# shiyao-li/NextBestPath

Hardware: AMD Instinct MI355X
Metric: exploration steps/s (+ NBP maps/s) at 256x256 (higher is better)
Workload: dtype f32

## Files before the change

include/nbp_hip.h:

```cpp
#ifndef NBP_HIP_H
#define NBP_HIP_H

#include <stddef.h>
#include <stdint.h>

#ifdef __cplusplus
extern "C" {
#endif

#define NBP_E_ARG      (-1)
#define NBP_E_WS       (-2)
#define NBP_E_SHAPE    (-3)

int nbp_abi_version(void);
int nbp_device_info(char* arch_host, int arch_len, int* cu_count_host);
int nbp_tuning_active(void);
int nbp_tuning_report(char* buf_host, int len);
int nbp_tile_kernel_symbol(int tile, char* buf_host, int len);

#define NBP_N_CONV 48

typedef struct nbp_weights nbp_weights;

size_t nbp_packed_weights_bytes(void);

int nbp_pack_weights(const void* const* w_host_array, const void* const* scale_host_array,
                     const void* const* shift_host_array, void* packed, size_t packed_bytes,
                     void* stream, nbp_weights** handle_out);
void nbp_free_weights(nbp_weights* handle);

size_t nbp_forward_workspace_bytes(int B, int S);

int nbp_forward_f32(const nbp_weights* handle, const float* x, int B, int S, float* out1,
                    float* out2, void* ws, size_t ws_bytes, void* stream);

typedef struct nbp_layer_timing {
    char name[48];
    double flops;
    float ms;
    int tile, split_k;
    long long M;
    int N, K;
} nbp_layer_timing;
int nbp_forward_timed_f32(const nbp_weights* handle, const float* x, int B, int S, float* out1,
                          float* out2, void* ws, size_t ws_bytes, void* stream,
                          nbp_layer_timing* timings_host, int max_entries, int* n_entries_host);

double nbp_forward_flops(int B, int S);

int nbp_pack_weights_bf16(const void* const* w_host_array, const void* const* scale_host_array,
                          const void* const* shift_host_array, void* packed, size_t packed_bytes,
                          void* stream, nbp_weights** handle_out);
size_t nbp_packed_weights_bytes_bf16(void);
size_t nbp_forward_workspace_bytes_bf16(int B, int S);
int nbp_pack_upconv_weight_bf16(const float* w_oihw, int N, int C, unsigned short* dst, void* stream);
int nbp_forward_bf16(const nbp_weights* handle, const float* x, int B, int S, float* out1,
                     float* out2, void* ws, size_t ws_bytes, void* stream);
int nbp_forward_timed_bf16(const nbp_weights* handle, const float* x, int B, int S, float* out1,
                           float* out2, void* ws, size_t ws_bytes, void* stream,
                           nbp_layer_timing* timings_host, int max_entries, int* n_entries_host);

size_t nbp_packed_weights_bytes_split(void);
int nbp_pack_weights_split(const void* const* w_host_array, const void* const* scale_host_array,
                           const void* const* shift_host_array, void* packed, size_t packed_bytes, void* stream,
                           nbp_weights** handle_out);
size_t nbp_forward_workspace_bytes_split(int B, int S);
int nbp_forward_split_f32(const nbp_weights* handle, const float* x, int B, int S, float* out1, float* out2, void* ws,
                          size_t ws_bytes, void* stream);
int nbp_forward_timed_split_f32(const nbp_weights* handle, const float* x, int B, int S, float* out1, float* out2,
                                void* ws, size_t ws_bytes, void* stream, nbp_layer_timing* timings_host,
                                int max_entries, int* n_entries_host);
int nbp_pack_conv_weight_split(const float* w_oihw, int N, int C, int ksize, const float* scale_or_null, int c_off,
                               int c_total, void* dst_planes, void* wamax_out, void* stream);
int nbp_amax_f32(const float* x, long long n, void* amax_inout, void* stream);
int nbp_pack_upconv_weight_split(const float* w_oihw, int N, int C, void* dst_planes, void* wamax_out, void* stream);
int nbp_upconv3x3_split_f32(const float* src, int C, int B, int H, int W, const void* planes_up, const void* wamax_up, int N,
                            const float* scale, const float* shift, int relu, float* out, const void* amax_in_or_null,
                            void* amax_out_or_null, int split_k, void* ws, size_t ws_bytes, void* stream);
size_t nbp_conv_split_workspace_bytes(int B, int H, int W, int N, int split_k);
size_t nbp_conv_split_planned_workspace_bytes(int B, int H, int W, int C, int N, int ups, int* split_k_out);
size_t nbp_conv_split_planned_workspace_bytes_k(int B, int H, int W, int C, int N, int ups, int split_k, int* split_k_out);
int nbp_conv3x3_split_f32(const float* src0, int C0, const float* src1, int C1, int ups, int B, int H, int W,
                          const void* w_planes, const void* wamax, int N, const float* scale, const float* shift, int relu,
                          float* out, const void* amax_in_or_null, void* amax_out_or_null, int split_k, void* ws,
                          size_t ws_bytes, void* stream);
size_t nbp_conv_first_wgrad_workspace_bytes(void);
int nbp_conv_first_wgrad_f32(const float* x_nchw, int B, int H, int W, const float* dy, float* dw, void* ws, size_t ws_bytes, void* stream);
int nbp_prepack_weights_split(const void* descs_dev, int n, void* wamax_words, void* stream);
int nbp_prepack_desc_bytes(void);
int nbp_pack_conv_weight_split_prezeroed(const float* w_oihw, int N, int C, int ksize, int c_total, void* dst_planes,
                                         void* wamax_zeroed, void* stream);
int nbp_pack_conv_weight_split_dgrad_known(const float* w_oihw, int N, int C, int c_total, void* dst_planes, const void* wamax_known,
                                           void* stream);
int nbp_pack_upconv_weight_split_dgrad(const float* w_oihw, int N, int C, void* dst_planes, void* wamax_out, void* stream);
size_t nbp_upconv_split_dgrad_workspace_bytes(int B, int H, int W, int N, int C);
int nbp_upconv3x3_split_dgrad_f32(const float* dy, int N, int B, int H, int W, const void* planes, const void* wamax, int C,
                                  const float* scale, const float* shift, float* dx, const void* amax_in, void* amax_out_or_null,
                                  void* ws, size_t ws_bytes, void* stream);
size_t nbp_upconv_wgrad_split_workspace_bytes(int B, int Hs, int Ws, int C, int N);
int nbp_upconv_wgrad_split_f32(const float* x, int C, int B, int Hs, int Ws, const float* dy, int N, float* dw,
                               const void* amax_x, const void* amax_y, void* ws, size_t ws_bytes, void* stream);
int nbp_conv1x1_split_f32(const float* src, int C, long long M, const void* w_planes, const void* wamax, int N,
                          const float* scale, const float* shift, int relu, float* out, const void* amax_in, void* stream);
int nbp_pack_conv1x1_weight_split_dgrad(const float* w_nc, int N, int C, void* dst_planes, void* wamax_out, void* stream);
int nbp_pack_conv_weight_split_dgrad(const float* w_oihw, int N, int C, int c_total, void* dst_planes, void* wamax_out, void* stream);

int nbp_conv_bn_part_rows(int B, int H, int W);
int nbp_conv3x3_split_bn_f32(const float* src0, int C0, const float* src1, int C1, int ups, int B, int H, int W,
                             const void* w_planes, const void* wamax, int N, const float* scale, const float* shift, int relu,
                             float* out, const void* amax_in_or_null, void* amax_out_or_null, int split_k, void* ws,
                             size_t ws_bytes, double* bn_part, int* bn_rows, void* stream);
int nbp_upconv3x3_split_bn_f32(const float* src, int C, int B, int H, int W, const void* planes_up, const void* wamax_up, int N,
                               const float* scale, const float* shift, int relu, float* out, const void* amax_in_or_null,
                               void* amax_out_or_null, int split_k, void* ws, size_t ws_bytes, double* bn_part, int* bn_rows,
                               void* stream);
int nbp_pack_conv_weight_split_h1(const float* w_oihw, int N, int C, int ksize, const float* scale_or_null, int c_off,
                                  int c_total, void* dst_planes, void* wamax_out, void* stream);
int nbp_pack_conv_weight_split_prezeroed_h1(const float* w_oihw, int N, int C, int ksize, int c_total, void* dst_planes,
                                            void* wamax_zeroed, void* stream);
int nbp_pack_conv_weight_split_dgrad_h1(const float* w_oihw, int N, int C, int c_total, void* dst_planes, void* wamax_out, void* stream);
int nbp_pack_conv_weight_split_dgrad_known_h1(const float* w_oihw, int N, int C, int c_total, void* dst_planes, const void* wamax_known,
                                              void* stream);
int nbp_pack_upconv_weight_split_h1(const float* w_oihw, int N, int C, void* dst_planes, void* wamax_out, void* stream);
int nbp_pack_upconv_weight_split_dgrad_h1(const float* w_oihw, int N, int C, void* dst_planes, void* wamax_out, void* stream);
int nbp_pack_conv1x1_weight_split_dgrad_h1(const float* w_nc, int N, int C, void* dst_planes, void* wamax_out, void* stream);
int nbp_prepack_weights_split_h1(const void* descs_dev, int n, void* wamax_words, void* stream);
int nbp_conv3x3_split_f32_h1(const float* src0, int C0, const float* src1, int C1, int ups, int B, int H, int W,
                             const void* w_planes, const void* wamax, int N, const float* scale, const float* shift, int relu,
                             float* out, const void* amax_in_or_null, void* amax_out_or_null, int split_k, void* ws,
                             size_t ws_bytes, void* stream);
int nbp_conv3x3_split_bn_f32_h1(const float* src0, int C0, const float* src1, int C1, int ups, int B, int H, int W,
                                const void* w_planes, const void* wamax, int N, const float* scale, const float* shift, int relu,
                                float* out, const void* amax_in_or_null, void* amax_out_or_null, int split_k, void* ws,
                                size_t ws_bytes, double* bn_part, int* bn_rows, void* stream);
int nbp_upconv3x3_split_f32_h1(const float* src, int C, int B, int H, int W, const void* planes_up, const void* wamax_up, int N,
                               const float* scale, const float* shift, int relu, float* out, const void* amax_in_or_null,
                               void* amax_out_or_null, int split_k, void* ws, size_t ws_bytes, void* stream);
int nbp_upconv3x3_split_bn_f32_h1(const float* src, int C, int B, int H, int W, const void* planes_up, const void* wamax_up, int N,
                                  const float* scale, const float* shift, int relu, float* out, const void* amax_in_or_null,
                                  void* amax_out_or_null, int split_k, void* ws, size_t ws_bytes, double* bn_part, int* bn_rows,
                                  void* stream);
int nbp_upconv3x3_split_dgrad_f32_h1(const float* dy, int N, int B, int H, int W, const void* planes, const void* wamax, int C,
                                     const float* scale, const float* shift, float* dx, const void* amax_in, void* amax_out_or_null,
                                     void* ws, size_t ws_bytes, void* stream);
int nbp_conv1x1_split_f32_h1(const float* src, int C, long long M, const void* w_planes, const void* wamax, int N,
                             const float* scale, const float* shift, int relu, float* out, const void* amax_in, void* stream);
int nbp_upconv_wgrad_split_f32_h1(const float* x, int C, int B, int Hs, int Ws, const float* dy, int N, float* dw,
                                  const void* amax_x, const void* amax_y, void* ws, size_t ws_bytes, void* stream);
int nbp_conv_wgrad_split_f32_h1(const float* src0, int C0, const float* src1, int C1, int ups, int B, int H, int W, int ksize,
                                const float* dy, int N, int c_real, int n_real, float* dw, const void* amax0_or_null,
                                const void* amax1_or_null, const void* amaxy_or_null, void* ws, size_t ws_bytes, void* stream);
int nbp_bn_train_forward_part4_f32(const float* x, long long M, int C, const float* gamma, const float* beta, float eps,
                                   float momentum, float* running_mean, float* running_var, int relu, float* mean, float* invstd,
                                   float* y, void* amax_out, double* stat_out, int stat_doubles, const double* part, int rows,
                                   const float* zero_row, void* stream);
int nbp_conv_igemm_bf16(const unsigned short* src0, int C0, const unsigned short* src1, int C1, int ups,
                        int B, int H, int W, int ksize, const unsigned short* w_packed, int N,
                        const float* scale, const float* shift, int relu, unsigned short* out,
                        int split_k, int tile, void* ws, size_t ws_bytes, void* stream);
size_t nbp_conv_igemm_bf16_workspace_bytes(int B, int H, int W, int N, int split_k);
int nbp_pack_conv_weight_bf16(const float* w_oihw, int N, int C, int ksize, const float* scale_or_null,
                              int c_off, int c_total, unsigned short* dst, void* stream);
int nbp_f32_to_bf16(const float* in, long long n, unsigned short* out, void* stream);
int nbp_bf16_to_f32(const unsigned short* in, long long n, float* out, void* stream);

int nbp_conv_igemm_f32(const float* src0, int C0, const float* src1, int C1, int ups, int B, int H,
                       int W, int ksize, const float* w_packed, int N, const float* scale,
                       const float* shift, int relu, float* out, int split_k, int tile, void* ws,
                       size_t ws_bytes, void* stream);
size_t nbp_conv_igemm_workspace_bytes(int B, int H, int W, int N, int split_k);

int nbp_pack_conv_weight(const float* w_oihw, int N, int C, int ksize, const float* scale_or_null,
                         int c_off, int c_total, float* dst, void* stream);

int nbp_conv_first_f32(const float* x_nchw, int B, int H, int W, const float* w_oihw,
                       const float* scale, const float* shift, float* out_nhwc, void* stream);
int nbp_conv_first_linear_f32(const float* x_nchw, int B, int H, int W, const float* w_oihw, const float* scale,
                              const float* shift, float* out_nhwc, void* stream);
int nbp_maxpool2_nhwc_f32(const float* in, int B, int H, int W, int C, float* out, void* stream);
int nbp_psi_gate_f32(const float* q, int F, const float* w_psi, const float* s_t2, const float* x,
                     int C, long long M, float* out, void* stream);
int nbp_final_1x1_f32(const float* in, int B, int H, int W, int C, const float* w_oc, int n_out,
                      const float* scale, const float* shift, int sigmoid, float* out_nchw,
                      void* stream);
int nbp_nchw_to_nhwc_f32(const float* in, int B, int C, int H, int W, float* out, void* stream);
int nbp_nhwc_to_nchw_f32(const float* in, int B, int C, int H, int W, float* out, void* stream);

int nbp_transform_points_f32(const float* points, long long N, float cx, float cy, float cz,
                             float* out_2d, void* stream);
int nbp_map_points_to_imgs_f32(const float* pts2d, int n, long long m, int S0, int S1, float lo,
                               float hi, float* out, void* stream);
int nbp_point_position_i64(const float* pts2d, long long K, int S0, int S1, float lo, float hi,
                           long long* out_2xK, void* stream);
int nbp_map_accumulate_f32(const float* points, long long N, const long long* N_dev_or_null, float cx,
                           float cy, float cz, const float* bounds_host, int n_bounds, float band_lo,
                           float band_hi, int S, float lo, float hi, float* out6, void* stream);
int nbp_step_maps_f32(const float* points, long long N, const long long* N_dev_or_null, float cx, float cy,
                      float cz, const float* bounds_host, int n_bounds, float band_lo, float band_hi, int S,
                      float lo, float hi, float* traj_pts, int n_traj_old, const float* traj_fresh_host,
                      int n_traj_fresh, float* out6, float* net_in5, void* stream);
int nbp_step_maps_batch_f32(int n, const float* const* points, const long long* N_cap, const long long* const* N_dev,
                            const float* poses_xyz_host, const float* bounds_host, const int* n_bounds,
                            const float* band_lo_hi_host, int S, float lo, float hi, float* const* traj_pts,
                            const int* n_traj_old, const float* traj_fresh_host, const int* n_traj_fresh,
                            float* out6_all, float* net_in_all, void* stream);
size_t nbp_cloud_bins_bytes(const float* lo_xz_host, const float* hi_xz_host, long long capacity);
int nbp_cloud_bins_geometry(const float* lo_xz_host, const float* hi_xz_host, long long capacity, int* nx_nz_maxpages_host,
                            float* x0_z0_tile_host);
int nbp_cloud_bins_init(void* store, size_t store_bytes, const float* lo_xz_host, const float* hi_xz_host, long long capacity,
                        void* stream);
int nbp_step_maps_binned_f32(void* store, int page_bound, const float* points, long long N, const long long* N_dev_or_null,
                             float cx, float cy, float cz, const float* bounds_host, int n_bounds, float band_lo, float band_hi,
                             int S, float lo, float hi, float* traj_pts, int n_traj_old, const float* traj_fresh_host,
                             int n_traj_fresh, float* out6, float* net_in5, void* stream);
int nbp_step_maps_prefiled_f32(void* store, int page_bound, const float* points, long long N, const long long* N_dev_or_null,
                               float cx, float cy, float cz, const float* bounds_host, int n_bounds, float band_lo, float band_hi,
                               int S, float lo, float hi, float* traj_pts, int n_traj_old, const float* traj_fresh_host,
                               int n_traj_fresh, float* out6, float* net_in5, void* stream);
int nbp_step_maps_binned_batch_f32(int n, void* const* stores, const int* page_bound, const float* const* points,
                                   const long long* N_cap, const long long* const* N_dev, const float* poses_xyz_host,
                                   const float* bounds_host, const int* n_bounds, const float* band_lo_hi_host, int S, float lo,
                                   float hi, float* const* traj_pts, const int* n_traj_old, const float* traj_fresh_host,
                                   const int* n_traj_fresh, float* out6_all, float* net_in_all, void* stream);
int nbp_coverage_count_planned_batch_f32(int n, void* const* plans, const int* G, float threshold, const float* bbox_lo_host,
                                         const float* bbox_hi_host, const float* const* pc3, const long long* N,
                                         const long long* const* N_dev, const long long* sample_k, const unsigned* seed,
                                         const unsigned* epoch, int* const* count_accum, int* const* m_out, void* stream);
int nbp_unproject_append_shaded_batch_f32(int n, const float* const* depth, const void* const* zface, const float* const* verts,
                                          const int* const* faces, const float* const* vcolors, const float* cams12_host,
                                          int n_frames, int H, int W, float tan_half_fov, float fov_range,
                                          double gathering_factor, const unsigned* seeds, float ambient, int* const* counts2,
                                          float* const* cloud, float* const* cloud_rgb, long long* const* cloud_count,
                                          const long long* capacity, void* const* ws, size_t ws_bytes_each, void* stream);
int nbp_raster_zface_batch_f32(int n, const float* const* verts, const int* n_verts, const int* const* faces, const int* n_faces,
                               const float* cams12_host, int n_frames, int H, int W, float tan_half_fov, float z_clip,
                               float* const* zbuf, void* const* zface, void* const* ws, const size_t* ws_bytes, void* stream);


// ... 224 lines not shown
```

nextbestpath_amd/_lib.py:

```python
from __future__ import annotations

import ctypes as C
import os
import threading

HERE = os.path.dirname(os.path.abspath(__file__))
LIB_PATH = os.path.join(HERE, "libnbp_hip.so")

_vp, _i, _ll, _f, _sz, _d = C.c_void_p, C.c_int, C.c_longlong, C.c_float, C.c_size_t, C.c_double

SIGNATURES = {
    "nbp_abi_version": (_i, []),
    "nbp_device_info": (_i, [C.c_char_p, _i, C.POINTER(_i)]),
    "nbp_tuning_active": (_i, []),
    "nbp_tuning_report": (_i, [C.c_char_p, _i]),
    "nbp_tile_kernel_symbol": (_i, [_i, C.c_char_p, _i]),
    "nbp_packed_weights_bytes": (_sz, []),
    "nbp_pack_weights": (_i, [C.POINTER(_vp), C.POINTER(_vp), C.POINTER(_vp), _vp, _sz, _vp, C.POINTER(_vp)]),
    "nbp_free_weights": (None, [_vp]),
    "nbp_forward_workspace_bytes": (_sz, [_i, _i]),
    "nbp_forward_f32": (_i, [_vp, _vp, _i, _i, _vp, _vp, _vp, _sz, _vp]),
    "nbp_forward_flops": (_d, [_i, _i]),
    "nbp_conv_igemm_f32": (_i, [_vp, _i, _vp, _i, _i, _i, _i, _i, _i, _vp, _i, _vp, _vp, _i, _vp, _i, _i, _vp,
                                _sz, _vp]),
    "nbp_conv_igemm_workspace_bytes": (_sz, [_i, _i, _i, _i, _i]),
    "nbp_pack_conv_weight": (_i, [_vp, _i, _i, _i, _vp, _i, _i, _vp, _vp]),
    "nbp_conv_first_f32": (_i, [_vp, _i, _i, _i, _vp, _vp, _vp, _vp, _vp]),
    "nbp_maxpool2_nhwc_f32": (_i, [_vp, _i, _i, _i, _i, _vp, _vp]),
    "nbp_psi_gate_f32": (_i, [_vp, _i, _vp, _vp, _vp, _i, _ll, _vp, _vp]),
    "nbp_final_1x1_f32": (_i, [_vp, _i, _i, _i, _i, _vp, _i, _vp, _vp, _i, _vp, _vp]),
    "nbp_nchw_to_nhwc_f32": (_i, [_vp, _i, _i, _i, _i, _vp, _vp]),
    "nbp_nhwc_to_nchw_f32": (_i, [_vp, _i, _i, _i, _i, _vp, _vp]),
    "nbp_transform_points_f32": (_i, [_vp, _ll, _f, _f, _f, _vp, _vp]),
    "nbp_map_points_to_imgs_f32": (_i, [_vp, _i, _ll, _i, _i, _f, _f, _vp, _vp]),
    "nbp_point_position_i64": (_i, [_vp, _ll, _i, _i, _f, _f, _vp, _vp]),
    "nbp_map_accumulate_f32": (_i, [_vp, _ll, _vp, _f, _f, _f, C.POINTER(_f), _i, _f, _f, _i, _f, _f, _vp, _vp]),
    "nbp_coverage_count_planned_batch_f32": (_i, [_i, _vp, _vp, _f, _vp, _vp, _vp, _vp, _vp, _vp, _vp, _vp, _vp, _vp, _vp]),
    "nbp_unproject_append_shaded_batch_f32": (_i, [_i, _vp, _vp, _vp, _vp, _vp, _vp, _i, _i, _i, _f, _f, _d, _vp, _f, _vp, _vp, _vp, _vp,
                                                   _vp, _vp, _sz, _vp]),
    "nbp_raster_zface_batch_f32": (_i, [_i, _vp, _vp, _vp, _vp, _vp, _i, _i, _i, _f, _f, _vp, _vp, _vp, _vp, _vp]),
    "nbp_replan_batch_f32": (_i, [_i, _vp, _vp, _vp, _f, _i, _vp, _vp, _vp, _vp, _vp, _vp, _i, _f, _f, _vp, _vp, _vp, _vp, _vp, _vp, _vp, _vp]),
    "nbp_step_maps_batch_f32": (_i, [_i, _vp, _vp, _vp, _vp, _vp, _vp, _vp, _i, _f, _f, _vp, _vp, _vp, _vp, _vp, _vp, _vp]),
    "nbp_step_maps_f32": (_i, [_vp, _ll, _vp, _f, _f, _f, C.POINTER(_f), _i, _f, _f, _i, _f, _f, _vp, _i, _vp, _i, _vp, _vp, _vp]),
    "nbp_cloud_bins_bytes": (_sz, [C.POINTER(_f), C.POINTER(_f), _ll]),
    "nbp_cloud_bins_geometry": (_i, [C.POINTER(_f), C.POINTER(_f), _ll, C.POINTER(_i), C.POINTER(_f)]),
    "nbp_cloud_bins_init": (_i, [_vp, _sz, C.POINTER(_f), C.POINTER(_f), _ll, _vp]),
    "nbp_step_maps_binned_f32": (_i, [_vp, _i, _vp, _ll, _vp, _f, _f, _f, C.POINTER(_f), _i, _f, _f, _i, _f, _f, _vp, _i, _vp, _i, _vp, _vp,
                                      _vp]),
    "nbp_step_maps_binned_batch_f32": (_i, [_i, _vp, _vp, _vp, _vp, _vp, _vp, _vp, _vp, _vp, _i, _f, _f, _vp, _vp, _vp, _vp, _vp, _vp, _vp]),
    "nbp_unproject_workspace_bytes": (_sz, [_i, _i, _i]),
    "nbp_unproject_append_f32": (_i, [_vp, _vp, C.POINTER(_f), _i, _i, _i, _f, _f, _d, C.c_uint, _vp, _vp, _vp, _ll, _vp, _sz,
                                      _vp]),
    "nbp_raster_workspace_bytes": (_sz, [_i, _i, _i, _i, _i]),
    "nbp_raster_zbuf_f32": (_i, [_vp, _i, _vp, _i, C.POINTER(_f), _i, _i, _i, _f, _f, _i, _vp, _vp, _vp, _sz, _vp]),
    "nbp_segments_hit_mesh_f32": (_i, [_vp, _vp, _i, _vp, _i, _vp, _vp]),
    "nbp_axis_ray_counts_f32": (_i, [_vp, _vp, _i, _vp, _i, _vp, _vp]),
    "nbp_carve_update_f32": (_i, [_vp, _i, _vp, _vp, C.POINTER(_f), _i, _i, _f, _f, _f, _f, _f, _vp, _vp, _vp, _vp, _vp]),
    "nbp_view_state_update_f32": (_i, [_vp, _i, _vp, _vp, _f, C.POINTER(_f), _i, _i, _i, _vp, _vp]),
    "nbp_view_gain_i32": (_i, [_vp, _i, _vp, _vp, C.POINTER(_f), C.POINTER(_f), _i, _i, _i, _i, _i, _f, _f, _vp, _vp]),
    "nbp_carve_view_update_f32": (_i, [_vp, _i, _vp, _vp, C.POINTER(_f), _i, _i, _f, _f, _f, _f, _f, _vp, _vp, _vp, _vp,
                                       C.POINTER(_f), _i, _i, _f, _vp, _vp, _vp, _vp]),
    "nbp_append_points_f32": (_i, [_vp, _ll, C.POINTER(_f), _i, _vp]),
    "nbp_perm_index_host": (C.c_uint, [C.c_uint, C.c_uint, C.c_uint]),
    "nbp_colreduce_workspace_bytes": (_sz, [_ll, _i]),
    "nbp_bn_train_forward_f32": (_i, [_vp, _ll, _i, _vp, _vp, _f, _f, _vp, _vp, _i, _vp, _vp, _vp, _vp, _sz, _vp]),
    "nbp_bn_train_forward_amax_f32": (_i, [_vp, _ll, _i, _vp, _vp, _f, _f, _vp, _vp, _i, _vp, _vp, _vp, _vp, _vp, _sz, _vp]),
    "nbp_bn_train_forward_stat4_f32": (_i, [_vp, _ll, _i, _vp, _vp, _f, _f, _vp, _vp, _i, _vp, _vp, _vp, _vp, _vp, _i, _vp, _sz, _vp]),
    "nbp_bn_train_backward_stat_f32": (_i, [_vp, _vp, _vp, _vp, _ll, _i, _vp, _vp, _vp, _i, _vp, _vp, _vp, _vp, _vp, _vp, _sz, _vp]),
    "nbp_bn_backward_fuses": (_i, [_i]),
    "nbp_bn_train_backward_fused_f32": (_i, [_vp, _vp, _vp, _ll, _i, _vp, _vp, _vp, _i, _vp, _vp, _vp, _vp, _vp, _vp, _sz, _vp]),
    "nbp_bn_train_backward_f32": (_i, [_vp, _vp, _vp, _ll, _i, _vp, _vp, _vp, _i, _vp, _vp, _vp, _vp, _sz, _vp]),
    "nbp_colsum_f32": (_i, [_vp, _vp, _ll, _i, _vp, _vp, _sz, _vp]),
    "nbp_elementwise_f32": (_i, [_i, _vp, _vp, _ll, _vp, _vp]),
    "nbp_rowscale_f32": (_i, [_vp, _vp, _ll, _i, _vp, _vp]),
    "nbp_rowdot_f32": (_i, [_vp, _vp, _i, _ll, _i, _vp, _vp]),
    "nbp_rowscale_backward_f32": (_i, [_vp, _ll, _vp, _vp, _ll, _i, _vp, _vp, _vp]),
    "nbp_outer_f32": (_i, [_vp, _vp, _ll, _i, _vp, _vp]),
    "nbp_maxpool2_backward_f32": (_i, [_vp, _vp, _i, _i, _i, _i, _vp, _vp]),
    "nbp_sum2x2_f32": (_i, [_vp, _i, _i, _i, _i, _vp, _vp]),
    "nbp_slice_channels_f32": (_i, [_vp, _ll, _i, _i, _i, _vp, _vp]),
    "nbp_pad_channels_f32": (_i, [_vp, _ll, _i, _i, _vp, _vp]),
    "nbp_pack_conv_weight_padded": (_i, [_vp, _i, _i, _i, _i, _i, _vp, _vp]),
    "nbp_pack_conv_weight_dgrad": (_i, [_vp, _i, _i, _i, _i, _i, _vp, _vp]),
    "nbp_conv_wgrad_workspace_bytes": (_sz, [_i, _i, _i, _i, _i, _i, _i]),
    "nbp_conv_wgrad_f32": (_i, [_vp, _i, _vp, _i, _i, _i, _i, _i, _i, _vp, _i, _i, _i, _vp, _vp, _sz, _vp]),
    "nbp_conv_wgrad_split_f32": (_i, [_vp, _i, _vp, _i, _i, _i, _i, _i, _i, _vp, _i, _i, _i, _vp, _vp, _vp, _vp, _vp, _sz, _vp]),
    "nbp_gather_values_f32": (_i, [_vp, _vp, _i, _i, _i, _i, _vp, _vp]),
    "nbp_scatter_values_f32": (_i, [_vp, _vp, _i, _i, _i, _i, _vp, _vp]),
    "nbp_loss_f32": (_i, [_i, _vp, _vp, _ll, _f, _vp, _vp, _vp, _sz, _vp]),
    "nbp_augment_batch_f32": (_i, [_vp, _vp, _vp, _i, _i, _vp, _vp, _vp]),
    "nbp_fuse_obstacle_f32": (_i, [_vp, _vp, _vp, _f, _i, _vp, _vp, _vp]),
    "nbp_score_candidates_f32": (_i, [_vp, _i, _f, _f, _vp, _i, _vp, _i, _f, _f, _vp, _vp, _vp, _vp, _vp]),
    "nbp_edges_blocked_u8": (_i, [_vp, _i, _f, _f, _f, _f, _vp, _vp, _i, _vp, _vp]),
    "nbp_plan_search_host": (_i, [_i, _vp, _vp, _i, _vp, _vp, _vp, _vp, _vp, _vp, _vp, _i, _i, _f, _f, _vp, _i, _f, _f,
                                  _vp, _i, _i, _i, _vp, _vp, _vp, _vp, _vp, _i, _vp]),
    "nbp_coverage_workspace_bytes": (_sz, [C.POINTER(_f), C.POINTER(_f), _f, _ll]),
    "nbp_coverage_count_f32": (_i, [_vp, _i, _vp, _ll, _vp, _ll, C.c_uint, _f, C.POINTER(_f), C.POINTER(_f), _vp, _vp,
                                    _vp, _sz, _vp]),
}



class LayerTiming(C.Structure):
    _fields_ = [("name", C.c_char * 48), ("flops", _d), ("ms", _f), ("tile", _i), ("split_k", _i), ("M", _ll),
                ("N", _i), ("K", _i)]


SIGNATURES["nbp_forward_timed_f32"] = (_i, [_vp, _vp, _i, _i, _vp, _vp, _vp, _sz, _vp, C.POINTER(LayerTiming), _i,
                                            C.POINTER(_i)])
SIGNATURES["nbp_forward_timed_bf16"] = SIGNATURES["nbp_forward_timed_f32"]
SIGNATURES["nbp_pack_weights_bf16"] = SIGNATURES["nbp_pack_weights"]
SIGNATURES["nbp_packed_weights_bytes_bf16"] = SIGNATURES["nbp_packed_weights_bytes"]
SIGNATURES["nbp_pack_upconv_weight_bf16"] = (_i, [_vp, _i, _i, _vp, _vp])
SIGNATURES["nbp_forward_workspace_bytes_bf16"] = SIGNATURES["nbp_forward_workspace_bytes"]
SIGNATURES["nbp_forward_bf16"] = SIGNATURES["nbp_forward_f32"]
SIGNATURES["nbp_packed_weights_bytes_split"] = SIGNATURES["nbp_packed_weights_bytes"]
SIGNATURES["nbp_pack_weights_split"] = SIGNATURES["nbp_pack_weights"]
SIGNATURES["nbp_forward_workspace_bytes_split"] = SIGNATURES["nbp_forward_workspace_bytes"]
SIGNATURES["nbp_forward_split_f32"] = SIGNATURES["nbp_forward_f32"]
SIGNATURES["nbp_forward_timed_split_f32"] = SIGNATURES["nbp_forward_timed_f32"]
SIGNATURES["nbp_pack_conv_weight_split"] = (_i, [_vp, _i, _i, _i, _vp, _i, _i, _vp, _vp, _vp])
SIGNATURES["nbp_amax_f32"] = (_i, [_vp, _ll, _vp, _vp])
SIGNATURES["nbp_pack_upconv_weight_split"] = (_i, [_vp, _i, _i, _vp, _vp, _vp])
SIGNATURES["nbp_upconv3x3_split_f32"] = (_i, [_vp, _i, _i, _i, _i, _vp, _vp, _i, _vp, _vp, _i, _vp, _vp, _vp, _i, _vp, _sz, _vp])
SIGNATURES["nbp_conv_split_workspace_bytes"] = SIGNATURES["nbp_conv_igemm_workspace_bytes"]
SIGNATURES["nbp_conv_split_planned_workspace_bytes"] = (_sz, [_i, _i, _i, _i, _i, _i, _vp])
SIGNATURES["nbp_conv_split_planned_workspace_bytes_k"] = (_sz, [_i, _i, _i, _i, _i, _i, _i, _vp])
SIGNATURES["nbp_conv3x3_split_f32"] = (_i, [_vp, _i, _vp, _i, _i, _i, _i, _i, _vp, _vp, _i, _vp, _vp, _i, _vp, _vp, _vp, _i, _vp,
                                            _sz, _vp])
SIGNATURES["nbp_pack_upconv_weight_split_dgrad"] = (_i, [_vp, _i, _i, _vp, _vp, _vp])
SIGNATURES["nbp_upconv_split_dgrad_workspace_bytes"] = (_sz, [_i, _i, _i, _i, _i])
SIGNATURES["nbp_upconv3x3_split_dgrad_f32"] = (_i, [_vp, _i, _i, _i, _i, _vp, _vp, _i, _vp, _vp, _vp, _vp, _vp, _vp, _sz, _vp])
SIGNATURES["nbp_upconv_wgrad_split_workspace_bytes"] = (_sz, [_i, _i, _i, _i, _i])
SIGNATURES["nbp_upconv_wgrad_split_f32"] = (_i, [_vp, _i, _i, _i, _i, _vp, _i, _vp, _vp, _vp, _vp, _sz, _vp])
SIGNATURES["nbp_pack_conv_weight_split_prezeroed"] = (_i, [_vp, _i, _i, _i, _i, _vp, _vp, _vp])
SIGNATURES["nbp_pack_conv_weight_split_dgrad_known"] = (_i, [_vp, _i, _i, _i, _vp, _vp, _vp])
SIGNATURES["nbp_prepack_weights_split"] = (_i, [_vp, _i, _vp, _vp])
SIGNATURES["nbp_prepack_desc_bytes"] = (_i, [])
SIGNATURES["nbp_rowscale_amax_f32"] = (_i, [_vp, _vp, _ll, _i, _vp, _vp, _vp])
SIGNATURES["nbp_conv_first_linear_f32"] = (_i, [_vp, _i, _i, _i, _vp, _vp, _vp, _vp, _vp])
SIGNATURES["nbp_conv_first_wgrad_workspace_bytes"] = (_sz, [])
SIGNATURES["nbp_conv_first_wgrad_f32"] = (_i, [_vp, _i, _i, _i, _vp, _vp, _vp, _sz, _vp])
SIGNATURES["nbp_conv1x1_split_f32"] = (_i, [_vp, _i, _ll, _vp, _vp, _i, _vp, _vp, _i, _vp, _vp, _vp])
SIGNATURES["nbp_pack_conv1x1_weight_split_dgrad"] = (_i, [_vp, _i, _i, _vp, _vp, _vp])
SIGNATURES["nbp_pack_conv_weight_split_dgrad"] = (_i, [_vp, _i, _i, _i, _vp, _vp, _vp])
SIGNATURES["nbp_conv_bn_part_rows"] = (_i, [_i, _i, _i])
SIGNATURES["nbp_conv3x3_split_bn_f32"] = (_i, [_vp, _i, _vp, _i, _i, _i, _i, _i, _vp, _vp, _i, _vp, _vp, _i, _vp, _vp, _vp, _i, _vp,
                                               _sz, _vp, C.POINTER(_i), _vp])
SIGNATURES["nbp_upconv3x3_split_bn_f32"] = (_i, [_vp, _i, _i, _i, _i, _vp, _vp, _i, _vp, _vp, _i, _vp, _vp, _vp, _i, _vp, _sz, _vp,
                                                 C.POINTER(_i), _vp])
SIGNATURES["nbp_bn_train_forward_part4_f32"] = (_i, [_vp, _ll, _i, _vp, _vp, _f, _f, _vp, _vp, _i, _vp, _vp, _vp, _vp, _vp, _i, _vp, _i, _vp, _vp])
for _n in ("nbp_pack_conv_weight_split", "nbp_pack_conv_weight_split_prezeroed", "nbp_pack_conv_weight_split_dgrad",
           "nbp_pack_conv_weight_split_dgrad_known", "nbp_pack_upconv_weight_split", "nbp_pack_upconv_weight_split_dgrad",
           "nbp_pack_conv1x1_weight_split_dgrad", "nbp_prepack_weights_split", "nbp_conv3x3_split_f32", "nbp_conv3x3_split_bn_f32",
           "nbp_upconv3x3_split_f32", "nbp_upconv3x3_split_bn_f32", "nbp_upconv3x3_split_dgrad_f32", "nbp_conv1x1_split_f32",
           "nbp_upconv_wgrad_split_f32", "nbp_conv_wgrad_split_f32"):
    SIGNATURES[_n + "_h1"] = SIGNATURES[_n]
SIGNATURES["nbp_conv_igemm_bf16"] = SIGNATURES["nbp_conv_igemm_f32"]
SIGNATURES["nbp_conv_igemm_bf16_workspace_bytes"] = SIGNATURES["nbp_conv_igemm_workspace_bytes"]
SIGNATURES["nbp_pack_conv_weight_bf16"] = SIGNATURES["nbp_pack_conv_weight"]
SIGNATURES["nbp_f32_to_bf16"] = (_i, [_vp, _ll, _vp, _vp])
SIGNATURES["nbp_bf16_to_f32"] = (_i, [_vp, _ll, _vp, _vp])
_fpp, _ipp = C.POINTER(_f), C.POINTER(_i)
SIGNATURES["nbp_scene_fill_workspace_bytes"] = (_sz, [_fpp, _ipp, _i, _ll, _d])
SIGNATURES["nbp_scene_fill_cells_f32"] = (_i, [_vp, _ll, _vp, _fpp, _ipp, _i, _d, _i, C.c_uint, _vp, _vp, _vp, _sz, _vp])
SIGNATURES["nbp_scene_gather_f32"] = (_i, [_vp, _vp, _i, _i, _vp, _ll, _vp, _vp])
SIGNATURES["nbp_scene_coverage_workspace_bytes"] = (_sz, [_fpp, _ipp, _i, _d])
SIGNATURES["nbp_scene_coverage_f32"] = (_i, [_vp, _vp, _i, _vp, _vp, _i, _fpp, _ipp, _d, _vp, _vp, _sz, _vp])
SIGNATURES["nbp_coverage_plan_bytes"] = (_sz, [_fpp, _fpp, _f, _i])
SIGNATURES["nbp_coverage_plan_workspace_bytes"] = (_sz, [_fpp, _fpp, _f, _i])
SIGNATURES["nbp_coverage_plan_build_f32"] = (_i, [_vp, _i, _f, _fpp, _fpp, _vp, _sz, _vp, _sz, _vp])
SIGNATURES["nbp_coverage_count_planned_f32"] = (_i, [_vp, _i, _f, _fpp, _fpp, _vp, _ll, _vp, _ll, C.c_uint, C.c_uint, _vp, _vp,
                                                     _vp])
SIGNATURES["nbp_points_in_fov_u8"] = (_i, [_vp, _i, _fpp, _i, _i, _i, _f, _f, _vp, _vp, _vp])
SIGNATURES["nbp_sample_points_f32"] = (_i, [_vp, _ll, _vp, _ll, C.c_uint, _vp, _vp, _vp])
SIGNATURES["nbp_raster_rgb_workspace_bytes"] = (_sz, [_i, _i, _i, _i])
SIGNATURES["nbp_raster_rgbz_f32"] = (_i, [_vp, _i, _vp, _i, _vp, _fpp, _i, _i, _i, _f, _f, _f, _f, _vp, _vp, _vp, _sz, _vp])
SIGNATURES["nbp_unproject_append_rgb_f32"] = (_i, [_vp, _vp, _vp, _fpp, _i, _i, _i, _f, _f, _d, C.c_uint, _vp, _vp, _vp, _vp, _ll,
                                                   _vp, _sz, _vp])
SIGNATURES["nbp_raster_zface_f32"] = (_i, [_vp, _i, _vp, _i, _fpp, _i, _i, _i, _f, _f, _vp, _vp, _vp, _sz, _vp])
SIGNATURES["nbp_shade_image_f32"] = (_i, [_vp, _vp, _vp, _vp, _fpp, _i, _i, _i, _f, _f, _f, _vp, _vp])
SIGNATURES["nbp_unproject_append_shaded_f32"] = (_i, [_vp, _vp, _vp, _vp, _vp, _vp, _fpp, _i, _i, _i, _f, _f, _d, C.c_uint, _f,
                                                      _vp, _vp, _vp, _vp, _ll, _vp, _sz, _vp])
SIGNATURES["nbp_mdb_open"] = (_i, [C.c_char_p, C.c_ulonglong, _i, C.POINTER(_vp)])
SIGNATURES["nbp_mdb_close"] = (_i, [_vp])
SIGNATURES["nbp_mdb_entries"] = (_ll, [_vp])
SIGNATURES["nbp_mdb_put"] = (_i, [_vp, C.c_char_p, _sz, C.c_char_p, _sz])
SIGNATURES["nbp_mdb_del"] = (_i, [_vp, C.c_char_p, _sz])
SIGNATURES["nbp_mdb_get"] = (_i, [_vp, C.c_char_p, _sz, _vp, _sz, C.POINTER(_sz)])
SIGNATURES["nbp_mdb_keys"] = (_i, [_vp, _vp, _sz, C.POINTER(_sz)])
SIGNATURES["nbp_mdb_stat"] = (_i, [_vp, C.POINTER(C.c_ulonglong)])
SIGNATURES["nbp_gate_mid_workspace_bytes"] = (_sz, [_ll, _i])
SIGNATURES["nbp_gate_mid_forward_f32"] = (_i, [_vp, _vp, _ll, _i, _vp, _vp, _vp, _vp, _f, _f, _vp, _vp, _vp, _vp, _f, _f, _vp, _vp, _vp, _vp,
                                               _vp, _vp, _vp, _vp, _vp, _vp, _vp, _sz, _vp])
SIGNATURES["nbp_gate_mid_backward_f32"] = (_i, [_vp, _vp, _vp, _vp, _vp, _ll, _i, _vp, _vp, _vp, _vp, _vp, _vp, _vp, _vp, _vp, _vp, _vp, _vp,
                                                _vp, _vp, _vp, _vp, _vp, _vp, _sz, _vp])
SIGNATURES["nbp_sum_n_f32"] = (_i, [_i, _vp, _vp, _ll, _i, _vp, _vp])
SIGNATURES["nbp_unproject_append_filed_f32"] = (_i, [_vp, _vp, _vp, _vp, _vp, _vp, _vp, _fpp, _i, _i, _i, _f, _f, _d, C.c_uint, _f,
                                                     _vp, _vp, _vp, _vp, _ll, _vp, _vp, _vp, _i, _vp, _sz, _vp])
SIGNATURES["nbp_step_maps_prefiled_f32"] = SIGNATURES["nbp_step_maps_binned_f32"]
SIGNATURES["nbp_slice_obstacle_f32"] = (_i, [_vp, _vp, _i, _f, _f, _f, _i, _f, _f, _f, _vp, _vp])
SIGNATURES["nbp_slice_obstacle_fig_f32"] = (_i, [_vp, _vp, _i, _f, _f, _f, _i, _f, _f, _f, _f, _f, _f, _vp, _vp])
SIGNATURES["nbp_slice_obstacle_fig_batch_f32"] = (_i, [_i, _vp, _vp, _vp, _vp, _i, _f, _f, _f, _f, _f, _f, _vp, _vp])
SIGNATURES["nbp_goal_values_batch_f32"] = (_i, [_i, _vp, _vp, _vp, _vp, _i, _f, _f, _vp, _vp, _vp])
SIGNATURES["nbp_hindsight_cells_batch_i32"] = (_i, [_i, _vp, _vp, _i, _f, _f, _vp, _vp])

_lock = threading.Lock()
_lib = None


class NbpHipError(RuntimeError):
    pass


def lib() -> C.CDLL:
    global _lib
    if _lib is not None:
        return _lib
    with _lock:
        if _lib is not None:
            return _lib
        if not os.path.exists(LIB_PATH):
            raise NbpHipError(
                f"{LIB_PATH} is missing: build it with `python -m nextbestpath_amd.build` "
                "(hipcc --offload-arch=gfx950). There is no CPU fallback.")
        import torch
        handle = C.CDLL(LIB_PATH)
        for name, (res, args) in SIGNATURES.items():
            try:
                fn = getattr(handle, name)
            except AttributeError as e:
                raise NbpHipError(f"libnbp_hip.so does not export {name}") from e
            fn.restype = res
            fn.argtypes = args
        _lib = handle
    return _lib


_ERR = {-1: "NBP_E_ARG (bad argument)", -2: "NBP_E_WS (workspace too small)", -3: "NBP_E_SHAPE (unsupported shape)"}


def check(rc: int, what: str) -> None:
    if rc != 0:
        msg = _ERR.get(rc, f"hipError_t {rc}" if rc > 0 else f"error {rc}")
        raise NbpHipError(f"{what} failed: {msg}")


def ptr(t) -> int:
    if t is None:
        return 0
    if not t.is_contiguous():
        raise ValueError("tensor passed to the HIP path must be contiguous")
    return t.data_ptr()


_knobs = {}
NUMERICS_KNOBS = {"NBP_CONV_PRECISION", "NBP_SPLIT_MAX_K", "NBP_SPLIT_MAX_K_SMALL", "NBP_GATE_PSI", "NBP_CONV_HEAD", "NBP_BF16_PSI",
                  "NBP_BF16_FUSE"}


def tuning_active() -> bool:
    return os.environ.get("NBP_TUNING") == "1"


def tune(name: str, default: str) -> str:
    v = default
    if tuning_active():
        e = os.environ.get(name)
        if e is not None and e != "":
            v = e
    _knobs[name] = (default, v)
    return v


def effective_knobs() -> dict:
    out = {k: v for k, (d, v) in _knobs.items() if v != d}
    if _lib is not None:
        buf = C.create_string_buffer(4096)
        if _lib.nbp_tuning_report(buf, 4096) > 0:
            for item in buf.value.decode().split(","):
                if "=" in item:
                    k, v = item.split("=", 1)
# ... 16 lines not shown
```

nextbestpath_amd/csrc/nbp_forward.hip:

```cpp
#include "common.h"
#include "nbp_internal.h"
#include <stdio.h>
#include <stdlib.h>
#include <string.h>

namespace {

enum Kind { K_FIRST, K_CONV3, K_ATT_G, K_ATT_X, K_PSI, K_FINAL };
struct LayerSpec { Kind kind; int cin, cout, k; };

struct Table {
    LayerSpec L[NBP_N_CONV];
    size_t w_off[NBP_N_CONV];
    size_t s_off[NBP_N_CONV], t_off[NBP_N_CONV];
    size_t total_floats;
    size_t w3_off[NBP_N_CONV];
    size_t w3u_off[NBP_N_CONV];
    bool is_up[NBP_N_CONV];
    int up_rank[NBP_N_CONV];
    size_t total3_bytes;
    size_t wup16_off[NBP_N_CONV], total_up16_bytes;
    size_t w1_off[NBP_N_CONV];
    int gate_rank[NBP_N_CONV];
    Table() {
// ... 367 lines not shown
};
struct PathSplit : PathF32 {
    typedef AmaxBook Ctx;
    static constexpr int MODE = 2;
    static ConvPlan plan(long long M, int N, int chunks, int groups, int H = 0, int ksize = 0, int ups = 0) {
        if (ksize == 1) return ConvPlan{NBP_TILE_SPLIT_GATE, 1, chunks};
        const ConvPlan p = nbp_plan_conv_split(M, N, chunks, 0, groups, H, H, ksize, ups);
        return p.tile ? p : PathF32::plan(M, N, chunks, groups, H, ksize);
    }
    static int conv(Ctx& ctx, const nbp_weights* h, const int* li, const Ops& o, const Ops* o2, int C0, int C1, int ups, int B,
                    int H, int ks, int N, void* ws, size_t wsb, hipStream_t st) {
        if (ks == 1 && C1 == C0 && C0 % 64 == 0 && !ups && h->w1[li[0]] && (!o2 || h->w1[li[1]])) {
            const long long M = (long long)B * H * H;
            ConvOperandsSplit s[2];
            for (int g = 0; g < (o2 ? 2 : 1); ++g) {
                const Ops& q = g ? *o2 : o;
                s[g] = ConvOperandsSplit{q.src0, q.src1, h->w1[li[g]], q.scale, q.shift, q.out, nullptr, nullptr, h->wamax1[li[g]], nullptr,
                                         nullptr, nullptr};
                int rc = ctx.ensure(q.src0, M * C0, &s[g].amax0);
                if (!rc) rc = ctx.ensure(q.src1, M * C1, &s[g].amax1);
                if (rc) return rc;
            }
            GatePsi psi;
            for (int g = 0; g < 2; ++g) {
                const int l = li[(g && o2) ? 1 : 0] + 2;
                psi.wpsi[g] = (const float*)h->w[l]; psi.st[g] = h->scale[l]; psi.gated[g] = ctx.gated[(g && o2) ? 1 : 0];
            }
            unsigned* gslot[2] = {nullptr, nullptr};
            if (ctx.gated[0]) for (int g = 0; g < (o2 ? 2 : 1); ++g) psi.gated_amax[g] = gslot[g] = ctx.unbound();
            static const int psi_on_load = nbp_tune_int("NBP_SPLIT_PSI_ON_LOAD", 1);
            const ConvPlan pc = nbp_plan_conv_split(M, C0, (C0 + C0) / 32 * 9, 0, o2 ? 2 : 1, H, H, 3, 0);
            psi.psi_only = psi_on_load && (C0 >= 128 || psi_on_load >= 2) && ctx.gated[0] && gslot[0] && (!o2 || gslot[1]) && pc.tile != 0 &&
                           M * C0 * 4 < (1ll << 31);
            int fused = 0;
            const int rc = nbp_gate1x1_split_launch_g(s[0], o2 ? &s[1] : nullptr, C0, M, N, 1, st, ctx.gated[0] ? &psi : nullptr, &fused);
            if (fused) {
                ctx.gated_taken = true;
                for (int g = 0; g < (o2 ? 2 : 1); ++g) {
                    if (gslot[g]) ctx.bind(ctx.gated[g], gslot[g]);
                    else ctx.alias(ctx.gated[g], (g ? *o2 : o).src1);
                    if (psi.psi_only) { ctx.psi_key[g] = ctx.gated[g]; ctx.psi_x[g] = (g ? *o2 : o).src1; }
                }
            }
            return rc;
        }
        const ConvPlan p = nbp_plan_conv_split((long long)B * H * H, N, (C0 + C1) / 32 * ks * ks, 0, o2 ? 2 : 1, H, H, ks, ups);
        if (!p.tile) return PathF32::conv(ctx, h, li, o, o2, C0, C1, ups, B, H, ks, N, ws, wsb, st);
        const long long hw = (long long)B * (ups ? H / 2 : H) * (ups ? H / 2 : H);
        ConvOperandsSplit s[2];
        for (int g = 0; g < (o2 ? 2 : 1); ++g) {
            const Ops& q = g ? *o2 : o;
            s[g] = ConvOperandsSplit{q.src0, q.src1, h->w3[li[g]], q.scale, q.shift, q.out, nullptr, nullptr, h->wamax[li[g]], nullptr,
                                     h->w3u[li[g]], h->wamax_u[li[g]]};
            int rc = ctx.ensure(q.src0, hw * C0, &s[g].amax0);
            if (!rc && C1) rc = ctx.ensure(q.src1, hw * C1, &s[g].amax1);
            if (rc) return rc;
            s[g].amax_out = ctx.fresh(q.out);
            for (int k = 0; k < 2; ++k)
                if (ctx.psi_key[k] && q.src0 == ctx.psi_key[k]) {
                    s[g].src0 = ctx.psi_x[k]; s[g].psi0 = ctx.psi_key[k];
                    ctx.psi_key[k] = nullptr; ctx.psi_x[k] = nullptr;
                }
        }
        float* pools[2] = {ctx.pool, nullptr};
        int pooled = 0, headed = 0;
        const int rc = nbp_conv_split_launch_g(s[0], o2 ? &s[1] : nullptr, C0, C1, ups, B, H, H, ks, N, 1, 0, ws, wsb, st,
                                               (ctx.pool && !o2) ? pools : nullptr, &pooled, (ctx.head.out && !o2) ? &ctx.head : nullptr,
                                               &headed);
        if (headed) ctx.head_taken = true;
        if (pooled) {
            ctx.pool_taken = true;
            ctx.alias(ctx.pool, o.out);
        }
        return rc;
    }
    static int first(Ctx& ctx, const float* x, int B, int s, const nbp_weights* h, T* out, hipStream_t st) {
        unsigned* slot = ctx.fresh(out);
        int did = 0;
        const int rc = nbp_conv_first_amax_launch(x, B, s, s, (const float*)h->w[0], h->scale[0], h->shift[0], out, slot, &did, st);
        if (!did && slot) --ctx.n;
        return rc;
    }
    static int pool(Ctx& ctx, const T* in, int B, int H, int Cn, T* out, hipStream_t st) {
        ctx.alias(out, in);
        return nbp_maxpool2_nhwc_f32(in, B, H, H, Cn, out, st);
    }
    static int gate(Ctx& ctx, const T* q, int F, const float* w, const float* s2, const T* x, int Cn, long long M, T* out,
                    hipStream_t st) {
        ctx.alias(out, x);
        return nbp_psi_gate_f32(q, F, w, s2, x, Cn, M, out, st);
    }
};
struct Bf16Ctx : NoCtx {
    bf16_t* gated[2] = {nullptr, nullptr};
    bool gated_taken = false;
    void offer_gated(void* g0, void* g1) { gated[0] = (bf16_t*)g0; gated[1] = (bf16_t*)g1; gated_taken = false; }
    bool took_gated() { const bool t = gated_taken; gated[0] = gated[1] = nullptr; gated_taken = false; return t; }
    bf16_t* pool = nullptr;
    bool pool_taken = false;
    void offer_pool(void* p) { pool = (bf16_t*)p; pool_taken = false; }
    bool took_pool() { const bool t = pool_taken; pool = nullptr; pool_taken = false; return t; }
    ConvHead head = {nullptr, nullptr, nullptr, nullptr};
    bool head_taken = false;
    void offer_head(const float* w, const float* sc, const float* sh, float* out) { head = ConvHead{w, sc, sh, out}; head_taken = false; }
    bool took_head() { const bool t = head_taken; head = ConvHead{nullptr, nullptr, nullptr, nullptr}; head_taken = false; return t; }
};
struct PathBF16 {
    typedef bf16_t T;
    typedef ConvOperandsH Ops;
    typedef Bf16Ctx Ctx;
    static constexpr int CHUNK = 64;
    static ConvPlan plan(long long M, int N, int chunks, int groups, int H = 0, int ksize = 0, int ups = 0) {
        return nbp_plan_conv_bf16(M, N, chunks, 0, 0, groups, H, H, ksize, ups);
    }
    static constexpr int MODE = 1;
    static int conv(Ctx& ctx, const nbp_weights* h, const int* li, const Ops& o, const Ops* o2, int C0, int C1, int ups, int B, int H,
                    int ks, int N, void* ws, size_t wsb, hipStream_t st) {
        Ops a = o, b = o2 ? *o2 : o;
        a.wpk_up = (const bf16_t*)h->wup16[li[0]];
        if (o2) b.wpk_up = (const bf16_t*)h->wup16[li[1]];
        bf16_t* pools[2] = {ctx.pool, nullptr};
        int pooled = 0, headed = 0, psi_fused = 0;
        GatePsiH psi{{nullptr, nullptr}, {nullptr, nullptr}, {nullptr, nullptr}};
        const bool gate = ks == 1 && C1 == C0 && ctx.gated[0] && (!o2 || ctx.gated[1]);
        if (gate)
            for (int g = 0; g < (o2 ? 2 : 1); ++g) {
                const int l = li[g] + 2;
                psi.wpsi[g] = (const float*)h->w[l]; psi.st[g] = h->scale[l]; psi.gated[g] = ctx.gated[g];
            }
        const int rc = nbp_conv_igemm_bf16_launch_g(a, o2 ? &b : nullptr, C0, C1, ups, B, H, H, ks, N, 1, 0, 0, ws, wsb, st,
                                                    (ctx.pool && !o2) ? pools : nullptr, &pooled,
                                                    (ctx.head.out && !o2) ? &ctx.head : nullptr, &headed, gate ? &psi : nullptr, &psi_fused);
        if (pooled) ctx.pool_taken = true;
        if (headed) ctx.head_taken = true;
        if (psi_fused) ctx.gated_taken = true;
        return rc;
    }
    static int first(Ctx&, const float* x, int B, int s, const nbp_weights* h, T* out, hipStream_t st) {
        return nbp_conv_first_bf16_launch(x, B, s, s, (const float*)h->w[0], h->scale[0], h->shift[0], out, st);
    }
    static int pool(Ctx&, const T* in, int B, int H, int C, T* out, hipStream_t st) { return nbp_maxpool2_bf16_launch(in, B, H, H, C, out, st); }
    static int gate(Ctx&, const T* q, int F, const float* w, const float* s2, const T* x, int C, long long M, T* out, hipStream_t st) {
        return nbp_psi_gate_bf16_launch(q, F, w, s2, x, C, M, out, st);
    }
    static int head(const T* in, int B, int H, int C, const float* w, int no, const float* sc, const float* sh, int sig,
                    float* out, hipStream_t st) {
        return nbp_final_1x1_bf16_launch(in, B, H, H, C, w, no, sc, sh, sig, out, st);
    }
};

template <typename P>
size_t splitk_scratch_floats(long long M, int N, int cin_total, int taps, int groups, int H, int ups = 0) {
    ConvPlan p = P::plan(M, N, cin_total / P::CHUNK * taps, groups, H, taps == 9 ? 3 : 1, ups);
    return p.split_k > 1 ? (size_t)groups * p.split_k * M * N : 0;
}

template <typename P>
int run_forward(const nbp_weights* h, const float* x, int B, int S, float* out1, float* out2, Bump& bp,
                hipStream_t st, Timer* tm = nullptr) {
    typedef typename P::T T;
    typedef typename P::Ops Ops;
    char nm[48];
    const bool dry = bp.dry;
    const int enc[5] = {64, 128, 256, 512, 1024};
    int rc = 0;
    size_t sk = 0;
    {
        int s = S;
        sk = 0;
        for (int e = 0; e < 5; ++e, s /= 2) {
            long long M = (long long)B * s * s;
            if (e > 0) sk = max(sk, splitk_scratch_floats<P>(M, enc[e], enc[e - 1], 9, 1, s));
            sk = max(sk, splitk_scratch_floats<P>(M, enc[e], enc[e], 9, 1, s));
            if (e < 4) {
                for (int g = 1; g <= 2; ++g) {
                    sk = max(sk, splitk_scratch_floats<P>(M, enc[e], enc[e + 1], 9, g, s));
                    sk = max(sk, splitk_scratch_floats<P>(M, enc[e], enc[e + 1], 9, g, s, 1));
                    sk = max(sk, splitk_scratch_floats<P>(M, enc[e], enc[e], 9, g, s));
                    sk = max(sk, splitk_scratch_floats<P>(M, enc[e], 2 * enc[e], 9, g, s));
                    sk = max(sk, splitk_scratch_floats<P>(M, enc[e] / 2, 2 * enc[e], 1, g, s));
                }
            }
        }
    }
    float* skws = bp.take<float>(sk ? sk : 64);
    const size_t skbytes = sk * sizeof(float);
    typename P::Ctx ctx;
    rc = ctx.init(bp, st, dry);

    auto conv2 = [&](const char* name, int ng, const int* li, const T* const* s0, int C0, const T* const* s1,
                     int C1, int ups, int Hh, int ksize, int N, T* const* out) {
        if (dry || rc) return;
        Ops o[2];
        for (int g = 0; g < ng; ++g)
            o[g] = Ops{s0[g], s1 ? s1[g] : nullptr, (const T*)h->w[li[g]], h->scale[li[g]], h->shift[li[g]], out[g]};
        rc = P::conv(ctx, h, li, o[0], ng == 2 ? &o[1] : nullptr, C0, C1, ups, B, Hh, ksize, N, skws, skbytes, st);
        if (tm && !rc) {
            const long long M = (long long)B * Hh * Hh;
            const int K = (C0 + C1) * ksize * ksize;
            ConvPlan p = P::plan(M, N, K / P::CHUNK, ng, Hh, ksize, ups);
            tm->mark(name, 2.0 * ng * M * N * K, p.tile, p.split_k, M, N, K);
        }
    };
    auto conv = [&](const char* name, int li, const T* s0, int C0, const T* s1, int C1, int ups, int Hh,
                    int ksize, int N, T* out) {
        const T* s0a[1] = {s0};
        const T* s1a[1] = {s1};
        T* oa[1] = {out};
        conv2(name, 1, &li, s0a, C0, s1 ? s1a : nullptr, C1, ups, Hh, ksize, N, oa);
    };
    auto stamp = [&](const char* name, double flops, long long M, int N, int K) {
        if (tm && !dry && !rc) tm->mark(name, flops, -1, 1, M, N, K);
    };

    T* skip[5];
    int li = 0;
    int s = S;
    const T* prev = nullptr;
    T* pooled_next = nullptr;
    bool pool_fused = false;
    for (int e = 0; e < 5; ++e) {
        const int co = enc[e];
        const size_t n = (size_t)B * s * s * co;
        T* a = bp.take<T>(n);
        T* b = bp.take<T>(n);
        if (e == 0) {
            if (!dry && !rc) rc = P::first(ctx, x, B, s, h, a, st);
            stamp("Conv1.conv.0(first)", 2.0 * B * s * s * 64 * 45, (long long)B * s * s, 64, 45);
        } else {
            T* pooled = pooled_next;
            if (!dry && !rc && !pool_fused) rc = P::pool(ctx, prev, B, 2 * s, enc[e - 1], pooled, st);
            snprintf(nm, sizeof nm, "Maxpool%d", e);
            stamp(nm, 0, (long long)B * s * s, enc[e - 1], 0);
            snprintf(nm, sizeof nm, "Conv%d.conv.0", e + 1);
            conv(nm, li, pooled, enc[e - 1], nullptr, 0, 0, s, 3, co, a);
        }
        snprintf(nm, sizeof nm, "Conv%d.conv.3", e + 1);
        if (e < 4) {
            pooled_next = bp.take<T>((size_t)B * (s / 2) * (s / 2) * co);
            ctx.offer_pool(pooled_next);
        }
        conv(nm, li + 1, a, co, nullptr, 0, 0, s, 3, co, b);
        pool_fused = ctx.took_pool();
        li += 2;
        skip[e] = b; prev = b;
        if (e < 4) s /= 2;
    }
    const int li_d1 = 10, li_d2 = 22;
    bool head2_fused = false;
    const T* cur[2] = {skip[4], skip[4]};
    for (int Lv = 5; Lv >= 2; --Lv) {
        const int ng = Lv >= 4 ? 2 : 1;
        const int g0 = Lv >= 4 ? 0 : 1;
        const int co = enc[Lv - 2], ci = enc[Lv - 1];
        const int sr = S >> (Lv - 2);
        const long long M = (long long)B * sr * sr;
        const T* xs = skip[Lv - 2];
        T *dd[2], *q[2], *ag[2], *u[2], *o[2];
        int lis[2];
        const T *src[2], *xsa[2] = {xs, xs};
        for (int g = 0; g < ng; ++g) {
            dd[g] = bp.take<T>((size_t)M * co); q[g] = bp.take<T>((size_t)M * (co / 2)); ag[g] = bp.take<T>((size_t)M * co);
            u[g] = bp.take<T>((size_t)M * co); o[g] = bp.take<T>((size_t)M * co);
            const int d = g0 + g;
            lis[g] = (d == 0 ? li_d1 : li_d2) + (5 - Lv) * 6;
            src[g] = cur[d];
        }
        const char* tag = ng == 2 ? "{1,2}" : "2";
        auto shifted = [&](int k, int* dst) { for (int g = 0; g < ng; ++g) dst[g] = lis[g] + k; };
        int l[2];
        snprintf(nm, sizeof nm, "Up%d_%s.up.1", Lv, tag);
        shifted(0, l); conv2(nm, ng, l, src, ci, nullptr, 0, 1, sr, 3, co, dd);
        snprintf(nm, sizeof nm, "Att%d_%s.W_g+W_x", Lv, tag);
        ctx.offer_gated(ag[0], ng == 2 ? ag[1] : nullptr);
        shifted(1, l); conv2(nm, ng, l, (const T* const*)dd, co, xsa, co, 0, sr, 1, co / 2, q);
        const bool psi_fused = ctx.took_gated();
        for (int g = 0; g < ng && !dry && !rc && !psi_fused; ++g)
            rc = P::gate(ctx, q[g], co / 2, (const float*)h->w[lis[g] + 3], h->scale[lis[g] + 3], xs, co, M, ag[g], st);
        snprintf(nm, sizeof nm, "Att%d_%s.psi*x", Lv, tag);
        stamp(nm, 2.0 * ng * M * (co / 2), M, 1, co / 2);
        snprintf(nm, sizeof nm, "Up_conv%d_%s.conv.0", Lv, tag);
        shifted(4, l); conv2(nm, ng, l, (const T* const*)ag, co, (const T* const*)dd, co, 0, sr, 3, co, u);
        snprintf(nm, sizeof nm, "Up_conv%d_%s.conv.3", Lv, tag);
        if (Lv == 2 && !dry) ctx.offer_head((const float*)h->w[47], h->scale[47], h->shift[47], out2);
        shifted(5, l); conv2(nm, ng, l, (const T* const*)u, co, nullptr, 0, 0, sr, 3, co, o);
        if (Lv == 2) head2_fused = ctx.took_head();
        for (int g = 0; g < ng; ++g) cur[g0 + g] = o[g];
        if (Lv == 4) {
            if (!dry && !rc)
                rc = P::head(cur[0], B, S / 4, 256, (const float*)h->w[46], 8, h->scale[46], h->shift[46], 0, out1, st);
            stamp("Final1", 2.0 * B * (S / 4) * (S / 4) * 8 * 256, (long long)B * (S / 4) * (S / 4), 8, 256);
        }
    }
    if (!dry && !rc && !head2_fused)
        rc = P::head(cur[1], B, S, 64, (const float*)h->w[47], 1, h->scale[47], h->shift[47], 1, out2, st);
    stamp("Final2", 2.0 * B * S * S * 64, (long long)B * S * S, 1, 64);
    return rc;
}

}

template <typename P>
static size_t workspace_bytes_impl(int B, int S) {
    if (B < 1 || S < 16 || S % 16) return 0;
    Bump bp{nullptr, 0, 0, true};
    run_forward<P>(nullptr, nullptr, B, S, nullptr, nullptr, bp, nullptr);
    return bp.off + 256;
}

template <typename P>
static int forward_impl(const nbp_weights* handle, const float* x, int B, int S, float* out1, float* out2, void* ws,
                        size_t ws_bytes, void* stream, nbp_layer_timing* timings_host, int max_entries,
                        int* n_entries_host) {
    NBP_RETURN_IF(!handle || !x || !out1 || !out2 || !ws, NBP_E_ARG);
    NBP_RETURN_IF(handle->bf16 != (P::MODE == 1 ? 1 : 0) || (P::MODE == 2 && !handle->split), NBP_E_ARG);
    NBP_RETURN_IF(B < 1, NBP_E_ARG);
    NBP_RETURN_IF(S < 16 || S % 16, NBP_E_SHAPE);
    NBP_RETURN_IF(ws_bytes < workspace_bytes_impl<P>(B, S), NBP_E_WS);
    uintptr_t p = ((uintptr_t)ws + 255) / 256 * 256;
    Bump bp{(char*)p, ws_bytes, 0, false};
    if (!timings_host) return run_forward<P>(handle, x, B, S, out1, out2, bp, (hipStream_t)stream);
    NBP_RETURN_IF(!n_entries_host || max_entries < 1, NBP_E_ARG);
    static Timer tm;
    tm.st = (hipStream_t)stream; tm.out = timings_host; tm.cap = max_entries;
    int rc = tm.begin();
    if (rc) return rc;
    rc = run_forward<P>(handle, x, B, S, out1, out2, bp, (hipStream_t)stream, &tm);
    int rc2 = tm.finish();
    *n_entries_host = tm.n;
    return rc ? rc : rc2;
}

extern "C" size_t nbp_forward_workspace_bytes(int B, int S) { return workspace_bytes_impl<PathF32>(B, S); }
extern "C" size_t nbp_forward_workspace_bytes_bf16(int B, int S) { return workspace_bytes_impl<PathBF16>(B, S); }

extern "C" int nbp_forward_f32(const nbp_weights* handle, const float* x, int B, int S, float* out1, float* out2,
                               void* ws, size_t ws_bytes, void* stream) {
    NBP_ENTER();
    return forward_impl<PathF32>(handle, x, B, S, out1, out2, ws, ws_bytes, stream, nullptr, 0, nullptr);
}

extern "C" size_t nbp_forward_workspace_bytes_split(int B, int S) { return workspace_bytes_impl<PathSplit>(B, S); }
extern "C" int nbp_forward_split_f32(const nbp_weights* handle, const float* x, int B, int S, float* out1, float* out2,
                                     void* ws, size_t ws_bytes, void* stream) {
    NBP_ENTER();
    return forward_impl<PathSplit>(handle, x, B, S, out1, out2, ws, ws_bytes, stream, nullptr, 0, nullptr);
}
extern "C" int nbp_forward_timed_split_f32(const nbp_weights* handle, const float* x, int B, int S, float* out1,
                                           float* out2, void* ws, size_t ws_bytes, void* stream,
                                           nbp_layer_timing* timings_host, int max_entries, int* n_entries_host) {
    NBP_ENTER();
    NBP_RETURN_IF(!timings_host || !n_entries_host, NBP_E_ARG);
    return forward_impl<PathSplit>(handle, x, B, S, out1, out2, ws, ws_bytes, stream, timings_host, max_entries,
                                   n_entries_host);
// ... 41 lines not shown
```

nextbestpath_amd/csrc/nbp_internal.h:

```cpp
#pragma once
#include "common.h"

typedef unsigned short bf16_t;

enum { NBP_TILE_AUTO = 0, NBP_TILE_128x128 = 1, NBP_TILE_256x64 = 2, NBP_TILE_256x32 = 3, NBP_TILE_128x64 = 4,
       NBP_TILE_64x128 = 5,
       NBP_TILE_HALO_128 = 6, NBP_TILE_HALO_64 = 7,
       NBP_TILE_HALO4_128 = 8, NBP_TILE_HALO4_64 = 9,
       NBP_TILE_SPLIT_HALO_64 = 10, NBP_TILE_SPLIT_UP = 11,
       NBP_TILE_HALO_UP_128 = 12, NBP_TILE_HALO_UP_64 = 13,
       NBP_TILE_RESERVED_14 = 14,
       NBP_TILE_SPLIT_HALO_R8 = 15, NBP_TILE_SPLIT_UP_R8 = 16,
       NBP_TILE_SPLIT_UP_DGRAD = 17,
       NBP_TILE_SPLIT_HALO_128 = 18,
       NBP_TILE_SPLIT_GATE = 19 };
struct TileInfo { int bm, bn; };
struct ConvPlan { int tile; int split_k; int chunks_per_split; };

struct IgemmArgs {
    const float* src0;
    const float* src1;
    int C0, C1;
    int cc0;
    int ups;
    int H, W;
    int Hs, Ws;
    int taps;
    const float* wpk;
    int N;
    const float* scale;
    const float* shift;
    int relu;
    float* out;
    long long M;
    int split_k;
    int chunks_total;
    int chunks_per_split;
    unsigned bytes0, bytes1;
    unsigned bytesw;
    float* partial;
    int groups;
    const float* g_src0;
    const float* g_src1;
    const float* g_wpk;
    const float* g_scale;
    const float* g_shift;
    float* g_out;
    int xcd_remap;
};
struct ConvOperands { const float* src0; const float* src1; const float* wpk; const float* scale; const float* shift; float* out; };
ConvPlan nbp_plan_conv(long long M, int N, int chunks_total, int tile, int split_k, int groups, int H = 0, int W = 0,
                       int ksize = 0);
int nbp_conv_igemm_launch_g(const ConvOperands& o, const ConvOperands* o2, int C0, int C1, int ups, int B, int H, int W,
                            int ksize, int N, int relu, int split_k, int tile, void* ws, size_t ws_bytes, hipStream_t st);

struct ConvOperandsSplit {
    const float* src0; const float* src1; const void* planes; const float* scale; const float* shift; float* out;
    const unsigned* amax0; const unsigned* amax1; const unsigned* wamax; unsigned* amax_out;
    const void* planes_up; const unsigned* wamax_up;
    const float* psi0 = nullptr;
};
ConvPlan nbp_plan_conv_split(long long M, int N, int chunks_total, int split_k, int groups, int H, int W, int ksize, int ups = 0);
int nbp_pack_upconv_weight_split_launch(const float* w_oihw, int N, int C, void* dst, unsigned* wamax_out, hipStream_t st, int one = 0);
struct ConvHead { const float* w; const float* scale; const float* shift; float* out; };
int nbp_conv_split_launch_g(const ConvOperandsSplit& o, const ConvOperandsSplit* o2, int C0, int C1, int ups, int B, int H, int W,
                            int ksize, int N, int relu, int split_k, void* ws, size_t ws_bytes, hipStream_t st,
                            float* const* pool_out = nullptr, int* pooled = nullptr, const struct ConvHead* head = nullptr,
                            int* headed = nullptr, double* bn_part = nullptr, int* bn_rows = nullptr, int one = 0);
int nbp_pack_conv_weight_split_launch(const float* w_oihw, int N, int C, int ksize, const float* scale_or_null, int c_off,
                                      int c_total, void* dst, unsigned* wamax_out, hipStream_t st, int one = 0);
int nbp_amax_launch(const float* x, long long n, unsigned* amax_inout, hipStream_t st);
int nbp_wgrad_split_launch(const float* src0, int C0, const float* src1, int C1, int ups, int B, int H, int W, const float* dy, int N,
                           int n_tiles, int splits, unsigned* amax3, const unsigned* amax0_in, const unsigned* amax1_in,
                           const unsigned* amaxy_in, float* part, hipStream_t st);
int nbp_pack_gate_weight_split_launch(const float* wg, const float* scale_g, const float* wx, const float* scale_x, int N, int C,
                                      void* dst, unsigned* wamax_out, hipStream_t st);
struct GatePsi { const float* wpsi[2]; const float* st[2]; float* gated[2]; unsigned* gated_amax[2] = {nullptr, nullptr};
                 int psi_only = 0; };
int nbp_gate1x1_split_launch_g(const ConvOperandsSplit& o, const ConvOperandsSplit* o2, int C, long long M, int N, int relu,
                               hipStream_t st, const GatePsi* psi = nullptr, int* fused = nullptr);
int nbp_conv_first_amax_launch(const float* x_nchw, int B, int H, int W, const float* w_oihw, const float* scale, const float* shift,
                               float* out_nhwc, unsigned* amax_out, int* did_amax, hipStream_t st);

struct ConvOperandsH { const bf16_t* src0; const bf16_t* src1; const bf16_t* wpk; const float* scale; const float* shift; bf16_t* out;
                       const bf16_t* wpk_up; };
ConvPlan nbp_plan_conv_bf16(long long M, int N, int chunks_total, int tile, int split_k, int groups, int H = 0, int W = 0,
                            int ksize = 0, int ups = 0);
int nbp_pack_upconv_weight_bf16_launch(const float* w_oihw, int N, int C, bf16_t* dst, hipStream_t st);
struct GatePsiH { const float* wpsi[2]; const float* st[2]; bf16_t* gated[2]; };
int nbp_conv_igemm_bf16_launch_g(const ConvOperandsH& o, const ConvOperandsH* o2, int C0, int C1, int ups, int B, int H,
                                 int W, int ksize, int N, int relu, int split_k, int tile, void* ws, size_t ws_bytes,
                                 hipStream_t st, bf16_t* const* pool_out = nullptr, int* pooled = nullptr,
                                 const struct ConvHead* head = nullptr, int* headed = nullptr, const GatePsiH* psi = nullptr,
                                 int* psi_fused = nullptr);
int nbp_conv_first_bf16_launch(const float* x_nchw, int B, int H, int W, const float* w_oihw, const float* scale,
                               const float* shift, bf16_t* out_nhwc, hipStream_t st);
int nbp_maxpool2_bf16_launch(const bf16_t* in, int B, int H, int W, int C, bf16_t* out, hipStream_t st);
int nbp_psi_gate_bf16_launch(const bf16_t* q, int F, const float* w_psi, const float* s_t2, const bf16_t* x, int C,
                             long long M, bf16_t* out, hipStream_t st);
int nbp_final_1x1_bf16_launch(const bf16_t* in, int B, int H, int W, int C, const float* w_oc, int n_out,
                              const float* scale, const float* shift, int sigmoid, float* out_nchw, hipStream_t st);
```

nextbestpath_amd/csrc/nbp_split.hip:

```cpp
#include "common.h"
#include "nbp_internal.h"
#include <cstdlib>

namespace {

typedef _Float16 f16x8 __attribute__((ext_vector_type(8)));
typedef _Float16 f16x2 __attribute__((ext_vector_type(2)));
typedef unsigned u32x4 __attribute__((ext_vector_type(4)));
typedef unsigned u32x2 __attribute__((ext_vector_type(2)));
typedef __attribute__((address_space(3))) void* lds_ptr_t;

constexpr int SPLIT_EXP = 14;
__host__ __device__ inline int amax_exponent(unsigned bits) {
    if (!bits) return SPLIT_EXP;
    int e = (int)((bits >> 23) & 255u) - 127;
    return e < -100 ? -100 : (e > 100 ? 100 : e);
}
__host__ __device__ inline float pow2f(int e) {
    union { unsigned u; float f; } v;
    v.u = (unsigned)(127 + e) << 23;
    return v.f;
}

__device__ __forceinline__ void split_pair(float x0, float x1, unsigned& h, unsigned& l) {
    const _Float16 h0 = (_Float16)x0, h1 = (_Float16)x1;
    const _Float16 l0 = (_Float16)(x0 - (float)h0), l1 = (_Float16)(x1 - (float)h1);
    h = __builtin_bit_cast(unsigned, f16x2{h0, h1});
    l = __builtin_bit_cast(unsigned, f16x2{l0, l1});
}
__device__ __forceinline__ unsigned hi_pair(float x0, float x1) {
    return __builtin_bit_cast(unsigned, f16x2{(_Float16)x0, (_Float16)x1});
}

constexpr int AMAX_WORDS = 64;
#define NBP_SPLIT_MAX_K_DEFAULT 2304
#define NBP_SPLIT_MAX_K_SMALL_DEFAULT 1152
__device__ __forceinline__ void wave_amax(float mx, unsigned* out) {
#pragma unroll
    for (int o = 32; o; o >>= 1) mx = fmaxf(mx, __shfl_xor(mx, o));
    if ((threadIdx.x & 63) == 0)
        atomicMax(out + ((blockIdx.x * 4u + (threadIdx.x >> 6) + blockIdx.y * 17u + blockIdx.z * 29u) & (AMAX_WORDS - 1)), __float_as_uint(mx));
}
__device__ __forceinline__ void block_amax(float mx, unsigned* out, unsigned words = AMAX_WORDS) {
    __shared__ float part[4];
#pragma unroll
    for (int o = 32; o; o >>= 1) mx = fmaxf(mx, __shfl_xor(mx, o));
    if ((threadIdx.x & 63) == 0) part[threadIdx.x >> 6] = mx;
    __syncthreads();
    if (threadIdx.x == 0)
        atomicMax(out + (blockIdx.x & (words - 1)), __float_as_uint(fmaxf(fmaxf(part[0], part[1]), fmaxf(part[2], part[3]))));
}
__device__ __forceinline__ unsigned read_amax(const unsigned* slot) {
    unsigned v = slot[threadIdx.x & (AMAX_WORDS - 1)];
#pragma unroll
    for (int o = 32; o; o >>= 1) { const unsigned u = __shfl_xor(v, o); v = u > v ? u : v; }
    return v;
}

struct SplitOps {
    const float* src0; const float* src1; const void* planes; const float* scale; const float* shift; float* out;
    const unsigned* amax0; const unsigned* amax1; const unsigned* wamax; unsigned* amax_out;
    float* pool_out;
    const float* head_w; const float* head_ss[2]; float* head_out;
    double* bn_part;
    const float* psi0;
};
struct SplitArgs {
    SplitOps g[2];
    int C0, C1, ups, H, W, Hs, Ws, N, relu;
    long long M;
    int split_k, chunks_total, chunks_per_split;
    unsigned bytes0, bytes1, bytesw;
    float* partial;
    int groups, xcd_remap;
};

#ifdef NBP_DBG_TS
__device__ unsigned long long nbp_dbg_ts[8192];
__device__ unsigned nbp_dbg_n;
#define NBP_WALL(tag) do { if (dbg_on) { const unsigned k_ = dbg_i++; if (k_ < 4000) { nbp_dbg_ts[2 * k_] = (unsigned long long)(tag); nbp_dbg_ts[2 * k_ + 1] = wall_clock64(); } } } while (0)
#define NBP_TS(tag) do { if (dbg_on) { const unsigned k_ = dbg_i++; if (k_ < 4000) { nbp_dbg_ts[2 * k_] = (unsigned long long)(tag); nbp_dbg_ts[2 * k_ + 1] = __builtin_readcyclecounter(); } } } while (0)
#else
#define NBP_TS(tag) do {} while (0)
#endif
template <bool ONE, int TW, int TM, int TN, bool PH, bool BS = false, bool P2 = false, bool DG = false>
__global__ __launch_bounds__(256, 2) __attribute__((amdgpu_waves_per_eu(2, 2))) void conv3x3_halo_h2_kernel(SplitArgs a) {
    static_assert(!P2 || PH, "two-parity form: up_conv layers");
    static_assert(!DG || (PH && !BS && !P2), "data gradient of an up_conv layer: the one-parity tap structure");
    constexpr bool PHO = PH && !DG;
    int zs = blockIdx.z;
    const int py = PHO ? (P2 ? zs & 1 : (zs >> 1) & 1) : 0, px = (PHO && !P2) ? zs & 1 : 0;
    if (PHO) zs >>= (P2 ? 1 : 2);
    const int zslice = zs;
    const SplitOps& o = zs >= a.split_k ? a.g[1] : a.g[0];
    if (zs >= a.split_k) zs -= a.split_k;
    constexpr int ROWS = PH ? 2 : 3, TPR = PH ? 2 : 3, TAPS = ROWS * TPR;
    constexpr int BN = TN * 32, NB = BN / 64;
    constexpr int RPB = 32 / TW, TH = 4 * TM * RPB;
    constexpr int HW_ = TW + 2, HPIX = (TH + 2) * HW_;
    constexpr int RS = (HPIX + 7) / 8 * 8 * 16 + 64;
    constexpr int NPL = ONE ? 1 : 2;
    constexpr int HALO_BYTES = 2 * NPL * RS;
    constexpr int WI = TPR * 2 * NPL * NB;
    constexpr int NPAR = P2 ? 2 : 1;
    constexpr int WB1 = WI * 1024, WB = NPAR * WB1;
    constexpr int NF = (HPIX * 4 + 255) / 256;
    static_assert(BN % 64 == 0 && (TH == 16 || TH == 8), "tile shape");
    extern __shared__ __attribute__((aligned(16))) char ldsb[];
    char* const halo = ldsb;
    char* const wbuf = ldsb + HALO_BYTES;
    float* const psil = reinterpret_cast<float*>(ldsb + HALO_BYTES + 2 * WB);

    const int tid = threadIdx.x, lane = tid & 63, wave = tid >> 6;
#ifdef NBP_DBG_TS
    const bool dbg_on = blockIdx.x == gridDim.x / 2 && blockIdx.y == 0 && blockIdx.z == 0 && tid == 64;
    unsigned dbg_i = 0;
    NBP_WALL(100); NBP_TS(101);
#endif
    const int Ht = PHO ? a.Hs : a.H, Wt = PHO ? a.Ws : a.W;
    const int tiles_x = Wt / TW, tiles_y = Ht / TH;
    unsigned tile = blockIdx.x, nt = blockIdx.y;
    if (a.xcd_remap == 1) {
        const unsigned L = blockIdx.x + gridDim.x * blockIdx.y, T = gridDim.x * gridDim.y;
        const unsigned xcd = L & 7u, idx = L >> 3, q = T >> 3, r = T & 7u;
        const unsigned v = xcd * q + min(xcd, r) + idx;
        nt = v % gridDim.y;
        tile = v / gridDim.y;
    } else if (a.xcd_remap == 2) {
        const unsigned L = blockIdx.x + gridDim.x * blockIdx.y;
        const unsigned xcd = L & 7u, idx = L >> 3, nbk = gridDim.y;
        if (nbk >= 8u) {
            const unsigned per = nbk >> 3;
            nt = xcd * per + idx % per;
            tile = idx / per;
        } else {
            const unsigned g = 8u / nbk;
            nt = xcd / g;
            tile = idx * g + xcd % g;
        }
    }
    const unsigned tile_lin = tile;
    const int tx = tile % tiles_x; tile /= tiles_x;
    const int ty = tile % tiles_y;
    const int b = tile / tiles_y;
    const int y0 = ty * TH, x0 = tx * TW;
    const int n0 = nt * BN;

    const unsigned ma0 = read_amax(o.amax0), ma1 = o.amax1 ? read_amax(o.amax1) : 0u;
    const int ea = amax_exponent(ma0 > ma1 ? ma0 : ma1), ew = amax_exponent(*o.wamax);
    const float sa = pow2f(SPLIT_EXP - ea);
    const int einv = ea + ew - 2 * SPLIT_EXP;

    int hpix[NF];
#pragma unroll
    for (int k = 0; k < NF; ++k) {
        const int f = tid + 256 * k;
        const int hr = f >> 2;
        const int hy = hr / HW_, hx = hr - hy * HW_;
        const int yy = y0 - 1 + hy, xx = x0 - 1 + hx;
        const bool ok = hr < HPIX && (unsigned)yy < (unsigned)Ht && (unsigned)xx < (unsigned)Wt;
        hpix[k] = ok ? (DG ? (b * a.Hs + 2 * yy) * a.Ws + 2 * xx
                          : PH ? (b * a.Hs + yy) * a.Ws + xx : (b * a.Hs + (yy >> a.ups)) * a.Ws + (xx >> a.ups)) : -1;
    }
    const int hdst0 = ((tid & 3) >> 1) * RS + (tid >> 2) * 16 + (tid & 1) * 8;
    const __amdgpu_buffer_rsrc_t rs0 =
        __builtin_amdgcn_make_buffer_rsrc(const_cast<float*>(o.src0), 0, a.bytes0, 0x00020000);
    const __amdgpu_buffer_rsrc_t rs1 =
        __builtin_amdgcn_make_buffer_rsrc(const_cast<float*>(o.src1 ? o.src1 : o.src0), 0, a.bytes1, 0x00020000);
    const __amdgpu_buffer_rsrc_t rsw =
        __builtin_amdgcn_make_buffer_rsrc(const_cast<void*>(o.planes), 0, a.bytesw, 0x00020000);
    constexpr unsigned OOB = 0x80000000u;
    const int c16_0 = a.C0 >> 4;

    bool psi_on = false;
    if constexpr (!PH) {
        psi_on = o.psi0 != nullptr;
        if (psi_on) {
#pragma unroll
            for (int k = 0; k < NF; ++k) {
                const int hr = (tid >> 2) + 64 * k;
                if ((tid & 3) == 0 && hr < HPIX) psil[hr] = hpix[k] >= 0 ? o.psi0[hpix[k]] : 0.f;
            }
            __syncthreads();
        }
    }

    u32x4 hreg[NF];
    auto load_halo = [&](int c) {
        if constexpr (DG) {
            const int q = c / c16_0, cbase = (c - q * c16_0) * 16 + (tid & 3) * 4;
            const int shift = (q >> 1) * a.Ws + (q & 1);
#pragma unroll
            for (int k = 0; k < NF; ++k) {
                const unsigned off = hpix[k] >= 0 ? (unsigned)((hpix[k] + shift) * a.C0 + cbase) * 4u : OOB;
                hreg[k] = __builtin_amdgcn_raw_buffer_load_b128(rs0, off, 0, 0);
            }
            return;
        }
        const bool first = c < c16_0;
        const int Cs = first ? a.C0 : a.C1;
        const int cbase = (first ? c : c - c16_0) * 16 + (tid & 3) * 4;
#pragma unroll
        for (int k = 0; k < NF; ++k) {
            const unsigned off = hpix[k] >= 0 ? (unsigned)(hpix[k] * Cs + cbase) * 4u : OOB;
            hreg[k] = first ? __builtin_amdgcn_raw_buffer_load_b128(rs0, off, 0, 0) : __builtin_amdgcn_raw_buffer_load_b128(rs1, off, 0, 0);
        }
    };
    auto store_halo = [&](int c) {
        const bool gated = psi_on && c < c16_0;
#pragma unroll
        for (int k = 0; k < NF; ++k) {
            if ((tid >> 2) + 64 * k >= HPIX) continue;
            f32x4 v = __builtin_bit_cast(f32x4, hreg[k]);
            if constexpr (!PH) { if (gated) v = v * psil[(tid >> 2) + 64 * k]; }
            if constexpr (ONE) {
                *reinterpret_cast<u32x2*>(halo + hdst0 + k * 1024) = u32x2{hi_pair(v[0] * sa, v[1] * sa), hi_pair(v[2] * sa, v[3] * sa)};
                continue;
            }
            unsigned h0, l0, h1, l1;
            split_pair(v[0] * sa, v[1] * sa, h0, l0);
            split_pair(v[2] * sa, v[3] * sa, h1, l1);
            *reinterpret_cast<u32x2*>(halo + hdst0 + k * 1024) = u32x2{h0, h1};
            *reinterpret_cast<u32x2*>(halo + 2 * RS + hdst0 + k * 1024) = u32x2{l0, l1};
        }
    };
    auto issue_w = [&](int u) {
        const int c = u / ROWS, row = u - ROWS * c;
        char* dst = wbuf + (u & 1) * WB;
#pragma unroll
        for (int pq = 0; pq < NPAR; ++pq) {
            const long long pbase = PHO ? (long long)(py * 2 + (P2 ? pq : px)) * a.chunks_total * TAPS * (2 * NPL) * a.N : 0;
#pragma unroll
            for (int k = 0; k < (WI + 3) / 4; ++k) {
                const int q = wave + 4 * k;
                if (WI % 4 != 0 && q >= WI) continue;
                const int tt = q / (2 * NPL * NB), r = q - tt * (2 * NPL * NB);
                const int r4 = r / NB, nb = r - r4 * NB;
                const unsigned woff = (unsigned)((pbase + (((long long)c * TAPS + row * TPR + tt) * (2 * NPL) + r4) * a.N + n0 + nb * 64 + lane) * 16);
                __builtin_amdgcn_raw_ptr_buffer_load_lds(rsw, (lds_ptr_t)(dst + pq * WB1 + q * 1024), 16, woff, 0, 0, 0);
            }
        }
    };

    f32x16 accs[NPAR][TM][TN];
    f32x16 (&acc)[TM][TN] = accs[0];
#pragma unroll
    for (int pq = 0; pq < NPAR; ++pq)
#pragma unroll
        for (int i = 0; i < TM; ++i)
#pragma unroll
            for (int j = 0; j < TN; ++j)
#pragma unroll
                for (int r = 0; r < 16; ++r) accs[pq][i][j][r] = 0.f;

    const int khalf = lane >> 5;
    const int hbase = (TM * wave * RPB + ((lane & 31) / TW)) * HW_ + ((lane & 31) % TW);
    const char* const arow = halo + khalf * RS + hbase * 16;
    const int brow = khalf * NB * 1024 + (lane & 31) * 16;

    const int c_begin = zs * a.chunks_per_split;
    const int c_end = min(c_begin + a.chunks_per_split, a.chunks_total);
    if (c_begin < c_end) {
        load_halo(c_begin);
        issue_w(c_begin * ROWS);
        store_halo(c_begin);
    }
    asm volatile("s_waitcnt vmcnt(0)" ::: "memory");
    __syncthreads();
    __builtin_amdgcn_s_setprio(2);
    for (int c = c_begin; c < c_end; ++c) {
        const bool more = c + 1 < c_end;
        if (more) load_halo(c + 1);
#pragma unroll 1
        for (int row = 0; row < ROWS; ++row) {
            const int u = c * ROWS + row;
            NBP_TS(1);
            if (row < ROWS - 1 || more) issue_w(u + 1);
            const char* Bt = wbuf + (u & 1) * WB + brow;
            if constexpr (P2) {
                constexpr int PX[3] = {1, 0, 0};
                constexpr int PW[3] = {0, 1, 0};
#pragma unroll
                for (int col = 0; col < 3; ++col) {
                    if constexpr (ONE) {
                        u32x4 xh[TM];
#pragma unroll
                        for (int i = 0; i < TM; ++i) xh[i] = *reinterpret_cast<const u32x4*>(arow + ((row + py + i * RPB) * HW_ + col) * 16);
#pragma unroll
                        for (int pq = 0; pq < 2; ++pq) {
                            const int tt = col - pq;
                            if (tt < 0 || tt > 1) continue;
                            u32x4 wh[TN];
#pragma unroll
                            for (int j = 0; j < TN; ++j)
                                wh[j] = *reinterpret_cast<const u32x4*>(Bt + pq * WB1 + ((tt * 2) * NB + (j >> 1)) * 1024 + (j & 1) * 512);
#pragma unroll
                            for (int j = 0; j < TN; ++j)
#pragma unroll
                                for (int i = 0; i < TM; ++i)
                                    accs[pq][i][j] = __builtin_amdgcn_mfma_f32_32x32x16_f16(__builtin_bit_cast(f16x8, xh[i]),
                                                                                            __builtin_bit_cast(f16x8, wh[j]), accs[pq][i][j], 0, 0, 0);
                        }
                        continue;
                    }
                    u32x4 xp[TM][2];
#pragma unroll
                    for (int i = 0; i < TM; ++i)
#pragma unroll
                        for (int p = 0; p < 2; ++p)
                            xp[i][p] = *reinterpret_cast<const u32x4*>(arow + p * (2 * RS) + ((row + py + i * RPB) * HW_ + col) * 16);
#pragma unroll
                    for (int pq = 0; pq < 2; ++pq) {
                        const int tt = col - pq;
                        if (tt < 0 || tt > 1) continue;
                        u32x4 wp[TN][2];
#pragma unroll
                        for (int j = 0; j < TN; ++j)
#pragma unroll
                            for (int p = 0; p < 2; ++p)
                                wp[j][p] = *reinterpret_cast<const u32x4*>(Bt + pq * WB1 + ((tt * 4 + p * 2) * NB + (j >> 1)) * 1024 + (j & 1) * 512);
#pragma unroll
                        for (int v = 0; v < 3; ++v)
#pragma unroll
                            for (int j = 0; j < TN; ++j)
#pragma unroll
                                for (int i = 0; i < TM; ++i)
                                    accs[pq][i][j] = __builtin_amdgcn_mfma_f32_32x32x16_f16(__builtin_bit_cast(f16x8, xp[i][PX[v]]),
                                                                                            __builtin_bit_cast(f16x8, wp[j][PW[v]]), accs[pq][i][j], 0, 0, 0);
                    }
                }
            } else {
            const int pyc = DG ? 1 - ((c / c16_0) >> 1) : py, pxc = DG ? 1 - ((c / c16_0) & 1) : px;
#pragma unroll
            for (int tt = 0; tt < TPR; ++tt) {
                if constexpr (ONE) {
                    u32x4 xh[TM], wh[TN];
#pragma unroll
                    for (int i = 0; i < TM; ++i) xh[i] = *reinterpret_cast<const u32x4*>(arow + ((row + pyc + i * RPB) * HW_ + tt + pxc) * 16);
#pragma unroll
                    for (int j = 0; j < TN; ++j) wh[j] = *reinterpret_cast<const u32x4*>(Bt + ((tt * 2) * NB + (j >> 1)) * 1024 + (j & 1) * 512);
#pragma unroll
                    for (int j = 0; j < TN; ++j)
#pragma unroll
                        for (int i = 0; i < TM; ++i)
                            acc[i][j] = __builtin_amdgcn_mfma_f32_32x32x16_f16(__builtin_bit_cast(f16x8, xh[i]), __builtin_bit_cast(f16x8, wh[j]),
                                                                               acc[i][j], 0, 0, 0);
                    continue;
                }
                u32x4 xp[TM][2], wp[TN][2];
#pragma unroll
                for (int i = 0; i < TM; ++i)
#pragma unroll
                    for (int p = 0; p < 2; ++p)
                        xp[i][p] = *reinterpret_cast<const u32x4*>(arow + p * (2 * RS) + ((row + pyc + i * RPB) * HW_ + tt + pxc) * 16);
#pragma unroll
                for (int j = 0; j < TN; ++j)
#pragma unroll
                    for (int p = 0; p < 2; ++p)
                        wp[j][p] = *reinterpret_cast<const u32x4*>(Bt + ((tt * 4 + p * 2) * NB + (j >> 1)) * 1024 + (j & 1) * 512);
                constexpr int PX[3] = {1, 0, 0};
                constexpr int PW[3] = {0, 1, 0};
#pragma unroll
                for (int v = 0; v < 3; ++v)
#pragma unroll
                    for (int j = 0; j < TN; ++j)
#pragma unroll
                        for (int i = 0; i < TM; ++i)
                            acc[i][j] = __builtin_amdgcn_mfma_f32_32x32x16_f16(__builtin_bit_cast(f16x8, xp[i][PX[v]]),
                                                                               __builtin_bit_cast(f16x8, wp[j][PW[v]]), acc[i][j], 0, 0, 0);
            }
            }
            NBP_TS(2);
            asm volatile("s_waitcnt vmcnt(0)" ::: "memory");
            NBP_TS(3);
            __syncthreads();
            NBP_TS(4);
        }
        if (more) {
            __builtin_amdgcn_s_setprio(0);
            store_halo(c + 1);
            NBP_TS(5);
            __syncthreads();
            NBP_TS(6);
            __builtin_amdgcn_s_setprio(2);
        }
    }

    const bool final_out = (a.split_k == 1);
    float* outp = final_out ? o.out : a.partial + (long long)zslice * a.M * a.N;
    float mx = 0.f;
    constexpr bool HEADABLE = !PH && TN == 2;
    const bool head = HEADABLE && final_out && o.head_out;
    const bool bn_stats = BS && final_out && o.bn_part;
    double* const bsh = reinterpret_cast<double*>(ldsb);
    if constexpr (BS) { if (bn_stats) __syncthreads(); }
    double bs1[BS ? TN : 1], bs2[BS ? TN : 1];
#pragma unroll
    for (int j = 0; j < (BS ? TN : 1); ++j) { bs1[j] = 0.0; bs2[j] = 0.0; }
    float hp[HEADABLE ? TM : 1][16];
    if constexpr (HEADABLE) {
#pragma unroll
        for (int i = 0; i < TM; ++i)
#pragma unroll
            for (int r = 0; r < 16; ++r) hp[i][r] = 0.f;
    }
#pragma unroll
    for (int pq = 0; pq < NPAR; ++pq)
#pragma unroll
    for (int j = 0; j < TN; ++j) {
        const int pxe = P2 ? pq : px;
        const int n = n0 + j * 32 + (lane & 31);
        float sc = 1.f, sh = 0.f;
        if (final_out) { sc = o.scale[n]; sh = o.shift[n]; }
        const float hw = head ? o.head_w[n] : 0.f;
        float vals[TM][16];
#pragma unroll
        for (int i = 0; i < TM; ++i) {
            const long long mrow = PHO ? ((long long)b * a.H + 2 * (y0 + (TM * wave + i) * RPB) + py) * a.W + 2 * x0 + pxe
                                       : ((long long)b * a.H + y0 + (TM * wave + i) * RPB) * a.W + x0;
#pragma unroll
            for (int r = 0; r < 16; ++r) {
                const int pb = (r & 3) + 8 * (r >> 2) + 4 * khalf;
                const int poff = PHO ? 2 * ((pb / TW) * a.W + (pb % TW)) : (pb / TW) * a.W + (pb % TW);
                float v = ldexpf(accs[pq][i][j][r], einv) * sc + sh;
                if (final_out && a.relu) v = fmaxf(v, 0.f);
                mx = fmaxf(mx, fabsf(v));
                if (!head) outp[(mrow + poff) * a.N + n] = v;
                vals[i][r] = v;
                if constexpr (HEADABLE) hp[i][r] = fmaf(v, hw, hp[i][r]);
            }
        }
        if constexpr (BS) {
            if (bn_stats) {
#pragma unroll
                for (int i = 0; i < TM; ++i)
#pragma unroll
                    for (int r = 0; r < 16; ++r) { const double d = (double)vals[i][r]; bs1[j] += d; bs2[j] = fma(d, d, bs2[j]); }
            }
        }
        if (!PH && final_out && o.pool_out) {
            const int Hp = a.H >> 1, Wp = a.W >> 1;
            if constexpr (TW == 32) {
#pragma unroll
                for (int i = 0; i < TM; i += 2) {
                    const long long prow = ((long long)b * Hp + ((y0 + TM * wave + i) >> 1)) * Wp + (x0 >> 1);
#pragma unroll
                    for (int r = 0; r < 16; r += 2) {
                        const int xo = ((r & 3) + 8 * (r >> 2) + 4 * khalf) >> 1;
                        o.pool_out[(prow + xo) * a.N + n] = fmaxf(fmaxf(vals[i][r], vals[i][r + 1]), fmaxf(vals[i + 1][r], vals[i + 1][r + 1]));
                    }
                }
            } else {
#pragma unroll
                for (int i = 0; i < TM; ++i) {
                    const long long prow = ((long long)b * Hp + ((y0 + (TM * wave + i) * RPB) >> 1)) * Wp + (x0 >> 1);
#pragma unroll
                    for (int r = 0; r < 8; r += 2) {
                        const int xo = ((r & 3) + 8 * (r >> 2) + 4 * khalf) >> 1;
                        o.pool_out[(prow + xo) * a.N + n] = fmaxf(fmaxf(vals[i][r], vals[i][r + 1]), fmaxf(vals[i][r + 8], vals[i][r + 9]));
                    }
                }
            }
        }
    }
    if constexpr (HEADABLE) {
        if (head) {
            const float hs = o.head_ss[0][0], ht = o.head_ss[1][0];
#pragma unroll
            for (int i = 0; i < TM; ++i) {
                float p8[8], p4[4], p2[2];
                {
                    const bool up = lane & 16;
#pragma unroll
                    for (int k = 0; k < 8; ++k) p8[k] = (up ? hp[i][8 + k] : hp[i][k]) + __shfl_xor(up ? hp[i][k] : hp[i][8 + k], 16);
                }
                {
                    const bool up = lane & 8;
#pragma unroll
                    for (int k = 0; k < 4; ++k) p4[k] = (up ? p8[4 + k] : p8[k]) + __shfl_xor(up ? p8[k] : p8[4 + k], 8);
                }
                {
                    const bool up = lane & 4;
#pragma unroll
                    for (int k = 0; k < 2; ++k) p2[k] = (up ? p4[2 + k] : p4[k]) + __shfl_xor(up ? p4[k] : p4[2 + k], 4);
                }
                const bool up = lane & 2;
                float dot = (up ? p2[1] : p2[0]) + __shfl_xor(up ? p2[0] : p2[1], 2);
                dot += __shfl_xor(dot, 1);
                const int r = (lane & 31) >> 1;
                const int pb = (r & 3) + 8 * (r >> 2) + 4 * khalf;
                const long long mrow = ((long long)b * a.H + y0 + (TM * wave + i) * RPB) * a.W + x0;
                if (!(lane & 1)) o.head_out[mrow + (pb / TW) * a.W + (pb % TW)] = 1.f / (1.f + expf(-(dot * hs + ht)));
            }
        }
    }
    if constexpr (BS) {
        if (bn_stats) {
#pragma unroll
            for (int j = 0; j < TN; ++j) {
                const double s1 = bs1[j] + __shfl_xor(bs1[j], 32), s2 = bs2[j] + __shfl_xor(bs2[j], 32);
                if (lane < 32) { bsh[(wave * BN + j * 32 + lane) * 2] = s1; bsh[(wave * BN + j * 32 + lane) * 2 + 1] = s2; }
            }
            __syncthreads();
            if (tid < BN) {
                double s1 = 0.0, s2 = 0.0;
#pragma unroll
                for (int w = 0; w < 4; ++w) { s1 += bsh[(w * BN + tid) * 2]; s2 += bsh[(w * BN + tid) * 2 + 1]; }
                const long long row = P2 ? (long long)tile_lin * 2 + py : PH ? (long long)tile_lin * 4 + (py * 2 + px) : (long long)tile_lin;
                o.bn_part[(row * 2) * a.N + n0 + tid] = s1;
                o.bn_part[(row * 2 + 1) * a.N + n0 + tid] = s2;
            }
        }
    }
    if (final_out && o.amax_out) wave_amax(mx, o.amax_out);
#ifdef NBP_DBG_TS
    NBP_TS(7);
    NBP_TS(102); NBP_WALL(103);
    if (dbg_on) nbp_dbg_n = dbg_i;
#endif
}

#ifdef NBP_DBG_TS
extern "C" int nbp_dbg_read(unsigned long long* host, unsigned* n) {
    hipDeviceSynchronize();
    hipMemcpyFromSymbol(n, HIP_SYMBOL(nbp_dbg_n), sizeof(unsigned));
    return (int)hipMemcpyFromSymbol(host, HIP_SYMBOL(nbp_dbg_ts), sizeof(unsigned long long) * 8192);
}
#endif

struct GateArgs {
    SplitOps g[2];
    int C, N, relu;
    int C1;
    long long M;
    unsigned bytes0, bytesw;
    int groups;
    const float* wpsi[2];
    const float* st[2];
    float* gated[2];
    unsigned* gated_amax[2];
    int psi_only;
};

template <bool ONE, int TN, bool PSI>
__global__ __launch_bounds__(256, 2) void gate1x1_h2_kernel(GateArgs a) {
    const SplitOps& o = a.g[blockIdx.z];
    constexpr int BN = TN * 32;
    constexpr int WST = (ONE ? 4 : 8) * BN * 16;
    constexpr int WI = WST / 1024;
    extern __shared__ __attribute__((aligned(16))) char wbuf[];
    const int tid = threadIdx.x, lane = tid & 63, wave = tid >> 6;
    const long long m = (long long)blockIdx.x * 128 + wave * 32 + (lane & 31);
    const int n0 = blockIdx.y * BN, khalf = lane >> 5;
    const unsigned ma0 = read_amax(o.amax0), ma1 = o.amax1 ? read_amax(o.amax1) : 0u;
    const int ea = amax_exponent(ma0 > ma1 ? ma0 : ma1), ew = amax_exponent(*o.wamax);
    const float sa = pow2f(SPLIT_EXP - ea);
    const int einv = ea + ew - 2 * SPLIT_EXP;
    const __amdgpu_buffer_rsrc_t rs0 = __builtin_amdgcn_make_buffer_rsrc(const_cast<float*>(o.src0), 0, a.bytes0, 0x00020000);
    const __amdgpu_buffer_rsrc_t rs1 = __builtin_amdgcn_make_buffer_rsrc(const_cast<float*>(o.src1 ? o.src1 : o.src0), 0, a.bytes0, 0x00020000);
    const __amdgpu_buffer_rsrc_t rsw = __builtin_amdgcn_make_buffer_rsrc(const_cast<void*>(o.planes), 0, a.bytesw, 0x00020000);
    constexpr unsigned OOB = 0x80000000u;
    const int stages0 = a.C >> 5, stages = stages0 + (a.C1 >> 5);
    const unsigned prow = m < a.M ? (unsigned)(m * a.C) * 4u : OOB;

    constexpr int D = 4;
    u32x4 xr[D][2][2];
    auto load_x = [&](int st, int slot) {
        const bool first = st < stages0;
        const unsigned cb = (unsigned)((first ? st : st - stages0) * 32 + khalf * 8) * 4u;
#pragma unroll
        for (int ks = 0; ks < 2; ++ks)
#pragma unroll
            for (int h = 0; h < 2; ++h) {
                const unsigned off = (prow == OOB || st >= stages) ? OOB : prow + cb + ks * 64 + h * 16;
                xr[slot][ks][h] = first ? __builtin_amdgcn_raw_buffer_load_b128(rs0, off, 0, 0) : __builtin_amdgcn_raw_buffer_load_b128(rs1, off, 0, 0);
            }
    };
    auto issue_w = [&](int st) {
        char* dst = wbuf + (st & 1) * WST;
#pragma unroll
        for (int k = 0; k < (WI + 3) / 4; ++k) {
            const int q = wave + 4 * k;
            if (q < WI) {
                constexpr int PER = BN / 64 > 0 ? BN / 64 : 1;
                const int r8 = BN >= 64 ? q / PER : q * 2 + (lane >> 5), nb = BN >= 64 ? q - (q / PER) * PER : 0;
                const int row = BN >= 64 ? nb * 64 + lane : (lane & 31);
                const int ks = ONE ? r8 >> 1 : r8 >> 2, r4 = ONE ? r8 & 1 : r8 & 3;
                const unsigned woff = (unsigned)((((long long)(2 * st + ks) * (ONE ? 2 : 4) + r4) * a.N + n0 + row) * 16);
                __builtin_amdgcn_raw_ptr_buffer_load_lds(rsw, (lds_ptr_t)(dst + q * 1024), 16, woff, 0, 0, 0);
            }
        }
    };

    f32x16 acc[TN];
#pragma unroll
    for (int j = 0; j < TN; ++j)
#pragma unroll
        for (int r = 0; r < 16; ++r) acc[j][r] = 0.f;

    issue_w(0);
#pragma unroll
    for (int d = 0; d < D - 1; ++d) load_x(d, d);
    asm volatile("s_waitcnt vmcnt(0)" ::: "memory");
    __syncthreads();
    for (int base = 0; base < stages; base += D) {
#pragma unroll
        for (int u = 0; u < D; ++u) {
            const int st = base + u;
            if (st + 1 < stages) issue_w(st + 1);
            load_x(st + D - 1, (u + D - 1) % D);
            const char* Bt = wbuf + (st & 1) * WST + khalf * (BN * 16) + (lane & 31) * 16;
            if (st < stages)
#pragma unroll
            for (int ks = 0; ks < 2; ++ks) {
                const f32x4 v0 = __builtin_bit_cast(f32x4, xr[u][ks][0]), v1 = __builtin_bit_cast(f32x4, xr[u][ks][1]);
                if constexpr (ONE) {
                    const u32x4 xh = u32x4{hi_pair(v0[0] * sa, v0[1] * sa), hi_pair(v0[2] * sa, v0[3] * sa), hi_pair(v1[0] * sa, v1[1] * sa),
                                           hi_pair(v1[2] * sa, v1[3] * sa)};
#pragma unroll
                    for (int j = 0; j < TN; ++j) {
                        const u32x4 wh = *reinterpret_cast<const u32x4*>(Bt + (ks * 2) * (BN * 16) + j * 512);
                        acc[j] = __builtin_amdgcn_mfma_f32_32x32x16_f16(__builtin_bit_cast(f16x8, xh), __builtin_bit_cast(f16x8, wh), acc[j], 0, 0, 0);
                    }
                    continue;
                }
                unsigned h0, l0, h1, l1, h2, l2, h3, l3;
                split_pair(v0[0] * sa, v0[1] * sa, h0, l0); split_pair(v0[2] * sa, v0[3] * sa, h1, l1);
                split_pair(v1[0] * sa, v1[1] * sa, h2, l2); split_pair(v1[2] * sa, v1[3] * sa, h3, l3);
                const u32x4 xh = u32x4{h0, h1, h2, h3}, xl = u32x4{l0, l1, l2, l3};
#pragma unroll
                for (int j = 0; j < TN; ++j) {
                    const u32x4 wh = *reinterpret_cast<const u32x4*>(Bt + ((ks * 2 + 0) * 2) * (BN * 16) + j * 512);
                    const u32x4 wl = *reinterpret_cast<const u32x4*>(Bt + ((ks * 2 + 1) * 2) * (BN * 16) + j * 512);
                    acc[j] = __builtin_amdgcn_mfma_f32_32x32x16_f16(__builtin_bit_cast(f16x8, xl), __builtin_bit_cast(f16x8, wh), acc[j], 0, 0, 0);
                    acc[j] = __builtin_amdgcn_mfma_f32_32x32x16_f16(__builtin_bit_cast(f16x8, xh), __builtin_bit_cast(f16x8, wl), acc[j], 0, 0, 0);
                    acc[j] = __builtin_amdgcn_mfma_f32_32x32x16_f16(__builtin_bit_cast(f16x8, xh), __builtin_bit_cast(f16x8, wh), acc[j], 0, 0, 0);
                }
            }
            asm volatile("s_waitcnt vmcnt(4)" ::: "memory");
            __syncthreads();
        }
    }
    const long long mw = (long long)blockIdx.x * 128 + wave * 32;
    if constexpr (PSI) {
        float p[16];
#pragma unroll
        for (int r = 0; r < 16; ++r) p[r] = 0.f;
#pragma unroll
        for (int j = 0; j < TN; ++j) {
            const int n = j * 32 + (lane & 31);
            const float sc = o.scale[n], sh = o.shift[n], wp = a.wpsi[blockIdx.z][n];
#pragma unroll
            for (int r = 0; r < 16; ++r) {
                float v = ldexpf(acc[j][r], einv) * sc + sh;
                if (a.relu) v = fmaxf(v, 0.f);
                p[r] = fmaf(v, wp, p[r]);
            }
        }
        float p8[8], p4[4], p2[2];
        {
            const bool up = lane & 16;
#pragma unroll
            for (int i = 0; i < 8; ++i) p8[i] = (up ? p[8 + i] : p[i]) + __shfl_xor(up ? p[i] : p[8 + i], 16);
        }
        {
            const bool up = lane & 8;
#pragma unroll
// ... 673 lines not shown
                    const long long base = (((long long)q * (N >> 4) + (n >> 4)) * 4 + tap) * 2 + ((n >> 3) & 1);
                    dst[(base * C + c) * 8 + (n & 7)] = __builtin_bit_cast(unsigned short, (_Float16)ws);
                    continue;
                }
                const _Float16 l = (_Float16)(float)(ws - (double)(float)h);
                const long long base = (((long long)q * (N >> 4) + (n >> 4)) * 4 + tap) * 4 + ((n >> 3) & 1);
                dst[((base + 0) * C + c) * 8 + (n & 7)] = __builtin_bit_cast(unsigned short, h);
                dst[((base + 2) * C + c) * 8 + (n & 7)] = __builtin_bit_cast(unsigned short, l);
            }
    }
    if (!dst) block_amax(mx, wamax, 1u);
}

struct PrepackDesc { const float* w; unsigned short* planes; unsigned short* planes_t; unsigned* wamax; int N, C, kind, pad; };
__global__ __launch_bounds__(256) void prepack_amax_kernel(const PrepackDesc* __restrict__ descs) {
    const PrepackDesc d = descs[blockIdx.y];
    float mx = 0.f;
    if (d.kind == 2) {
        const long long NC = (long long)d.N * d.C;
        for (long long i = (long long)blockIdx.x * blockDim.x + threadIdx.x; i < NC; i += (long long)gridDim.x * blockDim.x) {
            double v[9];
#pragma unroll
            for (int k = 0; k < 9; ++k) v[k] = (double)d.w[i * 9 + k];
#pragma unroll
            for (int ph = 0; ph < 4; ++ph)
#pragma unroll
                for (int tap = 0; tap < 4; ++tap) mx = fmaxf(mx, fabsf((float)upconv_combined(v, ph, tap >> 1, tap & 1)));
        }
    } else {
        const long long total = (long long)d.N * d.C * (d.kind == 0 ? 9 : 1);
        for (long long i = (long long)blockIdx.x * blockDim.x + threadIdx.x; i < total; i += (long long)gridDim.x * blockDim.x)
            mx = fmaxf(mx, fabsf(d.w[i]));
    }
    __shared__ float part[4];
#pragma unroll
    for (int o = 32; o; o >>= 1) mx = fmaxf(mx, __shfl_xor(mx, o));
    if ((threadIdx.x & 63) == 0) part[threadIdx.x >> 6] = mx;
    __syncthreads();
    if (threadIdx.x == 0) atomicMax(d.wamax, __float_as_uint(fmaxf(fmaxf(part[0], part[1]), fmaxf(part[2], part[3]))));
}
template <bool ONE = false>
__device__ __forceinline__ void prepack_store_block(const PrepackDesc& d, const unsigned (&hl)[8][8], int n8, int c8, int slot_f, int slot_t,
                                                    int slots) {
    const int N = d.N, C = d.C, n0 = n8 * 8, c0 = c8 * 8;
    if constexpr (ONE) {
        const long long bf = ((long long)(c0 >> 4) * slots + slot_f) * 2 + ((c0 >> 3) & 1);
        uint4* hf = (uint4*)(d.planes + (bf * N + n0) * 8);
#pragma unroll
        for (int nn = 0; nn < 8; ++nn)
            hf[nn] = uint4{(hl[nn][0] & 0xffffu) | (hl[nn][1] << 16), (hl[nn][2] & 0xffffu) | (hl[nn][3] << 16),
                           (hl[nn][4] & 0xffffu) | (hl[nn][5] << 16), (hl[nn][6] & 0xffffu) | (hl[nn][7] << 16)};
        if (slot_t >= 0) {
            const long long bt = ((long long)(n0 >> 4) * slots + slot_t) * 2 + ((n0 >> 3) & 1);
            uint4* ht = (uint4*)(d.planes_t + (bt * C + c0) * 8);
#pragma unroll
            for (int cc = 0; cc < 8; ++cc)
                ht[cc] = uint4{(hl[0][cc] & 0xffffu) | (hl[1][cc] << 16), (hl[2][cc] & 0xffffu) | (hl[3][cc] << 16),
                               (hl[4][cc] & 0xffffu) | (hl[5][cc] << 16), (hl[6][cc] & 0xffffu) | (hl[7][cc] << 16)};
        }
        return;
    }
    {
        const long long base = ((long long)(c0 >> 4) * slots + slot_f) * 4 + ((c0 >> 3) & 1);
        uint4* hi = (uint4*)(d.planes + ((base + 0) * N + n0) * 8);
        uint4* lo = (uint4*)(d.planes + ((base + 2) * N + n0) * 8);
#pragma unroll
        for (int nn = 0; nn < 8; ++nn) {
            uint4 h, l;
            h.x = (hl[nn][0] & 0xffffu) | (hl[nn][1] << 16); h.y = (hl[nn][2] & 0xffffu) | (hl[nn][3] << 16);
            h.z = (hl[nn][4] & 0xffffu) | (hl[nn][5] << 16); h.w = (hl[nn][6] & 0xffffu) | (hl[nn][7] << 16);
            l.x = (hl[nn][0] >> 16) | (hl[nn][1] & 0xffff0000u); l.y = (hl[nn][2] >> 16) | (hl[nn][3] & 0xffff0000u);
            l.z = (hl[nn][4] >> 16) | (hl[nn][5] & 0xffff0000u); l.w = (hl[nn][6] >> 16) | (hl[nn][7] & 0xffff0000u);
            hi[nn] = h; lo[nn] = l;
        }
    }
    if (slot_t >= 0) {
        const long long base = ((long long)(n0 >> 4) * slots + slot_t) * 4 + ((n0 >> 3) & 1);
        uint4* hi = (uint4*)(d.planes_t + ((base + 0) * C + c0) * 8);
        uint4* lo = (uint4*)(d.planes_t + ((base + 2) * C + c0) * 8);
#pragma unroll
        for (int cc = 0; cc < 8; ++cc) {
            uint4 h, l;
            h.x = (hl[0][cc] & 0xffffu) | (hl[1][cc] << 16); h.y = (hl[2][cc] & 0xffffu) | (hl[3][cc] << 16);
            h.z = (hl[4][cc] & 0xffffu) | (hl[5][cc] << 16); h.w = (hl[6][cc] & 0xffffu) | (hl[7][cc] << 16);
            l.x = (hl[0][cc] >> 16) | (hl[1][cc] & 0xffff0000u); l.y = (hl[2][cc] >> 16) | (hl[3][cc] & 0xffff0000u);
            l.z = (hl[4][cc] >> 16) | (hl[5][cc] & 0xffff0000u); l.w = (hl[6][cc] >> 16) | (hl[7][cc] & 0xffff0000u);
            hi[cc] = h; lo[cc] = l;
        }
    }
}
template <bool ONE = false>
__global__ __launch_bounds__(256) void prepack_pack_kernel(const PrepackDesc* __restrict__ descs) {
    const PrepackDesc d = descs[blockIdx.y];
    const int N = d.N, C = d.C, N8 = N >> 3, C8 = C >> 3;
    const float swf = pow2f(SPLIT_EXP - amax_exponent(*d.wamax));
    if (d.kind == 2) {
        const double sw = (double)swf;
        const long long total = (long long)N8 * C8 * 16;
        for (long long i = (long long)blockIdx.x * blockDim.x + threadIdx.x; i < total; i += (long long)gridDim.x * blockDim.x) {
            const int pt = (int)(i & 15), ph = pt >> 2, tap = pt & 3;
            const long long t = i >> 4;
            const int c8 = (int)(t % C8), n8 = (int)(t / C8);
            const int py = ph >> 1, px = ph & 1, r = tap >> 1, tt = tap & 1;
            const int y_lo = py == 0 ? (r == 0 ? 0 : 1) : (r == 0 ? 0 : 2), y_hi = py == 0 ? (r == 0 ? 0 : 2) : (r == 0 ? 1 : 2);
            const int x_lo = px == 0 ? (tt == 0 ? 0 : 1) : (tt == 0 ? 0 : 2), x_hi = px == 0 ? (tt == 0 ? 0 : 2) : (tt == 0 ? 1 : 2);
            unsigned hl[8][8];
#pragma unroll
            for (int nn = 0; nn < 8; ++nn)
#pragma unroll
                for (int cc = 0; cc < 8; ++cc) {
                    const float* w9 = d.w + ((long long)(n8 * 8 + nn) * C + c8 * 8 + cc) * 9;
                    double acc = 0.0;
                    for (int y = y_lo; y <= y_hi; ++y)
                        for (int x = x_lo; x <= x_hi; ++x) acc += (double)w9[y * 3 + x];
                    const double ws = acc * sw;
                    const _Float16 h = ONE ? (_Float16)ws : (_Float16)(float)ws;
                    const _Float16 l = (_Float16)(float)(ws - (double)(float)h);
                    hl[nn][cc] = (unsigned)__builtin_bit_cast(unsigned short, h) | ((unsigned)__builtin_bit_cast(unsigned short, l) << 16);
                }
            PrepackDesc e = d;
            constexpr int NPL = ONE ? 1 : 2;
            e.planes = d.planes + (long long)ph * (C >> 4) * 4 * 2 * NPL * N * 8;
            if (d.planes_t) e.planes_t = d.planes_t + (long long)ph * (N >> 4) * 4 * 2 * NPL * C * 8;
            prepack_store_block<ONE>(e, hl, n8, c8, tap, d.planes_t ? (1 - r) * 2 + (1 - tt) : -1, 4);
        }
        return;
    }
    const int taps = d.kind == 0 ? 9 : 1;
    const long long total = (long long)N8 * C8 * taps;
    for (long long i = (long long)blockIdx.x * blockDim.x + threadIdx.x; i < total; i += (long long)gridDim.x * blockDim.x) {
        const int tap = (int)(i % taps);
        const long long t = i / taps;
        const int c8 = (int)(t % C8), n8 = (int)(t / C8);
        unsigned hl[8][8];
#pragma unroll
        for (int nn = 0; nn < 8; ++nn)
#pragma unroll
            for (int cc = 0; cc < 8; ++cc) {
                unsigned h, l;
                split_pair(d.w[((long long)(n8 * 8 + nn) * C + c8 * 8 + cc) * taps + tap] * swf, 0.f, h, l);
                hl[nn][cc] = (h & 0xffffu) | (l << 16);
            }
        prepack_store_block<ONE>(d, hl, n8, c8, tap, d.planes_t ? taps - 1 - tap : -1, taps);
    }
}

int split_tile_width(int H, int W, int N, int ksize) {
    if (ksize != 3 || H < 16 || H % 16) return 0;
    if (W >= 32 && W % 32 == 0 && N % 64 == 0) return 32;
    if (W >= 16 && W % 16 == 0 && N % 128 == 0) return 16;
    return 0;
}

template <int TW, int TM, int TN, bool PH, bool BS = false, bool P2 = false, bool DG = false, bool ONE = false>
int launch_h2(const SplitArgs& a, hipStream_t st, int tile) {
    {
        char nm[96];
        snprintf(nm, sizeof(nm), "conv3x3_halo_h2_kernel<%s, %d, %d, %d, %s, %s, %s, %s>", ONE ? "true" : "false", TW, TM, TN, PH ? "true" : "false",
                 BS ? "true" : "false", P2 ? "true" : "false", DG ? "true" : "false");
        nbp_note_kernel_symbol(tile, nm);
    }
    constexpr int TH = 4 * TM * (32 / TW);
    constexpr int HPIX = (TH + 2) * (TW + 2), RS = (HPIX + 7) / 8 * 8 * 16 + 64, NB = TN / 2;
    constexpr int NPL = ONE ? 1 : 2;
    constexpr size_t smem = 2 * NPL * (size_t)RS + 2 * (size_t)(PH ? 4 : 6) * NPL * NB * 1024 * (P2 ? 2 : 1) + (PH ? 0 : (HPIX * 4 + 15) / 16 * 16);
    static bool attr_set = false;
    if (!attr_set) {
        hipError_t e = hipFuncSetAttribute(reinterpret_cast<const void*>(&conv3x3_halo_h2_kernel<ONE, TW, TM, TN, PH, BS, P2, DG>),
                                           hipFuncAttributeMaxDynamicSharedMemorySize, (int)smem);
        if (e != hipSuccess) return (int)e;
        attr_set = true;
    }
    constexpr bool PHO = PH && !DG;
    dim3 grid((unsigned)(a.M / (PHO ? 4 : 1) / (TH * TW)), (unsigned)(a.N / (TN * 32)), (unsigned)(a.split_k * a.groups * (PHO ? (P2 ? 2 : 4) : 1)));
    conv3x3_halo_h2_kernel<ONE, TW, TM, TN, PH, BS, P2, DG><<<grid, 256, smem, st>>>(a);
    return nbp_launch_status();
}
template <int TW, int TM, int TN, bool PH, bool BS = false, bool P2 = false, bool DG = false>
int launch_h2o(const SplitArgs& a, hipStream_t st, int tile, int one) {
    return one ? launch_h2<TW, TM, TN, PH, BS, P2, DG, true>(a, st, tile) : launch_h2<TW, TM, TN, PH, BS, P2, DG, false>(a, st, tile);
}

}

static int chain_bounded_split(int sk, int cc, int taps, long long M, int N, int groups) {
    static const int max_k = nbp_tune_int("NBP_SPLIT_MAX_K", NBP_SPLIT_MAX_K_DEFAULT);
    static const int max_k_small = nbp_tune_int("NBP_SPLIT_MAX_K_SMALL", NBP_SPLIT_MAX_K_SMALL_DEFAULT);
    const bool small = (double)M * N * groups * 4.0 <= 64.0 * 1048576.0;
    const int mk = small && max_k_small > 0 ? max_k_small : max_k;
    if (mk <= 0) return sk;
    const int max_chunks = mk / (16 * taps) > 1 ? mk / (16 * taps) : 1;
    const int need = (int)nbp_cdiv(cc, max_chunks);
    return need > sk ? need : sk;
}

static long long half_rows_below() {
    static const int v = nbp_tune_int("NBP_SPLIT_R8_BLOCKS", 256);
    return v;
}


static bool half_rows_for_tail(long long workgroups) {
    if (workgroups <= 512) return false;
    const long long rem = workgroups % 512;
    return rem > 0 && rem <= 160;
}

ConvPlan nbp_plan_conv_split(long long M, int N, int chunks_total, int split_k, int groups, int H, int W, int ksize, int ups) {
    ConvPlan p{0, 1, chunks_total};
    constexpr int min_blocks = 256;
    if (ups && !((H | W) & 1)) {
        const int twu = split_tile_width(H / 2, W / 2, N, ksize);
        if (twu) {
            const int cc = chunks_total / 9 * 2;
            const long long blocks = (M / 4 / (16 * twu)) * (N / (twu == 32 ? 64 : 128)) * groups * 4;
            const bool r8 = blocks < half_rows_below();
            int sk = split_k;
            if (sk <= 0) {
                sk = 1;
                while (blocks * sk < min_blocks && cc / (sk * 2) >= 4 && sk < 16) sk *= 2;
            }
            if (split_k == 0) sk = chain_bounded_split(sk, cc, 4, M, N, groups);
            if (sk > cc) sk = cc;
            const int per = (int)nbp_cdiv(cc, sk);
            p.split_k = (int)nbp_cdiv(cc, per); p.chunks_per_split = per;
            const bool r8t = r8 || half_rows_for_tail((M / 4 / (16 * twu)) * (N / (twu == 32 ? 64 : 128)) * groups * 4 * p.split_k);
            p.tile = r8t ? NBP_TILE_SPLIT_UP_R8 : NBP_TILE_SPLIT_UP;
            return p;
        }
    }
    const int tw = split_tile_width(H, W, N, ksize);
    if (!tw) return p;
    const int cc = chunks_total / 9 * 2;
    const long long blocks = (M / (16 * tw)) * (N / (tw == 32 ? 64 : 128)) * groups;
    const bool r8 = blocks < half_rows_below();
    int sk = split_k;
    if (sk <= 0) {
        sk = 1;
        while (blocks * sk < min_blocks && cc / (sk * 2) >= 4 && sk < 16) sk *= 2;
        if (blocks * sk < 2 * min_blocks && cc / (sk * 2) >= 16 && sk < 16) sk *= 2;
        if (split_k == 0) sk = chain_bounded_split(sk, cc, 9, M, N, groups);
    }
    if (sk > cc) sk = cc;
    const int per = (int)nbp_cdiv(cc, sk);
    p.split_k = (int)nbp_cdiv(cc, per); p.chunks_per_split = per;
    const bool r8t = r8 || half_rows_for_tail((M / (16 * tw)) * (N / (tw == 32 ? 64 : 128)) * groups * p.split_k);
    p.tile = r8t ? NBP_TILE_SPLIT_HALO_R8 : (tw == 32 && N % 128 == 0) ? NBP_TILE_SPLIT_HALO_128 : NBP_TILE_SPLIT_HALO_64;
    return p;
}

int nbp_amax_launch(const float* x, long long n, unsigned* amax_inout, hipStream_t st) {
    if (n <= 0) return 0;
    amax_kernel<<<min(nbp_ew_grid(n / 4 + 1, 256), 1024), 256, 0, st>>>(x, n, nullptr, 1, amax_inout, AMAX_WORDS);
    return nbp_launch_status();
}

int nbp_conv_split_launch_g(const ConvOperandsSplit& o, const ConvOperandsSplit* o2, int C0, int C1, int ups, int B, int H, int W,
                            int ksize, int N, int relu, int split_k, void* ws, size_t ws_bytes, hipStream_t st,
                            float* const* pool_out, int* pooled, const ConvHead* head, int* headed, double* bn_part, int* bn_rows, int one) {
    const int groups = o2 ? 2 : 1;
    if (bn_rows) *bn_rows = 0;
    NBP_RETURN_IF(!o.src0 || !o.planes || !o.scale || !o.shift || !o.out || !o.amax0 || !o.wamax, NBP_E_ARG);
    NBP_RETURN_IF(o2 && (!o2->src0 || !o2->planes || !o2->scale || !o2->shift || !o2->out || !o2->amax0 || !o2->wamax), NBP_E_ARG);
    NBP_RETURN_IF(B < 1 || H < 1 || W < 1 || ksize != 3, NBP_E_ARG);
    NBP_RETURN_IF(C0 < 32 || C0 % 32 || C1 < 0 || C1 % 32 || N < 64 || N % 64, NBP_E_SHAPE);
    NBP_RETURN_IF(C1 > 0 && (!o.src1 || !o.amax1 || (o2 && (!o2->src1 || !o2->amax1))), NBP_E_ARG);
    NBP_RETURN_IF(ups && ((H | W) & 1), NBP_E_SHAPE);
    SplitArgs a;
    for (int g = 0; g < 2; ++g) {
        const ConvOperandsSplit& s = (g && o2) ? *o2 : o;
        a.g[g] = SplitOps{s.src0, s.src1, s.planes, s.scale, s.shift, s.out, s.amax0, C1 ? s.amax1 : nullptr, s.wamax, s.amax_out, nullptr, nullptr, {nullptr, nullptr}, nullptr, nullptr, s.psi0};
    }
    NBP_RETURN_IF((o.psi0 || (o2 && o2->psi0)) && ups, NBP_E_SHAPE);
    a.C0 = C0; a.C1 = C1; a.ups = ups ? 1 : 0;
    a.H = H; a.W = W; a.Hs = ups ? H / 2 : H; a.Ws = ups ? W / 2 : W;
    a.N = N; a.relu = relu; a.groups = groups;
    a.M = (long long)B * H * W;
    const long long b0 = (long long)B * a.Hs * a.Ws * C0 * 4, b1 = (long long)B * a.Hs * a.Ws * C1 * 4;
    const long long bw = (long long)(C0 + C1) * 9 * N * 4;
    NBP_RETURN_IF(b0 >= (1ll << 31) || b1 >= (1ll << 31) || bw >= (1ll << 31), NBP_E_SHAPE);
    a.bytes0 = (unsigned)b0; a.bytes1 = C1 ? (unsigned)b1 : (unsigned)b0; a.bytesw = (unsigned)bw;
    const bool have_up = ups && o.planes_up && o.wamax_up && (!o2 || (o2->planes_up && o2->wamax_up));
    const ConvPlan p = nbp_plan_conv_split(a.M, N, (C0 + C1) / 32 * 9, split_k, groups, H, W, ksize, have_up ? 1 : 0);
    NBP_RETURN_IF(p.tile != NBP_TILE_SPLIT_HALO_64 && p.tile != NBP_TILE_SPLIT_HALO_128 && p.tile != NBP_TILE_SPLIT_UP && p.tile != NBP_TILE_SPLIT_HALO_R8 &&
                  p.tile != NBP_TILE_SPLIT_UP_R8, NBP_E_SHAPE);
    const bool ph = p.tile == NBP_TILE_SPLIT_UP || p.tile == NBP_TILE_SPLIT_UP_R8;
    const bool r8 = p.tile == NBP_TILE_SPLIT_HALO_R8 || p.tile == NBP_TILE_SPLIT_UP_R8;
    const bool wide = p.tile == NBP_TILE_SPLIT_HALO_128;
    const int th = (r8 || wide) ? 8 : 16;
    a.split_k = p.split_k; a.chunks_per_split = p.chunks_per_split;
    a.chunks_total = (C0 + C1) / 16;
    const int tw = ph ? split_tile_width(H / 2, W / 2, N, ksize) : split_tile_width(H, W, N, ksize);
    if (ph) {
        NBP_RETURN_IF(C1 != 0, NBP_E_SHAPE);
        for (int g = 0; g < groups; ++g) {
            const ConvOperandsSplit& sg = (g && o2) ? *o2 : o;
            a.g[g].planes = sg.planes_up; a.g[g].wamax = sg.wamax_up;
        }
        const long long bwu = (long long)C0 * 16 * N * 4;
        NBP_RETURN_IF(bwu >= (1ll << 31), NBP_E_SHAPE);
        a.bytesw = (unsigned)bwu;
    }
    {
        const long long ptiles = a.M / (ph ? 4 : 1) / (th * tw), nbk = N / ((tw == 32 && !wide) ? 64 : 128);
        const long long tiles = ptiles * nbk;
        const double wb = (double)(C0 + C1) * (ph ? 16 : 9) * N * 4, ab = (double)a.M / (ups ? 4 : 1) * (C0 + C1) * 4;
        const bool fits2 = nbk >= 8 ? nbk % 8 == 0 : (8 % nbk == 0 && ptiles % (8 / nbk) == 0);
        const bool heavy = 7.0 * wb > ((nbk < 8 ? nbk : 8) - 1) * ab * 3.0;
        int mode = tiles >= 8 ? 1 : 0;
        if (fits2 && heavy && tiles >= 8) mode = 2;
        a.xcd_remap = mode;
    }
    a.partial = nullptr;
    if (p.split_k > 1) {
        NBP_RETURN_IF(!ws || ws_bytes < (size_t)groups * p.split_k * a.M * N * sizeof(float), NBP_E_WS);
        a.partial = (float*)ws;
    }
    static const int allow_pool = nbp_tune_int("NBP_CONV_POOL", 1);
    const bool with_pool = allow_pool && pool_out && pool_out[0] && (groups == 1 || pool_out[1]) && p.split_k == 1 && !ph && !ups &&
                           !((H | W) & 1);
    const bool pool_in_reduce = allow_pool && pool_out && pool_out[0] && groups == 1 && p.split_k > 1 && !ph && !ups && !((H | W) & 1);
    if (pooled) *pooled = with_pool || pool_in_reduce;
    if (with_pool || pool_in_reduce)
        for (int g = 0; g < groups; ++g) a.g[g].pool_out = pool_out[g];
    static const int allow_head = nbp_tune_int("NBP_CONV_HEAD", 1);
    const bool with_head = allow_head && head && head->w && head->scale && head->shift && head->out && groups == 1 && p.split_k == 1 &&
                           !ph && tw == 32 && N == 64 && relu;
    if (headed) *headed = with_head;
    if (with_head) { a.g[0].head_w = head->w; a.g[0].head_ss[0] = head->scale; a.g[0].head_ss[1] = head->shift; a.g[0].head_out = head->out; }
    if (bn_part && bn_rows && p.split_k == 1 && !r8 && groups == 1) {
        a.g[0].bn_part = bn_part;
        *bn_rows = (int)(a.M / (16 * tw));
        if (wide) {
            *bn_rows = (int)(a.M / 256);
            return launch_h2o<32, 2, 4, false, true>(a, st, p.tile, one);
        }
        return ph ? (tw == 32 ? launch_h2o<32, 2, 2, true, true, true>(a, st, p.tile, one) : launch_h2o<16, 2, 4, true, true>(a, st, p.tile, one))
                  : (tw == 32 ? launch_h2o<32, 4, 2, false, true>(a, st, p.tile, one) : launch_h2o<16, 2, 4, false, true>(a, st, p.tile, one));
    }
    int rc = (ph && !r8 && tw == 32) ? launch_h2o<32, 2, 2, true, false, true>(a, st, p.tile, one)
           : r8 ? (ph ? (tw == 32 ? launch_h2o<32, 2, 2, true>(a, st, p.tile, one) : launch_h2o<16, 1, 4, true>(a, st, p.tile, one))
                      : (tw == 32 ? launch_h2o<32, 2, 2, false>(a, st, p.tile, one) : launch_h2o<16, 1, 4, false>(a, st, p.tile, one)))
           : ph ? launch_h2o<16, 2, 4, true>(a, st, p.tile, one)
                : (tw == 32 ? (wide ? launch_h2o<32, 2, 4, false>(a, st, p.tile, one) : launch_h2o<32, 4, 2, false>(a, st, p.tile, one))
                            : launch_h2o<16, 2, 4, false>(a, st, p.tile, one));
    if (rc) return rc;
    if (p.split_k > 1) {
        const long long MN = a.M * N;
        NBP_RETURN_IF(MN >= (1ll << 31), NBP_E_SHAPE);
        dim3 grid((unsigned)min(nbp_cdiv(MN / 4, 256 * 4), 1024ll), (unsigned)groups);
        if (pool_in_reduce)
            splitk_reduce_pool_kernel<<<(unsigned)min(nbp_cdiv(MN / 16, 256), 1024ll), 256, 0, st>>>((const float*)ws, p.split_k, (unsigned)MN,
                                                                                                    (unsigned)N, H, W, a.g[0], relu);
        else
        splitk_reduce_split_kernel<<<grid, 256, 0, st>>>((const float*)ws, p.split_k, (unsigned)MN, (unsigned)N, a.g[0], a.g[1], relu);
        rc = nbp_launch_status();
    }
    return rc;
}

int nbp_pack_conv_weight_split_launch(const float* w_oihw, int N, int C, int ksize, const float* scale_or_null, int c_off,
                                      int c_total, void* dst, unsigned* wamax_out, hipStream_t st, int one) {
    NBP_RETURN_IF(!w_oihw || !dst || !wamax_out, NBP_E_ARG);
    NBP_RETURN_IF(ksize != 1 && ksize != 3, NBP_E_ARG);
    NBP_RETURN_IF(N < 1 || C < 1 || c_off != 0 || C > c_total || c_total % 32, NBP_E_SHAPE);
    const long long total = (long long)N * C * ksize * ksize;
    hipError_t e = hipMemsetAsync(wamax_out, 0, sizeof(unsigned), st);
    if (e != hipSuccess) return (int)e;
    amax_kernel<<<min(nbp_ew_grid(total, 256), 256), 256, 0, st>>>(w_oihw, total, scale_or_null, (long long)C * ksize * ksize, wamax_out, 1u);
    const int grid = nbp_ew_grid(total, 256);
    if (one) pack_conv_weight_h2_kernel<true><<<grid, 256, 0, st>>>(w_oihw, N, C, ksize * ksize, scale_or_null, c_off, wamax_out, (unsigned short*)dst);
    else pack_conv_weight_h2_kernel<<<grid, 256, 0, st>>>(w_oihw, N, C, ksize * ksize, scale_or_null, c_off, wamax_out, (unsigned short*)dst);
    return nbp_launch_status();
}

int nbp_pack_upconv_weight_split_launch(const float* w_oihw, int N, int C, void* dst, unsigned* wamax_out, hipStream_t st, int one) {
    NBP_RETURN_IF(!w_oihw || !dst || !wamax_out, NBP_E_ARG);
    NBP_RETURN_IF(N < 1 || C < 16 || C % 16, NBP_E_SHAPE);
    hipError_t e = hipMemsetAsync(wamax_out, 0, sizeof(unsigned), st);
    if (e != hipSuccess) return (int)e;
    const long long NC = (long long)N * C;
    const int grid = nbp_ew_grid(NC, 256);
    if (one) {
        pack_upconv_h2_kernel<true><<<min(grid, 256), 256, 0, st>>>(w_oihw, N, C, wamax_out, nullptr);
        pack_upconv_h2_kernel<true><<<grid, 256, 0, st>>>(w_oihw, N, C, wamax_out, (unsigned short*)dst);
    } else {
        pack_upconv_h2_kernel<<<min(grid, 256), 256, 0, st>>>(w_oihw, N, C, wamax_out, nullptr);
        pack_upconv_h2_kernel<<<grid, 256, 0, st>>>(w_oihw, N, C, wamax_out, (unsigned short*)dst);
    }
    return nbp_launch_status();
}

int nbp_pack_gate_weight_split_launch(const float* wg, const float* scale_g, const float* wx, const float* scale_x, int N, int C,
                                      void* dst, unsigned* wamax_out, hipStream_t st) {
    NBP_RETURN_IF(!wg || !wx || !dst || !wamax_out, NBP_E_ARG);
    NBP_RETURN_IF(N < 32 || N % 32 || C < 32 || C % 32, NBP_E_SHAPE);
    hipError_t e = hipMemsetAsync(wamax_out, 0, sizeof(unsigned), st);
    if (e != hipSuccess) return (int)e;
    const long long total = (long long)N * C;
    const int grid = min(nbp_ew_grid(total, 256), 256);
    amax_kernel<<<grid, 256, 0, st>>>(wg, total, scale_g, C, wamax_out, 1u);
    amax_kernel<<<grid, 256, 0, st>>>(wx, total, scale_x, C, wamax_out, 1u);
    pack_conv_weight_h2_kernel<<<nbp_ew_grid(total, 256), 256, 0, st>>>(wg, N, C, 1, scale_g, 0, wamax_out, (unsigned short*)dst);
    pack_conv_weight_h2_kernel<<<nbp_ew_grid(total, 256), 256, 0, st>>>(wx, N, C, 1, scale_x, C, wamax_out, (unsigned short*)dst);
    return nbp_launch_status();
}

int nbp_gate1x1_split_launch_g(const ConvOperandsSplit& o, const ConvOperandsSplit* o2, int C, long long M, int N, int relu,
                               hipStream_t st, const GatePsi* psi, int* fused) {
    const int groups = o2 ? 2 : 1;
    NBP_RETURN_IF(!o.src0 || !o.src1 || !o.planes || !o.scale || !o.shift || !o.out || !o.amax0 || !o.amax1 || !o.wamax, NBP_E_ARG);
    NBP_RETURN_IF(o2 && (!o2->src0 || !o2->src1 || !o2->planes || !o2->out || !o2->amax0 || !o2->amax1 || !o2->wamax), NBP_E_ARG);
    NBP_RETURN_IF(C < 64 || C % 64 || N < 32 || N % 32 || M < 1, NBP_E_SHAPE);
    const long long b0 = M * C * 4, bw = 2ll * C * N * 4;
    NBP_RETURN_IF(b0 >= (1ll << 31) || bw >= (1ll << 31), NBP_E_SHAPE);
    GateArgs a;
    for (int g = 0; g < 2; ++g) {
        const ConvOperandsSplit& s = (g && o2) ? *o2 : o;
        a.g[g] = SplitOps{s.src0, s.src1, s.planes, s.scale, s.shift, s.out, s.amax0, s.amax1, s.wamax, nullptr, nullptr, nullptr, {nullptr, nullptr}, nullptr};
        const int gi = g < groups ? g : 0;
        a.wpsi[g] = psi ? psi->wpsi[gi] : nullptr; a.st[g] = psi ? psi->st[gi] : nullptr; a.gated[g] = psi ? psi->gated[gi] : nullptr;
        a.gated_amax[g] = psi ? psi->gated_amax[gi] : nullptr;
    }
    a.psi_only = psi ? psi->psi_only : 0;
    a.C = C; a.C1 = C; a.N = N; a.relu = relu; a.M = M; a.bytes0 = (unsigned)b0; a.bytesw = (unsigned)bw; a.groups = groups;
    int bn = N % 128 == 0 ? 128 : (N % 64 == 0 ? 64 : 32);
    static const int allow_psi = nbp_tune_int("NBP_GATE_PSI", 1);
    const bool psi_wants_128 = allow_psi && psi && N == 128 && psi->wpsi[0] && psi->st[0] && psi->gated[0];
    if (bn == 128 && nbp_cdiv(M, 128) * (N / 128) * groups < 512 && !psi_wants_128) bn = 64;
    const bool with_psi = allow_psi && psi && bn == N && psi->wpsi[0] && psi->st[0] && psi->gated[0] &&
                          (groups == 1 || (psi->wpsi[1] && psi->st[1] && psi->gated[1]));
    if (fused) *fused = with_psi;
    dim3 grid((unsigned)nbp_cdiv(M, 128), (unsigned)(N / bn), (unsigned)groups);
    const size_t smem = 2 * (size_t)8 * bn * 16;
    {
        char nm[64];
        snprintf(nm, sizeof(nm), "gate1x1_h2_kernel<false, %d, %s>", bn / 32, with_psi ? "true" : "false");
        nbp_note_kernel_symbol(NBP_TILE_SPLIT_GATE, nm);
    }
    if (with_psi) {
        if (bn == 128) gate1x1_h2_kernel<false, 4, true><<<grid, 256, smem, st>>>(a);
        else if (bn == 64) gate1x1_h2_kernel<false, 2, true><<<grid, 256, smem, st>>>(a);
        else gate1x1_h2_kernel<false, 1, true><<<grid, 256, smem, st>>>(a);
    } else if (bn == 128) gate1x1_h2_kernel<false, 4, false><<<grid, 256, smem, st>>>(a);
    else if (bn == 64) gate1x1_h2_kernel<false, 2, false><<<grid, 256, smem, st>>>(a);
    else gate1x1_h2_kernel<false, 1, false><<<grid, 256, smem, st>>>(a);
    return nbp_launch_status();
}

int nbp_upconv_dgrad_split_launch(const float* dy, int N, int B, int H, int W, const void* planes, const unsigned* wamax,
                                  const unsigned* amax_in, int C, const float* scale, const float* shift, float* out, unsigned* amax_out,
                                  int split_k, void* ws, size_t ws_bytes, hipStream_t st, int one = 0) {
    NBP_RETURN_IF(!dy || !planes || !wamax || !amax_in || !scale || !shift || !out, NBP_E_ARG);
    NBP_RETURN_IF(B < 1 || N < 16 || N % 16 || C < 64 || C % 64, NBP_E_SHAPE);
    const int tw = split_tile_width(H, W, C, 3);
    NBP_RETURN_IF(!tw, NBP_E_SHAPE);
    SplitArgs a;
    for (int g = 0; g < 2; ++g)
        a.g[g] = SplitOps{dy, nullptr, planes, scale, shift, out, amax_in, nullptr, wamax, amax_out, nullptr, nullptr, {nullptr, nullptr}, nullptr, nullptr};
    a.C0 = N; a.C1 = 0; a.ups = 0; a.H = H; a.W = W; a.Hs = 2 * H; a.Ws = 2 * W; a.N = C; a.relu = 0; a.groups = 1;
    a.M = (long long)B * H * W;
    const long long b0 = (long long)B * 4 * H * W * N * 4, bw = 64ll * N * C;
    NBP_RETURN_IF(b0 >= (1ll << 31) || bw >= (1ll << 31), NBP_E_SHAPE);
    a.bytes0 = (unsigned)b0; a.bytes1 = (unsigned)b0; a.bytesw = (unsigned)bw;
    a.chunks_total = 4 * (N / 16);
    const long long blocks = (a.M / ((tw == 32 ? 8 : 16) * tw)) * (C / (tw == 32 ? 64 : 128));
    int sk = split_k;
    if (sk <= 0) { sk = 1; while (blocks * sk < 256 && a.chunks_total / (sk * 2) >= 4 && sk < 16) sk *= 2; }
    if (sk > a.chunks_total) sk = a.chunks_total;
    a.chunks_per_split = (int)nbp_cdiv(a.chunks_total, sk);
    a.split_k = (int)nbp_cdiv(a.chunks_total, a.chunks_per_split);
    a.xcd_remap = blocks >= 8 ? 1 : 0;
    a.partial = nullptr;
    if (a.split_k > 1) {
        NBP_RETURN_IF(!ws || ws_bytes < (size_t)a.split_k * a.M * C * sizeof(float), NBP_E_WS);
        a.partial = (float*)ws;
    }
    int rc = tw == 32 ? launch_h2o<32, 2, 2, true, false, false, true>(a, st, NBP_TILE_SPLIT_UP_DGRAD, one)
                      : launch_h2o<16, 2, 4, true, false, false, true>(a, st, NBP_TILE_SPLIT_UP_DGRAD, one);
    if (rc) return rc;
    if (a.split_k > 1) {
        const long long MN = a.M * C;
        NBP_RETURN_IF(MN >= (1ll << 31), NBP_E_SHAPE);
        dim3 grid((unsigned)min(nbp_cdiv(MN / 4, 256 * 4), 1024ll), 1u);
        splitk_reduce_split_kernel<<<grid, 256, 0, st>>>((const float*)ws, a.split_k, (unsigned)MN, (unsigned)C, a.g[0], a.g[1], 0);
        rc = nbp_launch_status();
    }
    return rc;
}

int nbp_conv1x1_split_launch(const float* src, int C, long long M, const void* planes, const unsigned* wamax, const unsigned* amax_in,
// ... 32 lines not shown
    if (e != hipSuccess) return (int)e;
    int rc = amax0_in ? 0 : nbp_amax_launch(src0, b0 / 4, amax3, st);
    if (!rc && C1 && !amax1_in) rc = nbp_amax_launch(src1, b1 / 4, amax3 + AMAX_WORDS, st);
    if (!rc && !amaxy_in) rc = nbp_amax_launch(dy, by / 4, amax3 + 2 * AMAX_WORDS, st);
    if (rc) return rc;
    WgradSplitArgs a;
    a.src0 = src0; a.src1 = src1 ? src1 : src0; a.C0 = C0; a.C1 = C1; a.ups = ups ? 1 : 0; a.H = H; a.W = W; a.Hs = Hs; a.Ws = Ws;
    a.dy = dy; a.N = N; a.bytes0 = (unsigned)b0; a.bytes1 = C1 ? (unsigned)b1 : (unsigned)b0; a.bytesy = (unsigned)by;
    a.co_tiles = N / 64; a.n_tiles = n_tiles; a.splits = splits;
    a.amax0 = amax0_in ? amax0_in : amax3; a.amax1 = amax1_in ? amax1_in : amax3 + AMAX_WORDS;
    a.amaxy = amaxy_in ? amaxy_in : amax3 + 2 * AMAX_WORDS; a.part = part;
    const bool wide = W % 32 == 0 && H % 2 == 0;
    const int smem = (one ? 2 : 4) * ((wide ? 4 * 34 * 64 : 6 * 18 * 64) + 64 * 64);
    dim3 grid((unsigned)(((C0 + C1) / 64) * (N / 64)), (unsigned)splits);
    if (one) {
        if (wide) wgrad_split_kernel<32, true><<<grid, 256, smem, st>>>(a);
        else wgrad_split_kernel<16, true><<<grid, 256, smem, st>>>(a);
        return nbp_launch_status();
    }
    static bool attr_set = false;
    if (!attr_set) {
        e = hipFuncSetAttribute(reinterpret_cast<const void*>(&wgrad_split_kernel<32>), hipFuncAttributeMaxDynamicSharedMemorySize,
                                4 * (4 * 34 * 64) + 4 * (64 * 64));

        if (e == hipSuccess)
            e = hipFuncSetAttribute(reinterpret_cast<const void*>(&wgrad_split_kernel<16>), hipFuncAttributeMaxDynamicSharedMemorySize,
                                    4 * (6 * 18 * 64) + 4 * (64 * 64));
        if (e != hipSuccess) return (int)e;
        attr_set = true;
    }
    if (wide) wgrad_split_kernel<32><<<grid, 256, smem, st>>>(a);
    else wgrad_split_kernel<16><<<grid, 256, smem, st>>>(a);
    return nbp_launch_status();
}

extern "C" int nbp_pack_conv_weight_split(const float* w_oihw, int N, int C, int ksize, const float* scale_or_null,
                                          int c_off, int c_total, void* dst_planes, void* wamax_out, void* stream) {
    NBP_ENTER();
    return nbp_pack_conv_weight_split_launch(w_oihw, N, C, ksize, scale_or_null, c_off, c_total, dst_planes, (unsigned*)wamax_out,
                                             (hipStream_t)stream);
}
extern "C" int nbp_pack_conv_weight_split_h1(const float* w_oihw, int N, int C, int ksize, const float* scale_or_null,
                                             int c_off, int c_total, void* dst_planes, void* wamax_out, void* stream) {
    NBP_ENTER();
    return nbp_pack_conv_weight_split_launch(w_oihw, N, C, ksize, scale_or_null, c_off, c_total, dst_planes, (unsigned*)wamax_out,
                                             (hipStream_t)stream, 1);
}

template <bool ONE>
static int pack_conv_weight_split_dgrad_impl(const float* w_oihw, int N, int C, int c_total, void* dst_planes, void* wamax_out,
                                             void* stream) {
    NBP_RETURN_IF(!w_oihw || !dst_planes || !wamax_out, NBP_E_ARG);
    NBP_RETURN_IF(N < 1 || C < 1 || N > c_total || c_total % 32, NBP_E_SHAPE);
    hipStream_t st = (hipStream_t)stream;
    const long long total = (long long)N * C * 9;
    hipError_t e = hipMemsetAsync(wamax_out, 0, sizeof(unsigned), st);
    if (e != hipSuccess) return (int)e;
    amax_kernel<<<min(nbp_ew_grid(total, 256), 256), 256, 0, st>>>(w_oihw, total, nullptr, 9ll * C, (unsigned*)wamax_out, 1u);
    pack_conv_weight_h2_kernel<ONE><<<nbp_ew_grid(total, 256), 256, 0, st>>>(w_oihw, C, N, 9, nullptr, 0, (const unsigned*)wamax_out,
                                                                            (unsigned short*)dst_planes, 1);
    return nbp_launch_status();
}
extern "C" int nbp_pack_conv_weight_split_dgrad(const float* w_oihw, int N, int C, int c_total, void* dst_planes, void* wamax_out,
                                                void* stream) {
    NBP_ENTER();
    return pack_conv_weight_split_dgrad_impl<false>(w_oihw, N, C, c_total, dst_planes, wamax_out, stream);
}
extern "C" int nbp_pack_conv_weight_split_dgrad_h1(const float* w_oihw, int N, int C, int c_total, void* dst_planes, void* wamax_out,
                                                   void* stream) {
    NBP_ENTER();
    return pack_conv_weight_split_dgrad_impl<true>(w_oihw, N, C, c_total, dst_planes, wamax_out, stream);
}

template <bool ONE>
static int prepack_weights_split_impl(const void* descs_dev, int n, void* wamax_words, void* stream) {
    NBP_RETURN_IF(!descs_dev || !wamax_words || n < 1 || n > 4096, NBP_E_ARG);
    hipStream_t st = (hipStream_t)stream;
    hipError_t e = hipMemsetAsync(wamax_words, 0, (size_t)n * sizeof(unsigned), st);
    if (e != hipSuccess) return (int)e;
    prepack_amax_kernel<<<dim3(64, (unsigned)n), 256, 0, st>>>((const PrepackDesc*)descs_dev);
    prepack_pack_kernel<ONE><<<dim3(256, (unsigned)n), 256, 0, st>>>((const PrepackDesc*)descs_dev);
    return nbp_launch_status();
}
extern "C" int nbp_prepack_weights_split(const void* descs_dev, int n, void* wamax_words, void* stream) {
    NBP_ENTER();
    return prepack_weights_split_impl<false>(descs_dev, n, wamax_words, stream);
}
extern "C" int nbp_prepack_weights_split_h1(const void* descs_dev, int n, void* wamax_words, void* stream) {
    NBP_ENTER();
    return prepack_weights_split_impl<true>(descs_dev, n, wamax_words, stream);
}
extern "C" int nbp_prepack_desc_bytes(void) { return (int)sizeof(PrepackDesc); }

template <bool ONE>
static int pack_conv_weight_split_prezeroed_impl(const float* w_oihw, int N, int C, int ksize, int c_total, void* dst_planes,
                                                 void* wamax_zeroed, void* stream) {
    NBP_RETURN_IF(!w_oihw || !dst_planes || !wamax_zeroed, NBP_E_ARG);
    NBP_RETURN_IF((ksize != 1 && ksize != 3) || N < 1 || C < 1 || C > c_total || c_total % 32, NBP_E_SHAPE);
    hipStream_t st = (hipStream_t)stream;
    const long long total = (long long)N * C * ksize * ksize;
    amax_kernel<<<min(nbp_ew_grid(total, 256), 256), 256, 0, st>>>(w_oihw, total, nullptr, (long long)C * ksize * ksize, (unsigned*)wamax_zeroed, 1u);
    pack_conv_weight_h2_kernel<ONE><<<nbp_ew_grid(total, 256), 256, 0, st>>>(w_oihw, N, C, ksize * ksize, nullptr, 0, (const unsigned*)wamax_zeroed,
                                                                            (unsigned short*)dst_planes);
    return nbp_launch_status();
}
template <bool ONE>
static int pack_conv_weight_split_dgrad_known_impl(const float* w_oihw, int N, int C, int c_total, void* dst_planes,
                                                   const void* wamax_known, void* stream) {
    NBP_RETURN_IF(!w_oihw || !dst_planes || !wamax_known, NBP_E_ARG);
    NBP_RETURN_IF(N < 1 || C < 1 || N > c_total || c_total % 32, NBP_E_SHAPE);
    const long long total = (long long)N * C * 9;
    pack_conv_weight_h2_kernel<ONE><<<nbp_ew_grid(total, 256), 256, 0, (hipStream_t)stream>>>(w_oihw, C, N, 9, nullptr, 0, (const unsigned*)wamax_known,
                                                                                             (unsigned short*)dst_planes, 1);
    return nbp_launch_status();
}
extern "C" int nbp_pack_conv_weight_split_prezeroed(const float* w_oihw, int N, int C, int ksize, int c_total, void* dst_planes,
                                                    void* wamax_zeroed, void* stream) {
    NBP_ENTER();
    return pack_conv_weight_split_prezeroed_impl<false>(w_oihw, N, C, ksize, c_total, dst_planes, wamax_zeroed, stream);
}
extern "C" int nbp_pack_conv_weight_split_dgrad_known(const float* w_oihw, int N, int C, int c_total, void* dst_planes,
                                                      const void* wamax_known, void* stream) {
    NBP_ENTER();
    return pack_conv_weight_split_dgrad_known_impl<false>(w_oihw, N, C, c_total, dst_planes, wamax_known, stream);
}
extern "C" int nbp_pack_conv_weight_split_prezeroed_h1(const float* w_oihw, int N, int C, int ksize, int c_total, void* dst_planes,
                                                       void* wamax_zeroed, void* stream) {
    NBP_ENTER();
    return pack_conv_weight_split_prezeroed_impl<true>(w_oihw, N, C, ksize, c_total, dst_planes, wamax_zeroed, stream);
}
extern "C" int nbp_pack_conv_weight_split_dgrad_known_h1(const float* w_oihw, int N, int C, int c_total, void* dst_planes,
                                                         const void* wamax_known, void* stream) {
    NBP_ENTER();
    return pack_conv_weight_split_dgrad_known_impl<true>(w_oihw, N, C, c_total, dst_planes, wamax_known, stream);
}
extern "C" int nbp_amax_f32(const float* x, long long n, void* amax_inout, void* stream) {
    NBP_ENTER();
    NBP_RETURN_IF(!x || !amax_inout || n < 0, NBP_E_ARG);
    return nbp_amax_launch(x, n, (unsigned*)amax_inout, (hipStream_t)stream);
}

extern "C" size_t nbp_conv_split_workspace_bytes(int B, int H, int W, int N, int split_k) {
    const int sk = split_k == 1 ? 0 : (split_k <= 0 ? 16 : split_k);
    return 256 + (size_t)sk * B * H * W * N * sizeof(float);
}

extern "C" size_t nbp_conv_split_planned_workspace_bytes_k(int B, int H, int W, int C, int N, int ups, int split_k, int* split_k_out);
extern "C" size_t nbp_conv_split_planned_workspace_bytes(int B, int H, int W, int C, int N, int ups, int* split_k_out) {
    return nbp_conv_split_planned_workspace_bytes_k(B, H, W, C, N, ups, 0, split_k_out);
}
extern "C" size_t nbp_conv_split_planned_workspace_bytes_k(int B, int H, int W, int C, int N, int ups, int split_k, int* split_k_out) {
    if (B < 1 || H < 1 || W < 1 || C < 32 || N < 1) return 0;
    const ConvPlan p = nbp_plan_conv_split((long long)B * H * W, N, C / 32 * 9, split_k, 1, H, W, 3, ups ? 1 : 0);
    if (split_k_out) *split_k_out = p.tile ? p.split_k : 0;
    const int sk = (p.tile && p.split_k > 1) ? p.split_k : 0;
    return 256 + (size_t)sk * B * H * W * N * sizeof(float);
}

static int conv3x3_split_impl(const float* src0, int C0, const float* src1, int C1, int ups, int B, int H, int W,
                              const void* w_planes, const void* wamax, int N, const float* scale, const float* shift,
                              int relu, float* out, const void* amax_in_or_null, void* amax_out_or_null, int split_k,
                              void* ws, size_t ws_bytes, void* stream, double* bn_part, int* bn_rows, int one = 0) {
    NBP_RETURN_IF(!ws || ws_bytes < 256 || !src0, NBP_E_WS);
    hipStream_t st = (hipStream_t)stream;
    const unsigned* amax = (const unsigned*)amax_in_or_null;
    if (!amax) {
        unsigned* slot = (unsigned*)ws;
        hipError_t e = hipMemsetAsync(slot, 0, 256, st);
        if (e != hipSuccess) return (int)e;
        const long long hw = (long long)B * (ups ? H / 2 : H) * (ups ? W / 2 : W);
        int rc = nbp_amax_launch(src0, hw * C0, slot, st);
        if (!rc && C1 > 0) { NBP_RETURN_IF(!src1, NBP_E_ARG); rc = nbp_amax_launch(src1, hw * C1, slot, st); }
        if (rc) return rc;
        amax = slot;
    }
    ConvOperandsSplit o{src0, src1, w_planes, scale, shift, out, amax, amax, (const unsigned*)wamax, (unsigned*)amax_out_or_null,
                        nullptr, nullptr};
    return nbp_conv_split_launch_g(o, nullptr, C0, C1, ups, B, H, W, 3, N, relu, split_k, (char*)ws + 256, ws_bytes - 256, st, nullptr,
                                   nullptr, nullptr, nullptr, bn_part, bn_rows, one);
}
extern "C" int nbp_conv3x3_split_f32(const float* src0, int C0, const float* src1, int C1, int ups, int B, int H, int W,
                                     const void* w_planes, const void* wamax, int N, const float* scale, const float* shift,
                                     int relu, float* out, const void* amax_in_or_null, void* amax_out_or_null, int split_k,
                                     void* ws, size_t ws_bytes, void* stream) {
    NBP_ENTER();
    return conv3x3_split_impl(src0, C0, src1, C1, ups, B, H, W, w_planes, wamax, N, scale, shift, relu, out, amax_in_or_null,
                              amax_out_or_null, split_k, ws, ws_bytes, stream, nullptr, nullptr);
}
extern "C" int nbp_conv_bn_part_rows(int B, int H, int W) { return (int)((long long)B * H * W / 256); }
extern "C" int nbp_conv3x3_split_bn_f32(const float* src0, int C0, const float* src1, int C1, int ups, int B, int H, int W,
                                        const void* w_planes, const void* wamax, int N, const float* scale, const float* shift,
                                        int relu, float* out, const void* amax_in_or_null, void* amax_out_or_null, int split_k,
                                        void* ws, size_t ws_bytes, double* bn_part, int* bn_rows, void* stream) {
    NBP_ENTER();
    NBP_RETURN_IF(!bn_part || !bn_rows || ((uintptr_t)bn_part & 7), NBP_E_ARG);
    return conv3x3_split_impl(src0, C0, src1, C1, ups, B, H, W, w_planes, wamax, N, scale, shift, relu, out, amax_in_or_null,
                              amax_out_or_null, split_k, ws, ws_bytes, stream, bn_part, bn_rows);
}
extern "C" int nbp_conv3x3_split_f32_h1(const float* src0, int C0, const float* src1, int C1, int ups, int B, int H, int W,
                                        const void* w_planes, const void* wamax, int N, const float* scale, const float* shift,
                                        int relu, float* out, const void* amax_in_or_null, void* amax_out_or_null, int split_k,
                                        void* ws, size_t ws_bytes, void* stream) {
    NBP_ENTER();
    return conv3x3_split_impl(src0, C0, src1, C1, ups, B, H, W, w_planes, wamax, N, scale, shift, relu, out, amax_in_or_null,
                              amax_out_or_null, split_k, ws, ws_bytes, stream, nullptr, nullptr, 1);
}
extern "C" int nbp_conv3x3_split_bn_f32_h1(const float* src0, int C0, const float* src1, int C1, int ups, int B, int H, int W,
                                           const void* w_planes, const void* wamax, int N, const float* scale, const float* shift,
                                           int relu, float* out, const void* amax_in_or_null, void* amax_out_or_null, int split_k,
                                           void* ws, size_t ws_bytes, double* bn_part, int* bn_rows, void* stream) {
    NBP_ENTER();
    NBP_RETURN_IF(!bn_part || !bn_rows || ((uintptr_t)bn_part & 7), NBP_E_ARG);
    return conv3x3_split_impl(src0, C0, src1, C1, ups, B, H, W, w_planes, wamax, N, scale, shift, relu, out, amax_in_or_null,
                              amax_out_or_null, split_k, ws, ws_bytes, stream, bn_part, bn_rows, 1);
}

static void wgrad_up_plan(int B, int Hs, int Ws, int C, int N, int* n_tiles, int* splits) {
    *n_tiles = (int)((long long)B * Hs * Ws / 64);
    const long long pairs = (long long)(C / 64) * (N / 64) * 4;
    long long sp = nbp_cdiv(768, pairs);
    if (sp > *n_tiles) sp = *n_tiles;
    if (sp > 1024) sp = 1024;
    if (sp < 1) sp = 1;
    *splits = (int)sp;
}
static bool wgrad_up_ok(int Hs, int Ws, int C, int N) {
    return C >= 64 && C % 64 == 0 && N >= 64 && N % 64 == 0 && ((Ws % 32 == 0 && Hs % 2 == 0) || (Ws % 16 == 0 && Hs % 4 == 0));
}
extern "C" size_t nbp_upconv_wgrad_split_workspace_bytes(int B, int Hs, int Ws, int C, int N) {
    if (B < 1 || !wgrad_up_ok(Hs, Ws, C, N)) return 0;
    int nt, sp;
    wgrad_up_plan(B, Hs, Ws, C, N, &nt, &sp);
    return 1024 + (size_t)sp * 16 * C * N * sizeof(float);
}
static int upconv_wgrad_split_impl(const float* x, int C, int B, int Hs, int Ws, const float* dy, int N, float* dw,
                                   const void* amax_x, const void* amax_y, void* ws, size_t ws_bytes, void* stream, int one) {
    NBP_RETURN_IF(!x || !dy || !dw || !amax_x || !amax_y || !ws || B < 1, NBP_E_ARG);
    NBP_RETURN_IF(!wgrad_up_ok(Hs, Ws, C, N), NBP_E_SHAPE);
    const long long b0 = (long long)B * Hs * Ws * C * 4, by = (long long)B * 4 * Hs * Ws * N * 4;
    NBP_RETURN_IF(b0 >= (1ll << 31) || by >= (1ll << 31), NBP_E_SHAPE);
    int n_tiles, splits;
    wgrad_up_plan(B, Hs, Ws, C, N, &n_tiles, &splits);
    NBP_RETURN_IF(ws_bytes < 1024 + (size_t)splits * 16 * C * N * sizeof(float), NBP_E_WS);
    hipStream_t st = (hipStream_t)stream;
    WgradSplitArgs a;
    a.src0 = x; a.src1 = x; a.C0 = C; a.C1 = 0; a.ups = 1; a.H = 2 * Hs; a.W = 2 * Ws; a.Hs = Hs; a.Ws = Ws;
    a.dy = dy; a.N = N; a.bytes0 = (unsigned)b0; a.bytes1 = (unsigned)b0; a.bytesy = (unsigned)by;
    a.co_tiles = N / 64; a.n_tiles = n_tiles; a.splits = splits;
    a.amax0 = (const unsigned*)amax_x; a.amax1 = a.amax0; a.amaxy = (const unsigned*)amax_y;
    a.part = (float*)((char*)(((uintptr_t)ws + 255) / 256 * 256));
    const bool wide = Ws % 32 == 0 && Hs % 2 == 0;
    constexpr int smem32 = 4 * (3 * 34 * 64) + 4 * (64 * 64), smem16 = 4 * (5 * 18 * 64) + 4 * (64 * 64);
    static bool attr_set = false;
    if (!attr_set) {
        hipError_t e = hipFuncSetAttribute(reinterpret_cast<const void*>(&wgrad_up_split_kernel<32>), hipFuncAttributeMaxDynamicSharedMemorySize, smem32);
        if (e == hipSuccess)
            e = hipFuncSetAttribute(reinterpret_cast<const void*>(&wgrad_up_split_kernel<16>), hipFuncAttributeMaxDynamicSharedMemorySize, smem16);
        if (e != hipSuccess) return (int)e;
        attr_set = true;
    }
    dim3 grid((unsigned)((C / 64) * (N / 64)), (unsigned)splits, 4u);
    if (one) {
        if (wide) wgrad_up_split_kernel<32, true><<<grid, 256, smem32 / 2, st>>>(a);
        else wgrad_up_split_kernel<16, true><<<grid, 256, smem16 / 2, st>>>(a);
    } else if (wide) wgrad_up_split_kernel<32><<<grid, 256, smem32, st>>>(a);
    else wgrad_up_split_kernel<16><<<grid, 256, smem16, st>>>(a);
    int rc = nbp_launch_status();
    if (rc) return rc;
    wgrad_up_reduce_kernel<<<nbp_ew_grid((long long)N * C * 9, 256), 256, 0, st>>>(a.part, splits, C, N, dw);
    return nbp_launch_status();
}
extern "C" int nbp_upconv_wgrad_split_f32(const float* x, int C, int B, int Hs, int Ws, const float* dy, int N, float* dw,
                                          const void* amax_x, const void* amax_y, void* ws, size_t ws_bytes, void* stream) {
    NBP_ENTER();
    return upconv_wgrad_split_impl(x, C, B, Hs, Ws, dy, N, dw, amax_x, amax_y, ws, ws_bytes, stream, 0);
}
extern "C" int nbp_upconv_wgrad_split_f32_h1(const float* x, int C, int B, int Hs, int Ws, const float* dy, int N, float* dw,
                                             const void* amax_x, const void* amax_y, void* ws, size_t ws_bytes, void* stream) {
    NBP_ENTER();
    return upconv_wgrad_split_impl(x, C, B, Hs, Ws, dy, N, dw, amax_x, amax_y, ws, ws_bytes, stream, 1);
}

int nbp_wgrad_1x1_split_launch(const float* x, int C, long long M, const float* dy, int N, int n_tiles, int splits, const unsigned* amax_x,
                               const unsigned* amax_y, float* part, hipStream_t st, int one) {
    NBP_RETURN_IF(M * C * 4 >= (1ll << 31) || M * N * 4 >= (1ll << 31), NBP_E_SHAPE);
    WgradSplitArgs a;
    NBP_RETURN_IF(M % 64 != 0, NBP_E_SHAPE);
    a.src0 = x; a.src1 = x; a.C0 = C; a.C1 = 0; a.ups = 0; a.H = (int)(M / 64); a.W = 64; a.Hs = a.H; a.Ws = a.W;
    a.dy = dy; a.N = N; a.bytes0 = (unsigned)(M * C * 4); a.bytes1 = a.bytes0; a.bytesy = (unsigned)(M * N * 4);
    a.co_tiles = (N + 63) / 64; a.n_tiles = n_tiles; a.splits = splits;
    a.amax0 = amax_x; a.amax1 = amax_x; a.amaxy = amax_y; a.part = part;
    dim3 grid((unsigned)((C / 64) * a.co_tiles), (unsigned)splits);
    if (one) wgrad_1x1_split_kernel<true><<<grid, 256, 4 * 64 * 64, st>>>(a);
    else wgrad_1x1_split_kernel<<<grid, 256, 8 * 64 * 64, st>>>(a);
    return nbp_launch_status();
}

template <bool ONE>
static int pack_upconv_weight_split_dgrad_impl(const float* w_oihw, int N, int C, void* dst_planes, void* wamax_out, void* stream) {
    NBP_RETURN_IF(!w_oihw || !dst_planes || !wamax_out, NBP_E_ARG);
    NBP_RETURN_IF(N < 16 || N % 16 || C < 1, NBP_E_SHAPE);
    hipStream_t st = (hipStream_t)stream;
    hipError_t e = hipMemsetAsync(wamax_out, 0, sizeof(unsigned), st);
    if (e != hipSuccess) return (int)e;
    const long long NC = (long long)N * C;
    pack_upconv_dgrad_h2_kernel<ONE><<<min(nbp_ew_grid(NC, 256), 256), 256, 0, st>>>(w_oihw, N, C, (unsigned*)wamax_out, nullptr);
    pack_upconv_dgrad_h2_kernel<ONE><<<nbp_ew_grid(NC, 256), 256, 0, st>>>(w_oihw, N, C, (unsigned*)wamax_out, (unsigned short*)dst_planes);
    return nbp_launch_status();
}
extern "C" int nbp_pack_upconv_weight_split_dgrad(const float* w_oihw, int N, int C, void* dst_planes, void* wamax_out, void* stream) {
    NBP_ENTER();
    return pack_upconv_weight_split_dgrad_impl<false>(w_oihw, N, C, dst_planes, wamax_out, stream);
}
extern "C" size_t nbp_upconv_split_dgrad_workspace_bytes(int B, int H, int W, int N, int C) {
    if (B < 1 || H < 1 || W < 1 || N < 16 || C < 64) return 0;
    const int tw = split_tile_width(H, W, C, 3);
    if (!tw) return 0;
    const long long M = (long long)B * H * W, blocks = (M / ((tw == 32 ? 8 : 16) * tw)) * (C / (tw == 32 ? 64 : 128));
    const int chunks = 4 * (N / 16);
    int sk = 1;
    while (blocks * sk < 256 && chunks / (sk * 2) >= 4 && sk < 16) sk *= 2;
    return 256 + (sk > 1 ? (size_t)sk * M * C * sizeof(float) : 0);
}
extern "C" int nbp_upconv3x3_split_dgrad_f32(const float* dy, int N, int B, int H, int W, const void* planes, const void* wamax, int C,
                                             const float* scale, const float* shift, float* dx, const void* amax_in, void* amax_out_or_null,
                                             void* ws, size_t ws_bytes, void* stream) {
    NBP_ENTER();
    return nbp_upconv_dgrad_split_launch(dy, N, B, H, W, planes, (const unsigned*)wamax, (const unsigned*)amax_in, C, scale, shift, dx,
                                         (unsigned*)amax_out_or_null, 0, ws ? (char*)ws + 256 : nullptr, ws_bytes >= 256 ? ws_bytes - 256 : 0,
                                         (hipStream_t)stream);
}
extern "C" int nbp_upconv3x3_split_dgrad_f32_h1(const float* dy, int N, int B, int H, int W, const void* planes, const void* wamax, int C,
// ... 115 lines not shown
```

Baseline: 2319.

## Run split-K slices serially inside one workgroup when occupancy is already sufficient

When the planner would split K only to bound chain length, and the grid already has enough workgroups, the conv kernel now processes all K slices in one workgroup. It stores each intermediate slice's accumulators to a per-block scratch area, then sums them in the epilogue, in place of launching split-K slices with a separate reduction. This aims to remove the extra reduction pass and the extra partial-buffer round trip. The cost is more serial work per workgroup plus scratch writes and reads. The change also adds a grouped conv entry point and a plan query API.

```diff
diff --git a/include/nbp_hip.h b/include/nbp_hip.h
--- a/include/nbp_hip.h
+++ b/include/nbp_hip.h
@@ -84,6 +84,12 @@
                           const void* w_planes, const void* wamax, int N, const float* scale, const float* shift, int relu,
                           float* out, const void* amax_in_or_null, void* amax_out_or_null, int split_k, void* ws,
                           size_t ws_bytes, void* stream);
+int nbp_conv_split_plan(int B, int H, int W, int C, int N, int ups, int groups, int split_k, int* split_k_out, int* chain_slices_out);
+int nbp_conv3x3_split_groups_f32(const float* const* src0, int C0, const float* const* src1, int C1, const float* const* psi0,
+                                 int ups, int B, int H, int W, const void* const* w_planes, const void* const* wamax, int N,
+                                 const float* const* scale, const float* const* shift, int relu, float* const* out,
+                                 const void* const* amax_in, void* const* amax_out, float* const* pool_out, int* pooled_out,
+                                 int groups, int split_k, void* ws, size_t ws_bytes, void* stream);
 size_t nbp_conv_first_wgrad_workspace_bytes(void);
 int nbp_conv_first_wgrad_f32(const float* x_nchw, int B, int H, int W, const float* dy, float* dw, void* ws, size_t ws_bytes, void* stream);
 int nbp_prepack_weights_split(const void* descs_dev, int n, void* wamax_words, void* stream);
diff --git a/nextbestpath_amd/_lib.py b/nextbestpath_amd/_lib.py
--- a/nextbestpath_amd/_lib.py
+++ b/nextbestpath_amd/_lib.py
@@ -128,6 +128,9 @@
 SIGNATURES["nbp_conv_split_planned_workspace_bytes_k"] = (_sz, [_i, _i, _i, _i, _i, _i, _i, _vp])
 SIGNATURES["nbp_conv3x3_split_f32"] = (_i, [_vp, _i, _vp, _i, _i, _i, _i, _i, _vp, _vp, _i, _vp, _vp, _i, _vp, _vp, _vp, _i, _vp,
                                             _sz, _vp])
+SIGNATURES["nbp_conv_split_plan"] = (_i, [_i, _i, _i, _i, _i, _i, _i, _i, C.POINTER(_i), C.POINTER(_i)])
+SIGNATURES["nbp_conv3x3_split_groups_f32"] = (_i, [_vp, _i, _vp, _i, _vp, _i, _i, _i, _i, _vp, _vp, _i, _vp, _vp, _i, _vp, _vp, _vp, _vp,
+                                                   C.POINTER(_i), _i, _i, _vp, _sz, _vp])
 SIGNATURES["nbp_pack_upconv_weight_split_dgrad"] = (_i, [_vp, _i, _i, _vp, _vp, _vp])
 SIGNATURES["nbp_upconv_split_dgrad_workspace_bytes"] = (_sz, [_i, _i, _i, _i, _i])
 SIGNATURES["nbp_upconv3x3_split_dgrad_f32"] = (_i, [_vp, _i, _i, _i, _i, _vp, _vp, _i, _vp, _vp, _vp, _vp, _vp, _vp, _sz, _vp])
diff --git a/nextbestpath_amd/csrc/nbp_forward.hip b/nextbestpath_amd/csrc/nbp_forward.hip
--- a/nextbestpath_amd/csrc/nbp_forward.hip
+++ b/nextbestpath_amd/csrc/nbp_forward.hip
@@ -543,7 +543,7 @@
 template <typename P>
 size_t splitk_scratch_floats(long long M, int N, int cin_total, int taps, int groups, int H, int ups = 0) {
     ConvPlan p = P::plan(M, N, cin_total / P::CHUNK * taps, groups, H, taps == 9 ? 3 : 1, ups);
-    return p.split_k > 1 ? (size_t)groups * p.split_k * M * N : 0;
+    return p.split_k > 1 ? (size_t)groups * p.split_k * M * N : p.chain_slices > 1 ? (size_t)groups * (p.chain_slices - 1) * M * N : 0;
 }
 
 template <typename P>
@@ -590,7 +590,7 @@
             const long long M = (long long)B * Hh * Hh;
             const int K = (C0 + C1) * ksize * ksize;
             ConvPlan p = P::plan(M, N, K / P::CHUNK, ng, Hh, ksize, ups);
-            tm->mark(name, 2.0 * ng * M * N * K, p.tile, p.split_k, M, N, K);
+            tm->mark(name, 2.0 * ng * M * N * K, p.tile, p.split_k * p.chain_slices, M, N, K);
         }
     };
     auto conv = [&](const char* name, int li, const T* s0, int C0, const T* s1, int C1, int ups, int Hh,
diff --git a/nextbestpath_amd/csrc/nbp_internal.h b/nextbestpath_amd/csrc/nbp_internal.h
--- a/nextbestpath_amd/csrc/nbp_internal.h
+++ b/nextbestpath_amd/csrc/nbp_internal.h
@@ -15,7 +15,7 @@
        NBP_TILE_SPLIT_HALO_128 = 18,
        NBP_TILE_SPLIT_GATE = 19 };
 struct TileInfo { int bm, bn; };
-struct ConvPlan { int tile; int split_k; int chunks_per_split; };
+struct ConvPlan { int tile; int split_k; int chunks_per_split; int chain_slices = 1; };
 
 struct IgemmArgs {
     const float* src0;
@@ -60,7 +60,8 @@
     const void* planes_up; const unsigned* wamax_up;
     const float* psi0 = nullptr;
 };
-ConvPlan nbp_plan_conv_split(long long M, int N, int chunks_total, int split_k, int groups, int H, int W, int ksize, int ups = 0);
+ConvPlan nbp_plan_conv_split(long long M, int N, int chunks_total, int split_k, int groups, int H, int W, int ksize, int ups = 0,
+                             int serial_ok = 1);
 int nbp_pack_upconv_weight_split_launch(const float* w_oihw, int N, int C, void* dst, unsigned* wamax_out, hipStream_t st, int one = 0);
 struct ConvHead { const float* w; const float* scale; const float* shift; float* out; };
 int nbp_conv_split_launch_g(const ConvOperandsSplit& o, const ConvOperandsSplit* o2, int C0, int C1, int ups, int B, int H, int W,
diff --git a/nextbestpath_amd/csrc/nbp_split.hip b/nextbestpath_amd/csrc/nbp_split.hip
--- a/nextbestpath_amd/csrc/nbp_split.hip
+++ b/nextbestpath_amd/csrc/nbp_split.hip
@@ -39,6 +39,16 @@
 #pragma unroll
     for (int o = 32; o; o >>= 1) mx = fmaxf(mx, __shfl_xor(mx, o));
     if ((threadIdx.x & 63) == 0)
+        atomicMax(out + ((blockIdx.x * 4u + (threadIdx.x >> 6) + blockIdx.y * 17u + blockIdx.z * 29u) & (AMAX_WORDS - 1)), __float_as_uint(mx));
+}
+__device__ __forceinline__ void wave_amax_late(float mx, unsigned* out) {
+    unsigned z = 0;
+    asm volatile("" : "+v"(z));
+    const unsigned self = __builtin_amdgcn_mbcnt_hi(~0u, __builtin_amdgcn_mbcnt_lo(~0u, z));
+#pragma unroll
+    for (unsigned o = 32; o; o >>= 1)
+        mx = fmaxf(mx, __int_as_float(__builtin_amdgcn_ds_bpermute((int)((self ^ o) << 2), __float_as_int(mx))));
+    if (self == 0)
         atomicMax(out + ((blockIdx.x * 4u + (threadIdx.x >> 6) + blockIdx.y * 17u + blockIdx.z * 29u) & (AMAX_WORDS - 1)), __float_as_uint(mx));
 }
 __device__ __forceinline__ void block_amax(float mx, unsigned* out, unsigned words = AMAX_WORDS) {
@@ -73,6 +83,7 @@
     unsigned bytes0, bytes1, bytesw;
     float* partial;
     int groups, xcd_remap;
+    int chain_slices;
 };
 
 #ifdef NBP_DBG_TS
@@ -83,10 +94,11 @@
 #else
 #define NBP_TS(tag) do {} while (0)
 #endif
-template <bool ONE, int TW, int TM, int TN, bool PH, bool BS = false, bool P2 = false, bool DG = false>
+template <bool ONE, bool SER, int TW, int TM, int TN, bool PH, bool BS = false, bool P2 = false, bool DG = false>
 __global__ __launch_bounds__(256, 2) __attribute__((amdgpu_waves_per_eu(2, 2))) void conv3x3_halo_h2_kernel(SplitArgs a) {
     static_assert(!P2 || PH, "two-parity form: up_conv layers");
     static_assert(!DG || (PH && !BS && !P2), "data gradient of an up_conv layer: the one-parity tap structure");
+    static_assert(!SER || (!ONE && !BS && !DG), "serial chains: planned for the eval forward only");
     constexpr bool PHO = PH && !DG;
     int zs = blockIdx.z;
     const int py = PHO ? (P2 ? zs & 1 : (zs >> 1) & 1) : 0, px = (PHO && !P2) ? zs & 1 : 0;
@@ -259,7 +271,11 @@
     const int brow = khalf * NB * 1024 + (lane & 31) * 16;
 
     const int c_begin = zs * a.chunks_per_split;
-    const int c_end = min(c_begin + a.chunks_per_split, a.chunks_total);
+    const int c_end = min(c_begin + a.chunks_per_split * (SER ? a.chain_slices : 1), a.chunks_total);
+    f32x4* const chain_ws = SER ? reinterpret_cast<f32x4*>(a.partial) + ((long long)(blockIdx.x + gridDim.x * (blockIdx.y + gridDim.y * blockIdx.z)) *
+                                                                         (a.chain_slices - 1) * (NPAR * TM * TN * 4)) * 256
+                                : nullptr;
+    int chain_left = a.chunks_per_split, chain_done = 0;
     if (c_begin < c_end) {
         load_halo(c_begin);
         issue_w(c_begin * ROWS);
@@ -376,6 +392,26 @@
             __syncthreads();
             NBP_TS(4);
         }
+        if constexpr (SER) {
+            if (--chain_left == 0 && more) {
+                f32x4* dst = chain_ws + (long long)chain_done * (NPAR * TM * TN * 4) * 256;
+#pragma unroll
+                for (int pq = 0; pq < NPAR; ++pq)
+#pragma unroll
+                    for (int j = 0; j < TN; ++j)
+#pragma unroll
+                        for (int i = 0; i < TM; ++i)
+#pragma unroll
+                            for (int q = 0; q < 4; ++q) {
+                                f32x16& ac = accs[pq][i][j];
+                                dst[(((pq * TN + j) * TM + i) * 4 + q) * 256 + tid] = f32x4{ldexpf(ac[4 * q], einv), ldexpf(ac[4 * q + 1], einv),
+                                                                                      ldexpf(ac[4 * q + 2], einv), ldexpf(ac[4 * q + 3], einv)};
+                                ac[4 * q] = 0.f; ac[4 * q + 1] = 0.f; ac[4 * q + 2] = 0.f; ac[4 * q + 3] = 0.f;
+                            }
+                ++chain_done;
+                chain_left = a.chunks_per_split;
+            }
+        }
         if (more) {
             __builtin_amdgcn_s_setprio(0);
             store_halo(c + 1);
@@ -386,8 +422,9 @@
         }
     }
 
-    const bool final_out = (a.split_k == 1);
+    const bool final_out = SER || (a.split_k == 1);
     float* outp = final_out ? o.out : a.partial + (long long)zslice * a.M * a.N;
+    if constexpr (SER) asm volatile("s_waitcnt vmcnt(0)" ::: "memory");
     float mx = 0.f;
     constexpr bool HEADABLE = !PH && TN == 2;
     const bool head = HEADABLE && final_out && o.head_out;
@@ -416,13 +453,38 @@
         float vals[TM][16];
 #pragma unroll
         for (int i = 0; i < TM; ++i) {
+            f32x4 tot[SER ? 4 : 1];
+            if constexpr (SER) {
+                const f32x4* ps = chain_ws + (((pq * TN + j) * TM + i) * 4) * 256;
+                constexpr long long CS = (long long)(NPAR * TM * TN * 4) * 256;
+                const int nst = a.chain_slices - 1;
+                constexpr int INF = 2;
+                f32x4 t[INF][4];
+#pragma unroll
+                for (int s = 0; s < INF; ++s)
+#pragma unroll
+                    for (int q = 0; q < 4; ++q) t[s][q] = s < nst ? ps[s * CS + q * 256 + tid] : f32x4{0.f, 0.f, 0.f, 0.f};
+#pragma unroll
+                for (int q = 0; q < 4; ++q) tot[q] = t[0][q];
+#pragma unroll
+                for (int s = 1; s < INF; ++s)
+                    if (s < nst) {
+#pragma unroll
+                        for (int q = 0; q < 4; ++q) tot[q] += t[s][q];
+                    }
+                for (int s = INF; s < nst; ++s)
+#pragma unroll
+                    for (int q = 0; q < 4; ++q) tot[q] += ps[s * CS + q * 256 + tid];
+            }
             const long long mrow = PHO ? ((long long)b * a.H + 2 * (y0 + (TM * wave + i) * RPB) + py) * a.W + 2 * x0 + pxe
                                        : ((long long)b * a.H + y0 + (TM * wave + i) * RPB) * a.W + x0;
 #pragma unroll
             for (int r = 0; r < 16; ++r) {
                 const int pb = (r & 3) + 8 * (r >> 2) + 4 * khalf;
                 const int poff = PHO ? 2 * ((pb / TW) * a.W + (pb % TW)) : (pb / TW) * a.W + (pb % TW);
-                float v = ldexpf(accs[pq][i][j][r], einv) * sc + sh;
+                float v;
+                if constexpr (SER) v = (tot[r >> 2][r & 3] + ldexpf(accs[pq][i][j][r], einv)) * sc + sh;
+                else v = ldexpf(accs[pq][i][j][r], einv) * sc + sh;
                 if (final_out && a.relu) v = fmaxf(v, 0.f);
                 mx = fmaxf(mx, fabsf(v));
                 if (!head) outp[(mrow + poff) * a.N + n] = v;
@@ -512,7 +574,8 @@
             }
         }
     }
-    if (final_out && o.amax_out) wave_amax(mx, o.amax_out);
+    if constexpr (SER) { if (o.amax_out) wave_amax_late(mx, o.amax_out); }
+    else if (final_out && o.amax_out) wave_amax(mx, o.amax_out);
 #ifdef NBP_DBG_TS
     NBP_TS(7);
     NBP_TS(102); NBP_WALL(103);
@@ -1492,12 +1555,12 @@
     return 0;
 }
 
-template <int TW, int TM, int TN, bool PH, bool BS = false, bool P2 = false, bool DG = false, bool ONE = false>
+template <int TW, int TM, int TN, bool PH, bool BS = false, bool P2 = false, bool DG = false, bool ONE = false, bool SER = false>
 int launch_h2(const SplitArgs& a, hipStream_t st, int tile) {
     {
         char nm[96];
-        snprintf(nm, sizeof(nm), "conv3x3_halo_h2_kernel<%s, %d, %d, %d, %s, %s, %s, %s>", ONE ? "true" : "false", TW, TM, TN, PH ? "true" : "false",
-                 BS ? "true" : "false", P2 ? "true" : "false", DG ? "true" : "false");
+        snprintf(nm, sizeof(nm), "conv3x3_halo_h2_kernel<%s, %s, %d, %d, %d, %s, %s, %s, %s>", ONE ? "true" : "false", SER ? "true" : "false", TW, TM, TN,
+                 PH ? "true" : "false", BS ? "true" : "false", P2 ? "true" : "false", DG ? "true" : "false");
         nbp_note_kernel_symbol(tile, nm);
     }
     constexpr int TH = 4 * TM * (32 / TW);
@@ -1506,15 +1569,19 @@
     constexpr size_t smem = 2 * NPL * (size_t)RS + 2 * (size_t)(PH ? 4 : 6) * NPL * NB * 1024 * (P2 ? 2 : 1) + (PH ? 0 : (HPIX * 4 + 15) / 16 * 16);
     static bool attr_set = false;
     if (!attr_set) {
-        hipError_t e = hipFuncSetAttribute(reinterpret_cast<const void*>(&conv3x3_halo_h2_kernel<ONE, TW, TM, TN, PH, BS, P2, DG>),
+        hipError_t e = hipFuncSetAttribute(reinterpret_cast<const void*>(&conv3x3_halo_h2_kernel<ONE, SER, TW, TM, TN, PH, BS, P2, DG>),
                                            hipFuncAttributeMaxDynamicSharedMemorySize, (int)smem);
         if (e != hipSuccess) return (int)e;
         attr_set = true;
     }
     constexpr bool PHO = PH && !DG;
     dim3 grid((unsigned)(a.M / (PHO ? 4 : 1) / (TH * TW)), (unsigned)(a.N / (TN * 32)), (unsigned)(a.split_k * a.groups * (PHO ? (P2 ? 2 : 4) : 1)));
-    conv3x3_halo_h2_kernel<ONE, TW, TM, TN, PH, BS, P2, DG><<<grid, 256, smem, st>>>(a);
+    conv3x3_halo_h2_kernel<ONE, SER, TW, TM, TN, PH, BS, P2, DG><<<grid, 256, smem, st>>>(a);
     return nbp_launch_status();
+}
+template <int TW, int TM, int TN, bool PH, bool P2 = false>
+int launch_h2s(const SplitArgs& a, hipStream_t st, int tile) {
+    return launch_h2<TW, TM, TN, PH, false, P2, false, false, true>(a, st, tile);
 }
 template <int TW, int TM, int TN, bool PH, bool BS = false, bool P2 = false, bool DG = false>
 int launch_h2o(const SplitArgs& a, hipStream_t st, int tile, int one) {
@@ -1523,6 +1590,13 @@
 
 }
 
+#define NBP_SPLIT_SERIAL_SLICES_DEFAULT 1
+#define NBP_SPLIT_SERIAL_MIN_WG_DEFAULT 512
+static bool serial_slices_for(long long workgroups) {
+    static const int on = nbp_tune_int("NBP_SPLIT_SERIAL_SLICES", NBP_SPLIT_SERIAL_SLICES_DEFAULT);
+    static const int min_wg = nbp_tune_int("NBP_SPLIT_SERIAL_MIN_WG", NBP_SPLIT_SERIAL_MIN_WG_DEFAULT);
+    return on != 0 && workgroups >= min_wg;
+}
 static int chain_bounded_split(int sk, int cc, int taps, long long M, int N, int groups) {
     static const int max_k = nbp_tune_int("NBP_SPLIT_MAX_K", NBP_SPLIT_MAX_K_DEFAULT);
     static const int max_k_small = nbp_tune_int("NBP_SPLIT_MAX_K_SMALL", NBP_SPLIT_MAX_K_SMALL_DEFAULT);
@@ -1546,7 +1620,8 @@
     return rem > 0 && rem <= 160;
 }
 
-ConvPlan nbp_plan_conv_split(long long M, int N, int chunks_total, int split_k, int groups, int H, int W, int ksize, int ups) {
+ConvPlan nbp_plan_conv_split(long long M, int N, int chunks_total, int split_k, int groups, int H, int W, int ksize, int ups,
+                             int serial_ok) {
     ConvPlan p{0, 1, chunks_total};
     constexpr int min_blocks = 256;
     if (ups && !((H | W) & 1)) {
@@ -1560,10 +1635,16 @@
                 sk = 1;
                 while (blocks * sk < min_blocks && cc / (sk * 2) >= 4 && sk < 16) sk *= 2;
             }
+            const int sk_occ = sk;
             if (split_k == 0) sk = chain_bounded_split(sk, cc, 4, M, N, groups);
             if (sk > cc) sk = cc;
             const int per = (int)nbp_cdiv(cc, sk);
             p.split_k = (int)nbp_cdiv(cc, per); p.chunks_per_split = per;
+            if (serial_ok && twu == 16 && split_k == 0 && sk_occ == 1 && p.split_k > 1 && !r8 && !half_rows_for_tail(blocks) && serial_slices_for(blocks)) {
+                p.chain_slices = p.split_k; p.split_k = 1;
+                p.tile = NBP_TILE_SPLIT_UP;
+                return p;
+            }
             const bool r8t = r8 || half_rows_for_tail((M / 4 / (16 * twu)) * (N / (twu == 32 ? 64 : 128)) * groups * 4 * p.split_k);
             p.tile = r8t ? NBP_TILE_SPLIT_UP_R8 : NBP_TILE_SPLIT_UP;
             return p;
@@ -1574,16 +1655,22 @@
     const int cc = chunks_total / 9 * 2;
     const long long blocks = (M / (16 * tw)) * (N / (tw == 32 ? 64 : 128)) * groups;
     const bool r8 = blocks < half_rows_below();
-    int sk = split_k;
+    int sk = split_k, sk_occ = 0;
     if (sk <= 0) {
         sk = 1;
         while (blocks * sk < min_blocks && cc / (sk * 2) >= 4 && sk < 16) sk *= 2;
         if (blocks * sk < 2 * min_blocks && cc / (sk * 2) >= 16 && sk < 16) sk *= 2;
+        sk_occ = sk;
         if (split_k == 0) sk = chain_bounded_split(sk, cc, 9, M, N, groups);
     }
     if (sk > cc) sk = cc;
     const int per = (int)nbp_cdiv(cc, sk);
     p.split_k = (int)nbp_cdiv(cc, per); p.chunks_per_split = per;
+    if (serial_ok && split_k == 0 && sk_occ == 1 && p.split_k > 1 && !r8 && !half_rows_for_tail(blocks) && serial_slices_for(blocks)) {
+        p.chain_slices = p.split_k; p.split_k = 1;
+        p.tile = (tw == 32 && N % 128 == 0) ? NBP_TILE_SPLIT_HALO_128 : NBP_TILE_SPLIT_HALO_64;
+        return p;
+    }
     const bool r8t = r8 || half_rows_for_tail((M / (16 * tw)) * (N / (tw == 32 ? 64 : 128)) * groups * p.split_k);
     p.tile = r8t ? NBP_TILE_SPLIT_HALO_R8 : (tw == 32 && N % 128 == 0) ? NBP_TILE_SPLIT_HALO_128 : NBP_TILE_SPLIT_HALO_64;
     return p;
@@ -1621,14 +1708,15 @@
     NBP_RETURN_IF(b0 >= (1ll << 31) || b1 >= (1ll << 31) || bw >= (1ll << 31), NBP_E_SHAPE);
     a.bytes0 = (unsigned)b0; a.bytes1 = C1 ? (unsigned)b1 : (unsigned)b0; a.bytesw = (unsigned)bw;
     const bool have_up = ups && o.planes_up && o.wamax_up && (!o2 || (o2->planes_up && o2->wamax_up));
-    const ConvPlan p = nbp_plan_conv_split(a.M, N, (C0 + C1) / 32 * 9, split_k, groups, H, W, ksize, have_up ? 1 : 0);
+    const ConvPlan p = nbp_plan_conv_split(a.M, N, (C0 + C1) / 32 * 9, split_k, groups, H, W, ksize, have_up ? 1 : 0, !one && !bn_part);
     NBP_RETURN_IF(p.tile != NBP_TILE_SPLIT_HALO_64 && p.tile != NBP_TILE_SPLIT_HALO_128 && p.tile != NBP_TILE_SPLIT_UP && p.tile != NBP_TILE_SPLIT_HALO_R8 &&
                   p.tile != NBP_TILE_SPLIT_UP_R8, NBP_E_SHAPE);
     const bool ph = p.tile == NBP_TILE_SPLIT_UP || p.tile == NBP_TILE_SPLIT_UP_R8;
     const bool r8 = p.tile == NBP_TILE_SPLIT_HALO_R8 || p.tile == NBP_TILE_SPLIT_UP_R8;
     const bool wide = p.tile == NBP_TILE_SPLIT_HALO_128;
     const int th = (r8 || wide) ? 8 : 16;
-    a.split_k = p.split_k; a.chunks_per_split = p.chunks_per_split;
+    a.split_k = p.split_k; a.chunks_per_split = p.chunks_per_split; a.chain_slices = p.chain_slices;
+    const bool serial = p.chain_slices > 1;
     a.chunks_total = (C0 + C1) / 16;
     const int tw = ph ? split_tile_width(H / 2, W / 2, N, ksize) : split_tile_width(H, W, N, ksize);
     if (ph) {
@@ -1654,6 +1742,9 @@
     a.partial = nullptr;
     if (p.split_k > 1) {
         NBP_RETURN_IF(!ws || ws_bytes < (size_t)groups * p.split_k * a.M * N * sizeof(float), NBP_E_WS);
+        a.partial = (float*)ws;
+    } else if (serial) {
+        NBP_RETURN_IF(!ws || ws_bytes < (size_t)groups * (p.chain_slices - 1) * a.M * N * sizeof(float), NBP_E_WS);
         a.partial = (float*)ws;
     }
     static const int allow_pool = nbp_tune_int("NBP_CONV_POOL", 1);
@@ -1677,6 +1768,13 @@
         }
         return ph ? (tw == 32 ? launch_h2o<32, 2, 2, true, true, true>(a, st, p.tile, one) : launch_h2o<16, 2, 4, true, true>(a, st, p.tile, one))
                   : (tw == 32 ? launch_h2o<32, 4, 2, false, true>(a, st, p.tile, one) : launch_h2o<16, 2, 4, false, true>(a, st, p.tile, one));
+    }
+    if (serial) {
+        NBP_RETURN_IF(r8 || one, NBP_E_SHAPE);
+        NBP_RETURN_IF(ph && tw == 32, NBP_E_SHAPE);
+        return ph ? launch_h2s<16, 2, 4, true>(a, st, p.tile)
+                  : (tw == 32 ? (wide ? launch_h2s<32, 2, 4, false>(a, st, p.tile) : launch_h2s<32, 4, 2, false>(a, st, p.tile))
+                              : launch_h2s<16, 2, 4, false>(a, st, p.tile));
     }
     int rc = (ph && !r8 && tw == 32) ? launch_h2o<32, 2, 2, true, false, true>(a, st, p.tile, one)
            : r8 ? (ph ? (tw == 32 ? launch_h2o<32, 2, 2, true>(a, st, p.tile, one) : launch_h2o<16, 1, 4, true>(a, st, p.tile, one))
@@ -2015,9 +2113,21 @@
 extern "C" size_t nbp_conv_split_planned_workspace_bytes_k(int B, int H, int W, int C, int N, int ups, int split_k, int* split_k_out) {
     if (B < 1 || H < 1 || W < 1 || C < 32 || N < 1) return 0;
     const ConvPlan p = nbp_plan_conv_split((long long)B * H * W, N, C / 32 * 9, split_k, 1, H, W, 3, ups ? 1 : 0);
-    if (split_k_out) *split_k_out = p.tile ? p.split_k : 0;
-    const int sk = (p.tile && p.split_k > 1) ? p.split_k : 0;
+    const int total = p.split_k * p.chain_slices;
+    if (split_k_out) *split_k_out = p.tile ? total : 0;
+    const int sk = (p.tile && total > 1) ? total : 0;
     return 256 + (size_t)sk * B * H * W * N * sizeof(float);
+}
+extern "C" int nbp_conv_split_plan(int B, int H, int W, int C, int N, int ups, int groups, int split_k, int* split_k_out,
+                                   int* chain_slices_out) {
+    if (split_k_out) *split_k_out = 0;
+    if (chain_slices_out) *chain_slices_out = 0;
+    if (B < 1 || H < 1 || W < 1 || C < 32 || N < 1 || groups < 1 || groups > 2) return 0;
+    const ConvPlan p = nbp_plan_conv_split((long long)B * H * W, N, C / 32 * 9, split_k, groups, H, W, 3, ups ? 1 : 0);
+    if (!p.tile) return 0;
+    if (split_k_out) *split_k_out = p.split_k;
+    if (chain_slices_out) *chain_slices_out = p.chain_slices;
+    return p.tile;
 }
 
 static int conv3x3_split_impl(const float* src0, int C0, const float* src1, int C1, int ups, int B, int H, int W,
@@ -2041,6 +2151,28 @@
                         nullptr, nullptr};
     return nbp_conv_split_launch_g(o, nullptr, C0, C1, ups, B, H, W, 3, N, relu, split_k, (char*)ws + 256, ws_bytes - 256, st, nullptr,
                                    nullptr, nullptr, nullptr, bn_part, bn_rows, one);
+}
+extern "C" int nbp_conv3x3_split_groups_f32(const float* const* src0, int C0, const float* const* src1, int C1, const float* const* psi0,
+                                            int ups, int B, int H, int W, const void* const* w_planes, const void* const* wamax, int N,
+                                            const float* const* scale, const float* const* shift, int relu, float* const* out,
+                                            const void* const* amax_in, void* const* amax_out, float* const* pool_out, int* pooled_out,
+                                            int groups, int split_k, void* ws, size_t ws_bytes, void* stream) {
+    NBP_ENTER();
+    if (pooled_out) *pooled_out = 0;
+    NBP_RETURN_IF(groups < 1 || groups > 2 || !src0 || !w_planes || !wamax || !scale || !shift || !out || !amax_in, NBP_E_ARG);
+    NBP_RETURN_IF(C1 > 0 && !src1, NBP_E_ARG);
+    ConvOperandsSplit o[2];
+    for (int g = 0; g < groups; ++g) {
+        NBP_RETURN_IF(!amax_in[g], NBP_E_ARG);
+        o[g] = ConvOperandsSplit{src0[g], C1 > 0 ? src1[g] : nullptr, w_planes[g], scale[g], shift[g], out[g], (const unsigned*)amax_in[g],
+                                 (const unsigned*)amax_in[g], (const unsigned*)wamax[g], amax_out ? (unsigned*)amax_out[g] : nullptr,
+                                 nullptr, nullptr};
+        o[g].psi0 = psi0 ? psi0[g] : nullptr;
+        if (ups) { o[g].planes_up = w_planes[g]; o[g].wamax_up = (const unsigned*)wamax[g]; }
+    }
+    NBP_RETURN_IF(ups && (C1 > 0 || psi0), NBP_E_SHAPE);
+    return nbp_conv_split_launch_g(o[0], groups == 2 ? &o[1] : nullptr, C0, C1, ups ? 1 : 0, B, H, W, 3, N, relu, split_k, ws, ws_bytes,
+                                   (hipStream_t)stream, (pool_out && groups == 1) ? pool_out : nullptr, pooled_out);
 }
 extern "C" int nbp_conv3x3_split_f32(const float* src0, int C0, const float* src1, int C1, int ups, int B, int H, int W,
                                      const void* w_planes, const void* wamax, int N, const float* scale, const float* shift,
```

New measurement: 2353, median of 6. 1.5% higher.
